# rg2/DeepFluoroLabeling-IPCAI2020

Measured on AMD Instinct MI355X. Metric: train images/sec, paper U-Net (depth 6, wf 5, BN, strided-conv down, seg + 14-landmark heads), 1x192x192 (8x-downsampled 184x184 padded), higher is better.
Workload: dtype bf16 (bf16 activations, activation gradients and GEMM weight copies in HBM; bf16 MFMA, fp32 accumulate, BatchNorm statistics, losses, weight gradients and master weights); 1 GPU; BASELINE configs[1]: 8x-downsampled, seg + 14-landmark heat-map dual head, batch 16 per GPU, Dice+NCC loss, SGD nesterov; global_batch=16, image=1x192x192, parallelism=dp1, math=bf16s, optimizer=dfl_amd.SGD(momentum 0.9, nesterov, wd 1e-4)

## Files before the change

deepfluorolabeling-ipcai2020_amd/_native.py:

```python
import ctypes as C
import os

_HERE = os.path.dirname(os.path.abspath(__file__))
LIB_PATH = os.environ.get('DFL_LIB_OVERRIDE') or os.path.join(_HERE, 'lib', 'libdfl_hip.so')

i32, i64, f32 = C.c_int32, C.c_int64, C.c_float
fp = C.c_void_p


class ConvArgs(C.Structure):
    _fields_ = [('x', fp), ('w', fp), ('bias', fp), ('in_scale', fp), ('in_shift', fp), ('add', fp),
                ('add_scale', fp), ('add_shift', fp), ('stat_other', fp), ('y', fp), ('stat_partials', fp),
                ('partial', fp),
                ('N', i32), ('Hin', i32), ('Win', i32), ('Cin', i32), ('ldx', i32),
                ('KH', i32), ('KW', i32), ('stride', i32), ('pad', i32),
                ('Hout', i32), ('Wout', i32), ('Ntot', i32), ('ldy', i32),
                ('ldadd', i32), ('ldso', i32), ('relu', i32), ('accumulate', i32), ('scatter2x2', i32),
                ('splits', i32), ('w_split', i32), ('x_split', i32), ('x_bf16', i32), ('y_bf16', i32),
                ('x2', fp), ('ldx2', i32), ('x_mode', i32),
                ('stat_totals', fp), ('in_tot', fp), ('in_gamma', fp), ('in_beta', fp), ('add_tot', fp), ('add_gamma', fp),
                ('add_beta', fp), ('in_count', C.c_double), ('add_count', C.c_double), ('bn_eps', f32), ('reserved3', i32),
                ('in_mean', fp), ('in_invstd', fp), ('x_out', fp), ('ldxo', i32), ('latency_form', i32), ('out_scale', fp), ('out_shift', fp)]


class WgradArgs(C.Structure):
    _fields_ = [('g', fp), ('d', fp), ('in_scale', fp), ('in_shift', fp), ('dw', fp), ('partial', fp),
                ('N', i32), ('Hin', i32), ('Win', i32), ('Cg', i32), ('ldg', i32),
                ('KH', i32), ('KW', i32), ('stride', i32), ('pad', i32),
                ('Hout', i32), ('Wout', i32), ('Cm', i32), ('ldd', i32), ('splits', i32), ('d_split', i32),
                ('g_bf16', i32), ('d_bf16', i32), ('d_mode', i32), ('d2', fp), ('coef', fp), ('bias_partial', fp),
                ('ldd2', i32), ('reserved2', i32), ('coef_tot', fp), ('bn_gamma', fp), ('bn_mean', fp), ('bn_invstd', fp),
                ('bn_count', C.c_double)]


class PackJob(C.Structure):
    _fields_ = [('src', fp), ('dst', fp), ('A', i32), ('B', i32), ('C', i32), ('kind', i32), ('flip', i32),
                ('split', i32), ('dst2', fp), ('kind2', i32), ('flip2', i32), ('first_tile', i32), ('split2', i32)]


PACK_PLAIN, SGD_PLAIN_TILE = 100, 4096


class SgdPackArgs(C.Structure):
    _fields_ = [('jobs_dev', fp), ('grad_delta', i64), ('buf_delta', i64), ('njobs', i32), ('total_tiles', i32), ('lr', f32),
                ('momentum', f32), ('weight_decay', f32), ('grad_scale', f32), ('nesterov', i32), ('reserved', i32)]


OPTIM_ADAM, OPTIM_RMSPROP = 1, 2


class OptimPackArgs(C.Structure):
    _fields_ = [('jobs_dev', fp), ('grad_delta', i64), ('state1_delta', i64), ('state2_delta', i64), ('beta1', C.c_double),
                ('beta2', C.c_double), ('alpha', C.c_double), ('njobs', i32), ('total_tiles', i32), ('kind', i32), ('lr', f32),
                ('eps', f32), ('weight_decay', f32), ('grad_scale', f32), ('step_size', f32), ('bc2_sqrt', f32), ('momentum', f32)]


class BnLiveJob(C.Structure):
    _fields_ = [('totals', fp), ('gamma', fp), ('beta', fp), ('running_mean', fp), ('running_var', fp), ('num_batches_tracked', fp),
                ('scale', fp), ('shift', fp), ('save_mean', fp), ('save_invstd', fp), ('count', i64), ('C', i32), ('eps', f32),
                ('momentum', f32), ('reserved', i32)]


class BnBwdLiveJob(C.Structure):
    _fields_ = [('totals', fp), ('save_mean', fp), ('save_invstd', fp), ('dgamma', fp), ('dbeta', fp), ('sum_out', fp), ('C', i32),
                ('reserved', i32)]


class BnBwdLiveArgs(C.Structure):
    _fields_ = [('jobs_dev', fp), ('njobs', i32), ('max_C', i32)]


class BnLiveArgs(C.Structure):
    _fields_ = [('jobs_dev', fp), ('njobs', i32), ('max_C', i32)]


class BnFinalizeArgs(C.Structure):
    _fields_ = [('partials', fp), ('gamma', fp), ('beta', fp), ('running_mean', fp), ('running_var', fp),
                ('num_batches_tracked', fp), ('scale', fp), ('shift', fp), ('save_mean', fp), ('save_invstd', fp),
                ('count', i64), ('nblocks', i32), ('C', i32), ('eps', f32), ('momentum', f32)]


class ColstatsArgs(C.Structure):
    _fields_ = [('a', fp), ('b', fp), ('partials', fp), ('M', i64), ('C', i32), ('lda', i32), ('ldb', i32),
                ('nblocks', i32), ('bf16', i32), ('reserved', i32)]


class BnBwdFinalizeArgs(C.Structure):
    _fields_ = [('partials', fp), ('gamma', fp), ('save_mean', fp), ('save_invstd', fp), ('dgamma', fp),
                ('dbeta', fp), ('coef', fp), ('count', i64), ('nblocks', i32), ('C', i32)]


class BnReluBwdArgs(C.Structure):
    _fields_ = [('dy', fp), ('r', fp), ('coef', fp), ('dpre', fp), ('partials', fp), ('M', i64), ('C', i32),
                ('lddy', i32), ('ldr', i32), ('ldo', i32), ('nblocks', i32), ('split_out', i32), ('bf16', i32),
                ('reserved', i32)]


class AffineCopyArgs(C.Structure):
    _fields_ = [('x', fp), ('y', fp), ('scale', fp), ('shift', fp),
                ('N', i32), ('H', i32), ('W', i32), ('C', i32),
                ('ldx', i32), ('xH', i32), ('xW', i32), ('xoy', i32), ('xox', i32),
                ('ldy', i32), ('yH', i32), ('yW', i32), ('yoy', i32), ('yox', i32),
                ('accumulate', i32), ('bf16', i32)]


class PoolArgs(C.Structure):
    _fields_ = [('x', fp), ('y', fp), ('dx', fp), ('N', i32), ('H', i32), ('W', i32), ('C', i32),
                ('ldx', i32), ('ldy', i32), ('lddx', i32), ('bf16', i32)]


class HeadFwdArgs(C.Structure):
    _fields_ = [('x', fp), ('w_seg', fp), ('w_l1', fp), ('w_l2', fp), ('seg', fp), ('heat', fp),
                ('N', i32), ('H', i32), ('W', i32), ('F', i32), ('ldx', i32),
                ('NC', i32), ('NM', i32), ('L', i32), ('softmax', i32), ('x_bf16', i32)]


class HeadBwdArgs(C.Structure):
    _fields_ = [('x', fp), ('seg', fp), ('dseg', fp), ('dheat', fp), ('w_seg', fp), ('w_l1', fp), ('w_l2', fp),
                ('dx', fp), ('scratch', fp),
                ('N', i32), ('H', i32), ('W', i32), ('F', i32), ('ldx', i32), ('lddx', i32),
                ('NC', i32), ('NM', i32), ('L', i32), ('softmax', i32), ('scratch_ld', i32), ('x_bf16', i32),
                ('dw_seg', fp), ('dw_l1', fp), ('dw_l2', fp), ('wg_partial', fp),
                ('stat_other', fp), ('stat_totals', fp), ('ldso', i32), ('reserved4', i32)]


class LossArgs(C.Structure):
    _fields_ = [('seg', fp), ('tseg', fp), ('heat', fp), ('theat', fp), ('loss', fp), ('dseg', fp), ('dheat', fp),
                ('ncc_vals', fp), ('sums', fp),
                ('seg_sN', i64), ('seg_sC', i64), ('seg_sH', i64), ('tseg_sN', i64), ('tseg_sC', i64), ('tseg_sH', i64),
                ('heat_sN', i64), ('heat_sC', i64), ('heat_sH', i64), ('theat_sN', i64), ('theat_sC', i64),
                ('theat_sH', i64),
                ('B', i32), ('C', i32), ('L', i32), ('h', i32), ('w', i32), ('skip_bg', i32),
                ('dice_wgt', f32), ('heat_wgt', f32), ('grad_scale', fp),
                ('dseg_sN', i64), ('dseg_sC', i64), ('dseg_sH', i64), ('dheat_sN', i64), ('dheat_sC', i64), ('dheat_sH', i64),
                ('stage', i32), ('reserved', i32)]


class EnsembleArgs(C.Structure):
    _fields_ = [('seg_ptrs', fp), ('heat_ptrs', fp), ('labels', fp), ('avg_seg', fp), ('heat_out', fp),
                ('minmax', fp),
                ('nnets', i32), ('C', i32), ('L', i32), ('Hp', i32), ('Wp', i32), ('h', i32), ('w', i32),
                ('oy', i32), ('ox', i32), ('raw_heat', i32)]


class SumPartialsArgs(C.Structure):
    _fields_ = [('src', fp), ('dst', fp), ('n', i64), ('splits', i32), ('T', i32)]


class PackArgs(C.Structure):
    _fields_ = [('jobs_dev', fp), ('max_elems', i64), ('njobs', i32), ('tiled', i32)]


class BnEvalArgs(C.Structure):
    _fields_ = [('gamma', fp), ('beta', fp), ('running_mean', fp), ('running_var', fp), ('scale', fp),
                ('shift', fp), ('C', i32), ('eps', f32)]


class ReducePartialsArgs(C.Structure):
    _fields_ = [('partials', fp), ('out', fp), ('nblocks', i32), ('stride', i32), ('C', i32), ('reserved', i32)]


class MemsetArgs(C.Structure):
    _fields_ = [('ptr', fp), ('bytes', i64)]


class ReduceJob(C.Structure):
    _fields_ = [('src', fp), ('dst', fp), ('n', i64), ('stride', i64), ('count', i32), ('first_block', i32),
                ('T', i32), ('reserved', i32)]


class ReduceBatchArgs(C.Structure):
    _fields_ = [('jobs_dev', fp), ('njobs', i32), ('total_blocks', i32)]


class PrepArgs(C.Structure):
# ... 50 lines not shown
    _fields_ = [('inp', fp), ('out', fp), ('plan', ResamplePlan), ('B', i32), ('reserved', i32)]


class FullresArgs(C.Structure):
    _fields_ = [('image', fp), ('labels', fp), ('rot180', fp), ('boxes', fp), ('n_boxes', fp), ('texts', fp),
                ('stamp_spans', fp), ('text_stamps', fp), ('text_masks', fp), ('scratch', fp), ('out', fp),
                ('plan', ResamplePlan), ('B', i32), ('H', i32), ('W', i32), ('n_tint', i32), ('tint_scale', f32),
                ('tint_add', (f32 * 3) * OVERLAY_MAX_COLORS), ('n_text_stamps', i32), ('n_stamp_spans', i32),
                ('tile0', i32), ('n_tiles', i32)]


MESH_MAX_LABELS, MESH_MC_CELLS, MESH_MAX_ITERS = 4, 4096, 64


class MeshMcArgs(C.Structure):
    _fields_ = [('volume', fp), ('tri_off', fp), ('tri_edges', fp), ('block_counts', fp), ('block_offsets', fp),
                ('totals', fp), ('keys', fp), ('nx', i32), ('ny', i32), ('nz', i32), ('n_labels', i32),
                ('labels', i32 * MESH_MAX_LABELS)]


class MeshDecodeArgs(C.Structure):
    _fields_ = [('keys', fp), ('pos', fp), ('V', i64), ('nx', i32), ('ny', i32)]


class MeshTopoArgs(C.Structure):
    _fields_ = [('tris', fp), ('edge_keys', fp), ('vt_keys', fp), ('T', i64), ('V', i64)]


class MeshCsrArgs(C.Structure):
    _fields_ = [('keys', fp), ('counts', fp), ('col', fp), ('row_ptr', fp), ('fixed', fp), ('nnz', i64), ('div', i64),
                ('col_div', i64), ('n_rows', i64)]


class MeshSmoothArgs(C.Structure):
    _fields_ = [('x', fp), ('row_ptr', fp), ('col', fp), ('fixed', fp), ('t_a', fp), ('t_b', fp), ('acc', fp), ('out', fp),
                ('V', i64), ('iterations', i32), ('reserved', i32), ('coef', f32 * (MESH_MAX_ITERS + 1))]


class MeshXformArgs(C.Structure):
    _fields_ = [('x', fp), ('out', fp), ('V', i64), ('M', C.c_double * 16)]


class MeshNormalsArgs(C.Structure):
    _fields_ = [('pos', fp), ('tris', fp), ('vt_ptr', fp), ('vt_tri', fp), ('normals', fp), ('V', i64)]


PREPROC_MAX_FACTOR = 16


class PreprocProjsArgs(C.Structure):
    _fields_ = [('pixels', fp), ('rot180', fp), ('out', fp), ('scratch', fp), ('N', i32), ('R', i32), ('C', i32),
                ('crop', i32), ('factor', i32), ('u16', i32), ('log', i32), ('min_intensity', f32)]


class PreprocSegsArgs(C.Structure):
    _fields_ = [('segs', fp), ('rot180', fp), ('out', fp), ('status', fp), ('N', i32), ('R', i32), ('C', i32),
                ('crop', i32), ('factor', i32), ('reserved', i32)]


class RestoreLabelsArgs(C.Structure):
    _fields_ = [('labels', fp), ('rot180', fp), ('out', fp), ('N', i32), ('R', i32), ('C', i32), ('crop', i32),
                ('factor', i32), ('reserved', i32)]


DRR_EXACT, DRR_TRILINEAR, DRR_MAX_LABELS = 0, 1, 16


class DrrObject(C.Structure):
    _fields_ = [('o', f32 * 3), ('M', f32 * 9), ('box_lo', i32 * 3), ('box_hi', i32 * 3), ('mask', C.c_uint32)]


class DrrArgs(C.Structure):
    _fields_ = [('mu', fp), ('labels', fp), ('objects', fp), ('att', fp), ('plen', fp), ('label_map', fp), ('qscale', f32 * 9),
                ('nx', i32), ('ny', i32), ('nz', i32), ('H', i32), ('W', i32), ('views', i32), ('n_obj', i32), ('n_labels', i32),
                ('interp', i32), ('mapping', i32), ('step_mm', f32), ('min_len_mm', f32), ('reserved', i32)]


SIM_TOTALS = 5


class SimPrepareArgs(C.Structure):
    _fields_ = [('fixed', fp), ('mask', fp), ('fx', fp), ('fy', fp), ('counted', fp), ('totals', fp), ('H', i32), ('W', i32)]


class SimGradnccArgs(C.Structure):
    _fields_ = [('moving', fp), ('fx', fp), ('fy', fp), ('counted', fp), ('totals', fp), ('scratch', fp), ('cost', fp),
                ('scratch_doubles', i64), ('V', i32), ('H', i32), ('W', i32), ('reserved', i32)]


EXPOSE_MAX_RADIUS = 8


class ExposeArgs(C.Structure):
    _fields_ = [('att', fp), ('out', fp), ('key_q', fp), ('key_e', fp), ('z1', fp), ('z2', fp),
                ('taps', f32 * (2 * EXPOSE_MAX_RADIUS + 1)), ('rho', i32), ('V', i32), ('R', i32), ('C', i32), ('u16', i32),
                ('quantum', i32), ('electronic', i32), ('photons', f32), ('gain', f32), ('electronic_sigma', f32)]


class UpsampleArgs(C.Structure):
    _fields_ = [('x', fp), ('y', fp), ('N', i32), ('H', i32), ('W', i32), ('C', i32), ('ldx', i32), ('ldy', i32),
                ('bf16', i32), ('accumulate', i32)]


class SyncArgs(C.Structure):
    _fields_ = [('event', i32), ('reserved', i32)]


CONV_CFG_LATENCY = 39


class ConvPairArgs(C.Structure):
    _fields_ = [('a', fp), ('b', fp)]


class Op(C.Structure):
    _fields_ = [('kind', i32), ('stream', i32), ('args', fp)]


OP_CONV, OP_WGRAD, OP_SUM_PARTIALS, OP_PACK, OP_BN_FINALIZE, OP_BN_EVAL, OP_COLSTATS, OP_BN_BWD_FINALIZE, \
    OP_BN_RELU_BWD, OP_REDUCE_PARTIALS, OP_AFFINE_COPY, OP_POOL_FWD, OP_POOL_BWD, OP_HEAD_FWD, OP_HEAD_BWD, \
    OP_MEMSET, OP_REDUCE_BATCH, OP_RECORD, OP_WAIT, OP_UPSAMPLE_FWD, OP_UPSAMPLE_BWD, OP_BN_FINALIZE_LIVE, OP_BN_BWD_FINALIZE_LIVE, \
    OP_CONV_PAIR = range(1, 25)

_KIND_OF = {ConvArgs: OP_CONV, WgradArgs: OP_WGRAD, SumPartialsArgs: OP_SUM_PARTIALS, PackArgs: OP_PACK,
            BnFinalizeArgs: OP_BN_FINALIZE, BnEvalArgs: OP_BN_EVAL, ColstatsArgs: OP_COLSTATS,
            BnBwdFinalizeArgs: OP_BN_BWD_FINALIZE, BnReluBwdArgs: OP_BN_RELU_BWD,
            ReducePartialsArgs: OP_REDUCE_PARTIALS, AffineCopyArgs: OP_AFFINE_COPY, HeadFwdArgs: OP_HEAD_FWD,
            HeadBwdArgs: OP_HEAD_BWD, MemsetArgs: OP_MEMSET, ReduceBatchArgs: OP_REDUCE_BATCH, BnLiveArgs: OP_BN_FINALIZE_LIVE, BnBwdLiveArgs: OP_BN_BWD_FINALIZE_LIVE,
            ConvPairArgs: OP_CONV_PAIR}

_SIZEOF_ORDER = [ConvArgs, WgradArgs, PackJob, BnFinalizeArgs, ColstatsArgs, BnBwdFinalizeArgs, BnReluBwdArgs,
                 AffineCopyArgs, PoolArgs, HeadFwdArgs, HeadBwdArgs, LossArgs, EnsembleArgs, Op, ReduceJob, PrepArgs, EstLandsArgs,
                 UpsampleArgs, AugmentArgs, AugmentItem, OverlayArgs, ResamplePlan, ResampleArgs, FullresArgs, MeshMcArgs, MeshDecodeArgs,
                 MeshTopoArgs, MeshCsrArgs, MeshSmoothArgs, MeshXformArgs, MeshNormalsArgs, PreprocProjsArgs, PreprocSegsArgs,
                 RestoreLabelsArgs, SimPrepareArgs, SimGradnccArgs, ExposeArgs, DrrObject, DrrArgs, OptimPackArgs]

EXPORTS = ['dfl_version', 'dfl_last_error', 'dfl_sizeof', 'dfl_conv2d', 'dfl_conv_grid_m', 'dfl_conv2d_wgrad',
           'dfl_wgrad_suggest_splits', 'dfl_sum_partials', 'dfl_pack_weights', 'dfl_bn_finalize',
           'dfl_bn_eval_prepare', 'dfl_rowblock_count', 'dfl_colstats', 'dfl_bn_bwd_finalize',
           'dfl_bn_relu_bwd_apply', 'dfl_reduce_partials', 'dfl_affine_copy', 'dfl_maxpool2x2_fwd',
           'dfl_maxpool2x2_bwd', 'dfl_head_fwd', 'dfl_head_bwd', 'dfl_head_scratch_ld', 'dfl_head_scratch_off',
           'dfl_dice_ncc_loss', 'dfl_loss_scratch_doubles', 'dfl_ensemble_reduce', 'dfl_sgd_step', 'dfl_exec',
           'dfl_exec_timed', 'dfl_conv_config', 'dfl_wgrad_config', 'dfl_conv_suggest_splits', 'dfl_reduce_batch',
           'dfl_reduce_job_blocks', 'dfl_prep_batch', 'dfl_prep_scratch_doubles', 'dfl_est_lands', 'dfl_hard_dice', 'dfl_get_math_mode',
           'dfl_set_math_mode', 'dfl_graph_capture', 'dfl_graph_launch', 'dfl_graph_nodes', 'dfl_graph_destroy',
           'dfl_set_conv_rows_min_tiles', 'dfl_conv_candidates', 'dfl_conv_force_geometry', 'dfl_conv_tune_add',
           'dfl_head_wgrad_blocks', 'dfl_head_scratch_ld_for', 'dfl_head_scratch_off_for', 'dfl_upsample2x_fwd',
           'dfl_upsample2x_bwd', 'dfl_bn_finalize_live', 'dfl_bn_bwd_finalize_live', 'dfl_pack_weights_tiled',
           'dfl_sgd_pack_tiled', 'dfl_conv2d_pair', 'dfl_conv_pair_ok', 'dfl_augment_batch',
           'dfl_augment_scratch_bytes', 'dfl_overlay_batch', 'dfl_resample_bilinear_u8', 'dfl_fullres_overlay',
           'dfl_mesh_mc_count', 'dfl_mesh_mc_emit', 'dfl_mesh_decode', 'dfl_mesh_topology', 'dfl_mesh_csr', 'dfl_mesh_smooth',
           'dfl_mesh_transform', 'dfl_mesh_normals', 'dfl_adam_step', 'dfl_rmsprop_step', 'dfl_optim_pack_tiled',
           'dfl_preproc_projs', 'dfl_preproc_segs', 'dfl_restore_labels', 'dfl_drr_render', 'dfl_sim_prepare', 'dfl_sim_gradncc',
           'dfl_sim_scratch_doubles', 'dfl_drr_expose']


class DflError(RuntimeError):
    pass


_lib = None


def lib():
    global _lib
    if _lib is not None:
        return _lib
    if not os.path.exists(LIB_PATH):
        raise DflError('libdfl_hip.so not found at %s -- build it with __graft_entry__.build() '
                       '(csrc/build.sh); there is no fallback path' % LIB_PATH)
    L = C.CDLL(LIB_PATH)
    for name in EXPORTS:
        if not hasattr(L, name):
            raise DflError('libdfl_hip.so does not export %s' % name)
    L.dfl_last_error.restype = C.c_char_p
    L.dfl_loss_scratch_doubles.restype = i64
    L.dfl_loss_scratch_doubles.argtypes = [i32, i32, i32]
    L.dfl_rowblock_count.argtypes = [i64, i32]
    L.dfl_sum_partials.argtypes = [fp, fp, i64, i32, i32, fp]
    L.dfl_pack_weights.argtypes = [fp, i32, i64, fp]
    L.dfl_pack_weights_tiled.argtypes = [fp, i32, i32, fp]
    L.dfl_sgd_pack_tiled.argtypes = [fp, fp]
    L.dfl_bn_eval_prepare.argtypes = [fp, fp, fp, fp, fp, fp, i32, f32, fp]
    L.dfl_reduce_partials.argtypes = [fp, fp, i32, i32, i32, fp]
    L.dfl_reduce_batch.argtypes = [fp, i32, i32, fp]
    L.dfl_bn_finalize_live.argtypes = [fp, i32, i32, fp]
    L.dfl_bn_bwd_finalize_live.argtypes = [fp, i32, i32, fp]
    L.dfl_reduce_job_blocks.argtypes = [i64, i32]
    L.dfl_prep_scratch_doubles.restype = i64
    L.dfl_prep_scratch_doubles.argtypes = [i32]
    L.dfl_prep_batch.argtypes = [fp, fp]
    L.dfl_est_lands.argtypes = [fp, fp]
    L.dfl_augment_scratch_bytes.restype = i64
    L.dfl_augment_scratch_bytes.argtypes = [i32, i32, i32, i32]
    L.dfl_augment_batch.argtypes = [fp, fp]
    L.dfl_overlay_batch.argtypes = [fp, fp]
    L.dfl_resample_bilinear_u8.argtypes = [fp, fp]
    L.dfl_fullres_overlay.argtypes = [fp, fp]
    for fn in ('dfl_preproc_projs', 'dfl_preproc_segs', 'dfl_restore_labels', 'dfl_drr_render', 'dfl_sim_prepare', 'dfl_sim_gradncc',
               'dfl_drr_expose'):
        getattr(L, fn).argtypes = [fp, fp]
    for fn in ('dfl_mesh_mc_count', 'dfl_mesh_mc_emit', 'dfl_mesh_decode', 'dfl_mesh_topology', 'dfl_mesh_csr',
               'dfl_mesh_smooth', 'dfl_mesh_transform', 'dfl_mesh_normals'):
        getattr(L, fn).argtypes = [fp, fp]
    L.dfl_sim_scratch_doubles.restype = i64
    L.dfl_sim_scratch_doubles.argtypes = [i32, i32, i32]
    L.dfl_set_math_mode.argtypes = [i32]
    L.dfl_hard_dice.argtypes = [fp, fp, i64, i32, i32, fp, fp, fp]
    L.dfl_sgd_step.argtypes = [fp, fp, fp, i64, f32, f32, f32, f32, i32, i32, fp]
    L.dfl_adam_step.argtypes = [fp, fp, fp, fp, i64, f32, C.c_double, C.c_double, f32, f32, f32, f32, f32, fp]
    L.dfl_rmsprop_step.argtypes = [fp, fp, fp, fp, i64, f32, C.c_double, f32, f32, f32, f32, fp]
    L.dfl_optim_pack_tiled.argtypes = [fp, fp]
    L.dfl_exec.argtypes = [fp, i32, fp]
    L.dfl_exec_timed.argtypes = [fp, i32, fp, fp]
    L.dfl_set_conv_rows_min_tiles.argtypes = [i32]
    L.dfl_graph_capture.argtypes = [fp, i32, fp, fp]
    L.dfl_graph_launch.argtypes = [fp, fp]
    L.dfl_graph_nodes.argtypes = [fp]
    L.dfl_graph_destroy.argtypes = [fp]
    L.dfl_conv_config.argtypes = [fp]
    L.dfl_wgrad_config.argtypes = [fp]
    for fn in ('dfl_conv2d', 'dfl_conv2d_wgrad', 'dfl_bn_finalize', 'dfl_colstats', 'dfl_bn_bwd_finalize',
               'dfl_bn_relu_bwd_apply', 'dfl_affine_copy', 'dfl_maxpool2x2_fwd', 'dfl_maxpool2x2_bwd',
               'dfl_head_fwd', 'dfl_head_bwd', 'dfl_dice_ncc_loss', 'dfl_ensemble_reduce', 'dfl_upsample2x_fwd',
               'dfl_upsample2x_bwd'):
        getattr(L, fn).argtypes = [fp, fp]
    for fn in ('dfl_conv_grid_m', 'dfl_wgrad_suggest_splits', 'dfl_conv_suggest_splits'):
        getattr(L, fn).argtypes = [fp]
    L.dfl_conv_candidates.argtypes = [fp, fp, i32]
    L.dfl_head_wgrad_blocks.argtypes = [i64]
    L.dfl_head_scratch_ld_for.argtypes = [i32, i32, i32, i32]
    L.dfl_head_scratch_off_for.argtypes = [i32, i32, i32, i32, i32]
    L.dfl_conv_force_geometry.argtypes = [fp]
    L.dfl_conv_tune_add.argtypes = [fp, fp]
    L.dfl_conv2d_pair.argtypes = [fp, fp, fp]
    L.dfl_conv_pair_ok.argtypes = [fp, fp]
    for k, cls in enumerate(_SIZEOF_ORDER):
        if L.dfl_sizeof(k) != C.sizeof(cls):
            raise DflError('struct mirror %s has size %d, library says %d' % (cls.__name__, C.sizeof(cls), L.dfl_sizeof(k)))
    _lib = L
    if os.environ.get('DFL_TUNE', '1') != '0':
        load_tuning(L, TUNE_PATH)
    return L


TUNE_PATH = os.environ.get('DFL_TUNE_FILE') or os.path.join(_HERE, 'tune', 'gfx950_convp.txt')


def load_tuning(L, path):
    if not os.path.exists(path):
        return 0
    n = 0
    with open(path) as f:
        for line in f:
            line = line.split('#')[0].split()
            if len(line) != 15:
                continue
            v = (i32 * 15)(*[int(t) for t in line])
            if L.dfl_conv_tune_add(C.addressof(v), C.addressof(v) + 40) < 0:
                raise DflError('bad tuning entry in %s: %s' % (path, ' '.join(line)))
            n += 1
    return n


def check(rc, what=''):
    if rc < 0:
        raise DflError('%s failed (%d): %s' % (what or 'libdfl_hip call', rc, lib().dfl_last_error().decode()))
    return rc


def ptr(t):
    return None if t is None else t.data_ptr()


def byref(s):
    return C.addressof(s)


def call(fn_name, args_struct, stream):
    return check(getattr(lib(), fn_name)(C.addressof(args_struct), stream), fn_name)


class Graph:

    def __init__(self, handle, program):
        self.handle, self.program = handle, program

    def launch(self, stream):
        check(lib().dfl_graph_launch(self.handle, stream), 'dfl_graph_launch')

    @property
    def nodes(self):
        return lib().dfl_graph_nodes(self.handle)

    def __del__(self):
        try:
            if self.handle and _lib is not None:
                _lib.dfl_graph_destroy(self.handle)
        except Exception:
            pass
        self.handle = None


class Program:

    def __init__(self):
        self.structs = []
        self.kinds = []
        self.streams = []
        self.volatile = []
        self._ops = None
        self.keep = []
        self._chunks = {}

    def add(self, args_struct, kind=None, stream=0, volatile=False):
        self.structs.append(args_struct)
        self.kinds.append(kind if kind is not None else _KIND_OF[type(args_struct)])
        self.streams.append(stream)
        self.volatile.append(bool(volatile))
        self._ops = None
        self._chunks = {}
        return args_struct

    def insert(self, index, args_struct, kind=None, stream=0, volatile=False):
        self.structs.insert(index, args_struct)
        self.kinds.insert(index, kind if kind is not None else _KIND_OF[type(args_struct)])
        self.streams.insert(index, stream)
        self.volatile.insert(index, bool(volatile))
        self._ops = None
        self._chunks = {}
        return args_struct

    def pop(self):
        self.kinds.pop()
        self.streams.pop()
        self.volatile.pop()
        self._ops = None
        self._chunks = {}
        return self.structs.pop()

    def record(self, event, stream=0):
        return self.add(SyncArgs(event=event), OP_RECORD, stream)

    def wait(self, event, stream=0):
        return self.add(SyncArgs(event=event), OP_WAIT, stream)

    def add_pool(self, args_struct, backward):
        return self.add(args_struct, OP_POOL_BWD if backward else OP_POOL_FWD)

    def extend(self, other):
        for s, k, st, v in zip(other.structs, other.kinds, other.streams, other.volatile):
            self.add(s, k, st, v)
        self.keep.extend(other.keep)

    def __len__(self):
        return len(self.structs)

    def _build(self):
        arr = (Op * len(self.structs))()
        for i, (s, k) in enumerate(zip(self.structs, self.kinds)):
            arr[i].kind = k
            arr[i].stream = self.streams[i]
            arr[i].args = C.addressof(s)
        self._ops = arr

    def run_timed(self, stream):
        if self._ops is None:
            self._build()
        n = len(self.structs)
        ms = (C.c_float * n)()
        check(lib().dfl_exec_timed(C.addressof(self._ops), n, stream, C.addressof(ms)), 'dfl_exec_timed')
        return list(ms)

    def capture(self, stream, start=0, count=None):
        if self._ops is None:
            self._build()
        n = len(self.structs) - start if count is None else count
        h = C.c_void_p()
        check(lib().dfl_graph_capture(C.addressof(self._ops) + start * C.sizeof(Op), n, stream, C.addressof(h)),
              'dfl_graph_capture')
        return Graph(h.value, self)

    MIN_GRAPH_OPS = 2

    def graph_chunks(self, stream, start=0, count=None):
        n = len(self.structs) - start if count is None else count
        key = (start, n)
        chunks = self._chunks.get(key)
        if chunks is None:
# ... 32 lines not shown
```

deepfluorolabeling-ipcai2020_amd/csrc/conv_plan.hip:

```cpp
#include <stdlib.h>
#include <string.h>

#include <mutex>
#include <vector>

#include "conv_plan.h"
#include "conv_rows.h"
#include "direct_small.h"

namespace dfl {

bool convs_enabled() {
  static const bool on = [] {
    const char* e = getenv("DFL_CONVS");
    return e == nullptr || atoi(e) != 0;
  }();
  return on;
}

enum class Family { Patch, Latency, Unrolled, Narrow };
struct Tile {
  Family family;
  int layout;
  int pers;
// ... 230 lines not shown
  if (!ok) return false;
  pl->launch = t.launch;
  pl->pers = t.pers;
  return true;
}

struct ConvGeom { int tile, ipp, ph, pw, splits; };
static thread_local ConvGeom t_force = {-1, 0, 0, 0, 0};
struct TuneEntry { int key[10]; ConvGeom g; };
static std::mutex g_tune_mu;
static std::vector<TuneEntry> g_tune;

static void tune_key(const dfl_conv_args& a, int* k) {
  k[0] = a.N; k[1] = a.Hin; k[2] = a.Win; k[3] = a.Cin; k[4] = a.Ntot;
  k[5] = a.KH; k[6] = a.KW; k[7] = a.stride; k[8] = a.pad; k[9] = a.scatter2x2 ? 1 : 0;
}

static bool tune_lookup(const dfl_conv_args& a, ConvGeom* g) {
  int k[10];
  tune_key(a, k);
  std::lock_guard<std::mutex> lock(g_tune_mu);
  for (const TuneEntry& e : g_tune)
    if (memcmp(e.key, k, sizeof(k)) == 0) {
      *g = e.g;
      return true;
    }
  return false;
}

static bool columns_ok(const dfl_conv_args& a, int wn, int tn, bool wide) {
  const int n32 = (int)ceil_div(a.Ntot, 32) * 32, bn = wn * tn * 32;
  if (wide) return !(bn > n32 || (bn < 64 && n32 >= 64) || (tn > 1 && bn > a.Ntot));
  if (tn != 1) return false;
  return a.Ntot <= 32 ? wn == 1 : (a.Ntot <= 64 ? wn == 2 : wn == 4);
}

static int patch_shapes(const ConvP& base, const PatchTile& t, bool wide, int (*shapes)[3]) {
  const int QP = t.WM * t.TM * 32;
  const int HW = base.Hg * base.Wg;
  int ns = 0;
  if (HW <= QP) {
    shapes[ns][0] = QP / HW; shapes[ns][1] = base.Hg; shapes[ns][2] = base.Wg; ++ns;
  }
  if (base.Wg <= QP) {
    int ph = QP / base.Wg;
    if (ph > base.Hg) ph = base.Hg;
    shapes[ns][0] = 1; shapes[ns][1] = ph; shapes[ns][2] = base.Wg; ++ns;
  }
  static const int kPh[] = {1, 2, 4, 8, 16, 3, 6, 12};
  for (int k = 0; k < (wide ? 8 : 5) && ns < 22; ++k) {
    const int ph = kPh[k];
    int pw = QP / ph;
    if (pw >= base.Wg || ph > base.Hg) continue;
    shapes[ns][0] = 1; shapes[ns][1] = ph; shapes[ns][2] = pw; ++ns;
  }
  return ns;
}

template <typename F>
static void for_each_candidate(const dfl_conv_args& a, const ConvP& base, int force_splits, bool wide, F&& f) {
  const std::vector<Tile>& T = tiles();
  for (int ti = 0; ti < (int)T.size(); ++ti) {
    const Tile& t = T[ti];
    if (t.measured && !wide) continue;
    int shapes[24][3];
    int ns = 0;
    if (t.family == Family::Patch) {
      const PatchTile& pt = convp_tiles()[t.layout];
      if (columns_ok(a, pt.WN, pt.TN, wide)) ns = patch_shapes(base, pt, wide, shapes);
    } else if (t.family == Family::Unrolled) {
      const QLayout& q = convq_layouts()[t.layout];
      if (columns_ok(a, q.WN, 1, wide)) {
        shapes[0][0] = 1; shapes[0][1] = 8 * q.WM; shapes[0][2] = 12; ns = 1;
      }
    } else if (t.family == Family::Narrow) {
      if (convn_shape_ok(a)) {
        shapes[0][0] = 1; narrow_patch(t.layout, &shapes[0][1], &shapes[0][2]); ns = 1;
      }
    }
    for (int si = 0; si < ns; ++si) {
      for (int sp = 1; sp <= 32; sp *= 2) {
        if (force_splits > 0 && sp != force_splits) continue;
        if (!wide && a.scatter2x2 == 0 && a.accumulate == 0 && sp > 1 && base.T * a.Cin < 1024) break;
        ConvPlan q;
        q.p = base;
        if (!try_geometry(a, &q, t, shapes[si][0], shapes[si][1], shapes[si][2], sp)) continue;
        if (q.p.splits != sp) continue;
        f(ti, q);
      }
    }
  }
}

static int convp_validate(const dfl_conv_args* a, ConvP* p) {
  DFL_REQUIRE(a->x && a->w && a->y, "dfl_conv2d (bf16): x, w and y are required");
  DFL_REQUIRE(a->N > 0 && a->Hin > 0 && a->Win > 0 && a->Cin > 0 && a->Ntot > 0, "dfl_conv2d (bf16): bad sizes");
  DFL_REQUIRE(a->Ntot % 8 == 0 && a->ldy % 8 == 0 && aligned16(a->y) && (a->add == nullptr || (a->ldadd % 8 == 0 && aligned16(a->add))) &&
                  (a->stat_other == nullptr || (a->ldso % 8 == 0 && aligned16(a->stat_other))),
              "dfl_conv2d (bf16): output columns and the pixel strides of y / add / stat_other must be multiples of 8, tensors 16-byte aligned");
  {
    const int64_t opx = (int64_t)a->N * a->Hout * a->Wout, lim = 1ll << 32;
    DFL_REQUIRE(opx * a->ldy < lim && (a->add == nullptr || opx * a->ldadd < lim) && (a->stat_other == nullptr || opx * a->ldso < lim),
                "dfl_conv2d (bf16): y / add / stat_other must stay below 2^32 elements");
  }
  DFL_REQUIRE(a->Cin % 16 == 0 && a->ldx % 8 == 0 && aligned16(a->x) && aligned16(a->w),
              "dfl_conv2d (bf16): needs Cin %% 16 == 0, ldx %% 8 == 0 and 16-byte aligned x / w (Cin = %d, ldx = %d)", a->Cin, a->ldx);
  DFL_REQUIRE(a->w_split == 2, "dfl_conv2d (bf16): weights must be packed with dfl_pack_job.split = 2");
  DFL_REQUIRE(a->x_mode != 0 || (a->in_scale == nullptr) == (a->in_shift == nullptr), "dfl_conv2d: in_scale/in_shift go together");
  DFL_REQUIRE(a->in_tot == nullptr || (a->in_scale == nullptr && a->in_gamma != nullptr && a->in_count > 0 &&
                                       (a->x_mode == 0 ? a->in_beta != nullptr : (a->in_mean != nullptr && a->in_invstd != nullptr))),
              "dfl_conv2d (bf16): in_tot replaces in_scale / in_shift and needs in_gamma, in_count and in_beta (x_mode 0) or in_mean, in_invstd (x_mode 1)");
  DFL_REQUIRE(a->add_tot == nullptr || (a->add != nullptr && a->add_scale == nullptr && a->add_gamma != nullptr && a->add_beta != nullptr && a->add_count > 0),
              "dfl_conv2d (bf16): add_tot replaces add_scale / add_shift and needs add, add_gamma, add_beta, add_count");

  DFL_REQUIRE((a->add_scale == nullptr) == (a->add_shift == nullptr), "dfl_conv2d: add_scale/add_shift go together");
  DFL_REQUIRE(a->KH * a->KW <= 16 && a->KH > 0 && a->KW > 0 && a->stride > 0 && a->pad >= 0, "dfl_conv2d (bf16): bad window");
  memset(p, 0, sizeof(*p));
  p->a = *a;
  if (a->scatter2x2) {
    DFL_REQUIRE(a->KH == 1 && a->KW == 1 && a->stride == 1 && a->pad == 0, "dfl_conv2d: scatter2x2 needs a 1x1 gather");
    DFL_REQUIRE(a->Ntot % 4 == 0 && a->Hout >= 2 * a->Hin && a->Wout >= 2 * a->Win, "dfl_conv2d: scatter2x2 geometry");
    DFL_REQUIRE(a->add == nullptr, "dfl_conv2d: scatter2x2 has no add epilogue");
    p->Hg = a->Hin;
    p->Wg = a->Win;
    p->Cout = a->Ntot / 4;
  } else {
    const int ho = (a->Hin + 2 * a->pad - a->KH) / a->stride + 1;
    const int wo = (a->Win + 2 * a->pad - a->KW) / a->stride + 1;
    DFL_REQUIRE(ho == a->Hout && wo == a->Wout, "dfl_conv2d: Hout/Wout (%d,%d) do not match the window (%d,%d)", a->Hout,
                a->Wout, ho, wo);
    p->Hg = a->Hout;
    p->Wg = a->Wout;
    p->Cout = a->Ntot;
  }
  DFL_REQUIRE(a->ldy >= p->Cout, "dfl_conv2d: ldy < Cout");
  const int64_t M = (int64_t)a->N * p->Hg * p->Wg;
  DFL_REQUIRE(M < (1ll << 31), "dfl_conv2d: too many pixels");
  p->Mtot = (int)M;
  p->T = a->KH * a->KW;
  const int64_t xb = (((int64_t)a->N * a->Hin * a->Win - 1) * a->ldx + a->Cin) * 2;
  const int64_t wb = (int64_t)p->T * a->Cin * a->Ntot * 2;
  const int64_t lim = (1ll << 31) - 4096;
  DFL_REQUIRE(xb < lim && wb < lim, "dfl_conv2d (bf16): tensors must stay below 2 GiB");
  p->x_bytes = (uint32_t)xb;
  p->w_bytes = (uint32_t)wb;
  if (a->x_mode != 0) {
    DFL_REQUIRE(a->x_mode == 1 && a->x2 != nullptr && a->in_shift == nullptr && a->ldx2 % 8 == 0 && aligned16(a->x2) &&
                    (a->in_scale == nullptr || aligned16(a->in_scale)),
                "dfl_conv2d (bf16): x_mode 1 needs x2 (16-byte aligned, ldx2 %% 8 == 0), coefficients in in_scale and no in_shift");
    const int64_t x2b = (((int64_t)a->N * a->Hin * a->Win - 1) * a->ldx2 + a->Cin) * 2;
    DFL_REQUIRE(x2b < lim, "dfl_conv2d (bf16): tensors must stay below 2 GiB");
    p->x2_bytes = (uint32_t)x2b;
  }
  p->xo_bytes = 0;
  if (a->x_out != nullptr) {
    DFL_REQUIRE(a->x_mode == 1 && a->KH == 3 && a->KW == 3 && a->stride == 1 && a->pad == 1 && a->Hout == a->Hin && a->Wout == a->Win,
                "dfl_conv2d (bf16): x_out goes with x_mode 1 of a 3x3 stride-1 pad-1 layer");
    DFL_REQUIRE(a->ldxo % 8 == 0 && a->ldxo >= a->Cin && aligned16(a->x_out) && a->x_out != a->x && a->x_out != a->x2,
                "dfl_conv2d (bf16): x_out must be 16-byte aligned with ldxo %% 8 == 0, ldxo >= Cin, and a tensor of its own");
    const int64_t xob = (((int64_t)a->N * a->Hin * a->Win - 1) * a->ldxo + a->Cin) * 2;
    DFL_REQUIRE(xob < lim, "dfl_conv2d (bf16): tensors must stay below 2 GiB");
    p->xo_bytes = (uint32_t)xob;
  }
  return DFL_OK;
}

static int convp_plan_search(const dfl_conv_args* a, ConvPlan* pl, int force_splits) {
  memset(pl, 0, sizeof(*pl));
  const int rc = convp_validate(a, &pl->p);
  if (rc != DFL_OK) return rc;

  if (t_force.tile < 0 && convs_eligible(*a, pl->p)) {
    convs_plan(*a, &pl->p, force_splits);
    pl->lds = (size_t)pl->p.lds_bytes;
    pl->launch = tiles()[CONVS_TILE].launch;
    return DFL_OK;
  }

  DFL_REQUIRE(a->out_scale == nullptr, "dfl_conv2d (bf16): out_scale / out_shift are implemented by the latency form only (dfl_conv_config tells)");
  const ConvP base = pl->p;
  int best_tile = -1;
  {
    ConvGeom g;
    const bool forced = t_force.tile >= 0;
    if (forced) g = t_force;
    if (forced || tune_lookup(*a, &g)) {
      if (g.tile >= 0 && g.tile < (int)tiles().size() && (force_splits <= 0 || force_splits == g.splits)) {
        ConvPlan q = *pl;
        if (try_geometry(*a, &q, tiles()[g.tile], g.ipp, g.ph, g.pw, g.splits) && q.p.splits == g.splits) {
          *pl = q;
          best_tile = g.tile;
        }
      }
      DFL_REQUIRE(!forced || best_tile >= 0, "dfl_conv2d (bf16): the forced geometry (tile %d, patch %dx%dx%d, %d slices) does not fit this layer",
                  g.tile, g.ipp, g.ph, g.pw, g.splits);
    }
  }
  if (best_tile < 0) {
    double best = 1e300;
    for_each_candidate(*a, base, force_splits, false, [&](int ti, const ConvPlan& q) {
      if (q.cost < best) {
        best = q.cost;
        *pl = q;
        best_tile = ti;
      }
    });
  }
  DFL_REQUIRE(best_tile >= 0, "dfl_conv2d (bf16): no patch geometry fits this layer (%dx%d, Cin %d, Ntot %d)", a->Hin, a->Win,
              a->Cin, a->Ntot);
  pl->p.tile = best_tile;
  static const bool dbg = getenv("DFL_CONVP_DEBUG") != nullptr;
  if (dbg && force_splits == 0)
    fprintf(stderr, "convp %dx%d Cin%d->%d k%d s%d: tile %d patch %dx%dx%d CK %d blocks %d splits %d lds %zu cost %.0f%s\n", a->Hin, a->Win,
            a->Cin, a->Ntot, a->KH, a->stride, best_tile, pl->p.IPP, pl->p.PH, pl->p.PW, pl->p.CK, pl->p.nblk, pl->p.splits, pl->lds,
            pl->cost, tiles()[best_tile].measured ? " (measured)" : "");
  return DFL_OK;
}

struct PlanMemo { dfl_conv_args a; int force_splits; ConvPlan pl; };
static std::mutex g_memo_mu;
static std::vector<PlanMemo> g_memo[64];
static inline unsigned memo_bucket(const dfl_conv_args* a, int force_splits) {
  uint64_t h = 1469598103934665603ull;
  const uint64_t* w = reinterpret_cast<const uint64_t*>(a);
  for (size_t i = 0; i < sizeof(dfl_conv_args) / 8; ++i) h = (h ^ w[i]) * 1099511628211ull;
  h ^= (uint64_t)force_splits;
  return (unsigned)((h ^ (h >> 29)) & 63u);
}
static void memo_clear() {
  std::lock_guard<std::mutex> lock(g_memo_mu);
  for (auto& b : g_memo) b.clear();
}

int convp_plan(const dfl_conv_args* a, ConvPlan* pl, int force_splits) {
  static_assert(sizeof(dfl_conv_args) % 8 == 0, "hashed as 64-bit words");
  DFL_REQUIRE(a != nullptr && pl != nullptr, "dfl_conv2d (bf16): null arguments");
  if (t_force.tile >= 0) return convp_plan_search(a, pl, force_splits);
  const unsigned b = memo_bucket(a, force_splits);
  {
    std::lock_guard<std::mutex> lock(g_memo_mu);
    for (const PlanMemo& m : g_memo[b])
      if (m.force_splits == force_splits && memcmp(&m.a, a, sizeof(*a)) == 0) {
        *pl = m.pl;
        return DFL_OK;
      }
  }
  const int rc = convp_plan_search(a, pl, force_splits);
  if (rc != DFL_OK) return rc;
  std::lock_guard<std::mutex> lock(g_memo_mu);
  if (g_memo[b].size() >= 256) g_memo[b].clear();
  g_memo[b].push_back(PlanMemo{*a, force_splits, *pl});
  return DFL_OK;
}

static int convp_candidates(const dfl_conv_args* a, int32_t* out, int max) {
  ConvPlan pl;
  const int saved_tile = t_force.tile;
  t_force.tile = -1;
  const int rc = convp_plan(a, &pl, 0);
  t_force.tile = saved_tile;
  if (rc != DFL_OK) return -1;
  int n = 0;
  for_each_candidate(*a, pl.p, 0, true, [&](int ti, const ConvPlan& q) {
    if (n < max) {
      int32_t* o = out + 5 * n;
      o[0] = ti; o[1] = q.p.IPP; o[2] = q.p.PH; o[3] = q.p.PW; o[4] = q.p.splits;
    }
    ++n;
  });
  return n;
}

static bool latency32_plan(const ConvK& k, int force_splits, ConvPlan* pl) {
  if (!k.a.latency_form || !convs_enabled()) return false;
  memset(pl, 0, sizeof(*pl));
  ConvP* p = &pl->p;
  p->a = k.a;
  p->Mtot = k.Mtot;
  p->Hg = k.Hg;
  p->Wg = k.Wg;
  p->Cout = k.Cout;
  p->T = k.a.KH * k.a.KW;
  p->x_bytes = k.x_bytes;
  p->w_bytes = k.w_bytes;
  if (!convs_eligible(k.a, *p)) return false;
  convs_plan(k.a, p, force_splits);
  pl->lds = (size_t)p->lds_bytes;
  pl->launch = convs_launch;
  return true;
}

int conv_route(const dfl_conv_args* a, int want_splits, ConvRoute* r) {
  if (a != nullptr && a->x_bf16) {
    const int rc = convp_plan(a, &r->plan, want_splits);
    if (rc != DFL_OK) return rc;
    r->form = FORM_BF16;
    r->cfg = 16 + r->plan.p.tile;
    r->splits = r->plan.p.splits;
    return DFL_OK;
  }
  const int rc = conv_prepare(a, &r->k);
  if (rc != DFL_OK) return rc;
  const ConvK& k = r->k;
  int sug;
  if (direct_conv_ok(a)) {
    r->stat_form = FORM_DIRECT;
    r->stat_cfg = CFG_DIRECT;
    sug = 1;
  } else {
    const int t = conv_rows_tile(k);
    r->stat_form = t ? FORM_ROWS : FORM_GEMM;
    r->stat_cfg = t ? t : conv_gemm_cfg(k);
    const int rs = conv_rows_splits(k);
    sug = rs ? rs : conv_gemm_splits(k);
  }
  r->form = r->stat_form;
  r->cfg = r->stat_cfg;
  r->splits = want_splits > 0 ? want_splits : sug;
  if (convs_first_ok(a)) {
    r->form = FORM_FIRST;
    r->cfg = 16 + CONVS_TILE;
    r->splits = 1;
  } else if (latency32_plan(k, want_splits, &r->plan)) {
    r->form = FORM_LATENCY32;
    r->cfg = 16 + CONVS_TILE;
    r->splits = r->plan.p.splits;
  }
  return DFL_OK;
}

static int want_splits(const dfl_conv_args* a) { return a != nullptr && a->splits > 1 ? a->splits : 1; }

int conv_pair_route(const dfl_conv_args* a, const dfl_conv_args* b, ConvRoute* r) {
  if (a == nullptr || b == nullptr || !a->latency_form || conv_route(a, want_splits(a), r) != DFL_OK) return 0;
  return r->form == FORM_BF16 || r->form == FORM_LATENCY32 ? convs_pair_ok(a, b, r->plan.p) : 0;
}

}

extern "C" int dfl_conv_config(const dfl_conv_args* a) {
  dfl::ConvRoute r;
  const int rc = dfl::conv_route(a, dfl::want_splits(a), &r);
  return rc != DFL_OK ? rc : r.cfg;
}

extern "C" int dfl_conv_grid_m(const dfl_conv_args* a) {
  dfl::ConvRoute r;
  const int rc = dfl::conv_route(a, dfl::want_splits(a), &r);
  if (rc != DFL_OK) return rc;
  if (r.form == dfl::FORM_BF16) return r.plan.p.splits > 1 ? dfl::convp_finish_rows(r.plan.p) : r.plan.p.npatch;
  if (a->splits > 1) return dfl::conv_finish_rows(r.k.Mtot, a->Ntot);
  if (r.stat_form == dfl::FORM_DIRECT) return dfl::direct_conv_blocks(a);
  if (r.stat_form == dfl::FORM_ROWS) return r.k.Mtot / dfl::conv_rows_bm(r.stat_cfg);
  return (int)dfl::ceil_div(r.k.Mtot, dfl::conv_gemm_bm(r.stat_cfg));
}

extern "C" int dfl_conv_suggest_splits(const dfl_conv_args* a) {
  dfl::ConvRoute r;
  const int rc = dfl::conv_route(a, 0, &r);
  return rc != DFL_OK ? rc : r.splits;
}

extern "C" int dfl_conv_pair_ok(const dfl_conv_args* a, const dfl_conv_args* b) {
  dfl::ConvRoute r;
  return dfl::conv_pair_route(a, b, &r);
}

extern "C" int dfl_conv_candidates(const dfl_conv_args* a, int32_t* out, int32_t max_rows) {
  DFL_REQUIRE(a != nullptr && (out != nullptr || max_rows <= 0) && a->x_bf16, "dfl_conv_candidates: bf16 convolution arguments and an output table are required");
  const int n = dfl::convp_candidates(a, out, max_rows);
  return n < 0 ? (int)DFL_ERR_INVALID_ARG : n;
}

extern "C" int dfl_conv_force_geometry(const int32_t* geom) {
  if (geom == nullptr) dfl::t_force.tile = -1;
  else dfl::t_force = dfl::ConvGeom{geom[0], geom[1], geom[2], geom[3], geom[4]};
  return DFL_OK;
}

extern "C" int dfl_conv_tune_add(const int32_t* key, const int32_t* geom) {
  DFL_REQUIRE(key == nullptr || geom != nullptr, "dfl_conv_tune_add: a key needs a geometry");
  dfl::memo_clear();
  std::lock_guard<std::mutex> lock(dfl::g_tune_mu);
  if (key == nullptr) {
    dfl::g_tune.clear();
    return DFL_OK;
  }
  dfl::TuneEntry e;
  for (int i = 0; i < 10; ++i) e.key[i] = key[i];
  e.g = dfl::ConvGeom{geom[0], geom[1], geom[2], geom[3], geom[4]};
  for (dfl::TuneEntry& o : dfl::g_tune)
    if (memcmp(o.key, e.key, sizeof(e.key)) == 0) {
      o = e;
      return DFL_OK;
    }
  dfl::g_tune.push_back(e);
  return DFL_OK;
}
```

deepfluorolabeling-ipcai2020_amd/csrc/convp.h:

```cpp
#pragma once
#include "common.h"

namespace dfl {

struct ConvP {
  dfl_conv_args a;
  int Mtot, Cout;
  int Hg, Wg;
  int PH, PW, IPP;
  int npy, npx, npatch;
  int IH, IW;
  int CK, nblk, blk_per_slice;
  int splits, T;
  int pix_stride, upp_shift;
  int lds_bytes, tile;
  int ntiles, grid, xcd_mode;
  uint32_t x_bytes, w_bytes;
  uint32_t x2_bytes, xo_bytes;
  uint32_t mPP, mPW;
  int tab_off, pad1;
  int s_mt, s_nt, s_ksplit_shift, s_cpk_shift, s_ksteps, s_kper;
  uint32_t qm_npatch, qm_ntiles, qm_perimg, qm_npx;
  int q_ngroups, q_stride;
};
constexpr int CONVS_TILE = 39;
constexpr int kLdsOptIn = 160 * 1024;

struct ConvPlan;
typedef int (*ConvLaunch)(const ConvPlan& pl, hipStream_t s);

struct ConvPlan {
  ConvP p;
  size_t lds;
  ConvLaunch launch;
  int pers;
  double cost;
};

int convp_plan(const dfl_conv_args* a, ConvPlan* pl, int force_splits);
int convp_launch(const ConvPlan& pl, hipStream_t s);
int convp_finish_rows(const ConvP& p);
bool convs_enabled();

struct PatchTile { int WM, WN, TM, TN, GA, KS; ConvLaunch launch; };
constexpr int kNumPatchTiles = CONVS_TILE;
const PatchTile* convp_tiles();

struct QLayout { int WM, WN, KS; ConvLaunch launch; };
constexpr int kNumQ = 9;
const QLayout* convq_layouts();
bool convq_shape_ok(const dfl_conv_args& a);
size_t convq_lds_bytes(int ck, int layout, int blk_per_slice, int pers, int* tab_off);
bool convq_pers_ok(int layout, int ck, int x_mode);
bool convq_ck_ok(int layout, int ck);

struct NLayout { int WX, R; ConvLaunch launch; };
constexpr int kNumN = 6;
const NLayout* convn_layouts();
bool convn_shape_ok(const dfl_conv_args& a);
bool convn_layout_ok(int layout, int ntot, int cin);
size_t convn_lds_bytes(int layout, int cin, int ntot, int pers, int* tab_off);
bool convn_pers_ok(int layout, const dfl_conv_args& a);

bool convs_eligible(const dfl_conv_args& a, const ConvP& p);
void convs_plan(const dfl_conv_args& a, ConvP* p, int force_splits);
int convs_launch(const ConvPlan& pl, hipStream_t s);
bool convs_first_ok(const dfl_conv_args* a);
int convs_first_launch(const dfl_conv_args* a, hipStream_t s);
int convs_pair_ok(const dfl_conv_args* a, const dfl_conv_args* b, const ConvP& pa);
int convs_pair_launch(const ConvP& pa, const dfl_conv_args* b, hipStream_t s);

struct WgP;
int wgradp_suggest_splits(const dfl_wgrad_args* a);
int wgradp_launch(const dfl_wgrad_args* a, hipStream_t s);
int wgradp_config(const dfl_wgrad_args* a);

}
```

deepfluorolabeling-ipcai2020_amd/csrc/convp_bf16.hip:

```cpp
#include "common.h"
#include "convp.h"

namespace dfl {

constexpr uint32_t POOB = 0x80000000u;
#ifndef DFL_BRB_U
#define DFL_BRB_U 4
#endif
typedef unsigned int pu32x4 __attribute__((ext_vector_type(4)));

__device__ __forceinline__ float round_bf(float v) { return (float)(__bf16)v; }
__device__ __forceinline__ int pdiv(int q, uint32_t m, int d) { return d == 1 ? q : (int)__umulhi((uint32_t)q, m); }
__device__ __forceinline__ float ld_bf(const __bf16* p) { return (float)*p; }

#ifndef DFL_CONVP_G1
#define DFL_CONVP_G1 4
#endif
#ifndef DFL_CONVP_PRIME
#define DFL_CONVP_PRIME 0
#endif
template <int WM, int WN, int TM, int TN, int AFF, bool GA, int KS = 1>
#ifndef DFL_CONVP_ADEPTH
#define DFL_CONVP_ADEPTH 1
#endif
#ifndef DFL_CONVP_MINW3
#define DFL_CONVP_MINW3 2
#endif
__global__ void __launch_bounds__(256 * KS, (TM * TN >= 6 || KS == 2) ? 1 : (TM * TN <= 3 ? DFL_CONVP_MINW3 : 2)) convp_kernel(const ConvP p) {
  static_assert(WM * WN == 4, "four waves per k-group");
  static_assert(KS == 1 || (KS == 2 && !GA), "two k-groups: LDS-image form only");
  static_assert(AFF != 2 || !GA, "the fused BatchNorm + ReLU backward operand is staged through LDS");
  constexpr int NT = 256 * KS;
  extern __shared__ __attribute__((aligned(16))) unsigned char smem[];
  const dfl_conv_args& a = p.a;
  const int tid = threadIdx.x, lane = tid & 63, wave = (tid >> 6) & 3;
  const int kg = KS == 1 ? 0 : __builtin_amdgcn_readfirstlane(tid >> 8);
  const int wm = wave / WN, wn = wave % WN, li = lane & 31, lh = lane >> 5;
  const int S = p.pix_stride;
  const int PP = p.PH * p.PW;

  int bpatch, btile, bslice;
  {
    const int b = blockIdx.x;
    if (p.xcd_mode == 0) {
      bpatch = b % p.npatch;
      const int r = b / p.npatch;
      btile = r % p.ntiles;
      bslice = r / p.ntiles;
    } else {
      const int x = b & 7, r = b >> 3;
      int s;
      if (p.xcd_mode == 1) {
        s = x + 8 * (r / p.npatch);
        bpatch = r % p.npatch;
      } else {
        const int pairs = p.ntiles * p.splits;
        s = x % pairs;
        bpatch = x / pairs + (8 / pairs) * r;
      }
      if (s >= p.ntiles * p.splits || bpatch >= p.npatch) return;
      btile = s % p.ntiles;
      bslice = s / p.ntiles;
    }
  }
  const int per_img = p.npy * p.npx;
  const int pg = bpatch / per_img, pr = bpatch - pg * per_img;
  const int ppy = pr / p.npx, ppx = pr - ppy * p.npx;
  const int img0 = pg * p.IPP, gy0 = ppy * p.PH, gx0 = ppx * p.PW;
  const int n0 = btile * (WN * TN * 32);

  uint32_t a_base[TM];
#pragma unroll
  for (int i = 0; i < TM; ++i) {
    int q = (wm * TM + i) * 32 + li;
    int img = pdiv(q, p.mPP, PP);
    int r = q - img * PP;
    int py = pdiv(r, p.mPW, p.PW), px = r - py * p.PW;
    if (img >= p.IPP) img = 0, py = 0, px = 0;
    a_base[i] = (uint32_t)(((img * p.IH + py * a.stride) * p.IW + px * a.stride) * S + lh * 16);
  }

  __amdgpu_buffer_rsrc_t rsX = __builtin_amdgcn_make_buffer_rsrc(const_cast<float*>(a.x), 0, (int)p.x_bytes, 0x00020000);
  __amdgpu_buffer_rsrc_t rsW = __builtin_amdgcn_make_buffer_rsrc(const_cast<float*>(a.w), 0, (int)p.w_bytes, 0x00020000);
  uint32_t b_voff[TN];
#pragma unroll
  for (int j = 0; j < TN; ++j) {
    const int n = n0 + (wn * TN + j) * 32 + li;
    b_voff[j] = n < a.Ntot ? (uint32_t)(n * 32 + lh * 16) : POOB;
  }

  f32x16 acc[TM][TN];
#pragma unroll
  for (int i = 0; i < TM; ++i)
#pragma unroll
    for (int j = 0; j < TN; ++j)
#pragma unroll
      for (int r = 0; r < 16; ++r) acc[i][j][r] = 0.f;

  float* in_tab = reinterpret_cast<float*>(smem + p.tab_off);
  float* add_tab = in_tab + 384;
  {
    constexpr int BN0 = WN * TN * 32;
    const bool scat0 = a.scatter2x2 != 0;
    for (int col = tid; col < BN0; col += NT) {
      const int n = n0 + col;
      float sc_ = 1.f, sh_ = 0.f, b_ = 0.f;
      if (n < a.Ntot) {
        if (a.bias != nullptr) b_ = a.bias[scat0 ? n % p.Cout : n];
        if (a.add != nullptr) {
          if (a.add_scale != nullptr) sc_ = a.add_scale[n], sh_ = a.add_shift[n];
          else if (a.add_tot != nullptr) bn_live_affine(a.add_tot, a.add_gamma, a.add_beta, a.add_count, a.bn_eps, a.Ntot, n, &sc_, &sh_);
        }
      }
      add_tab[col] = sc_;
      add_tab[BN0 + col] = sh_;
      add_tab[2 * BN0 + col] = b_;
    }
  }

  const int upp = p.CK >> 3, upp_sh = p.upp_shift;
  const int cg = tid & (upp - 1);
  const int dpix = NT >> upp_sh;
  const int dpix_y = dpix / p.IW, dpix_x = dpix - dpix_y * p.IW;
  const int npix = p.IPP * p.IH * p.IW;
  const int CKC = p.CK >> 4;
  const int ckc_sh = p.upp_shift - 1;
  const int S_steps = p.T * CKC;
  const int cin_chunks = a.Cin >> 4;
  const int KW = a.KW;
  const int kw_magic = (256 + KW - 1) / KW;

#ifdef DFL_CONVP_TRACE
  long long tr_t[10];
  tr_t[6] = tr_t[7] = tr_t[8] = 0;
  tr_t[0] = __builtin_amdgcn_s_memtime();
  tr_t[5] = __builtin_amdgcn_s_memrealtime();
  tr_t[1] = tr_t[2] = 0;
#define TR(i) tr_t[i] = __builtin_amdgcn_s_memtime();
#define TRACC(i, t0) tr_t[i] += __builtin_amdgcn_s_memtime() - (t0);
#else
#define TR(i)
#define TRACC(i, t0)
#endif
  if constexpr (GA) {
    uint32_t a_goff[TM];
#pragma unroll
    for (int i = 0; i < TM; ++i) {
      const int q = (wm * TM + i) * 32 + li;
      const int img = pdiv(q, p.mPP, PP);
      const int r = q - img * PP;
      const int py = pdiv(r, p.mPW, p.PW), px = r - py * p.PW;
      const int n = img0 + img, gy = gy0 + py, gx = gx0 + px;
      const bool ok = img < p.IPP && n < a.N && gy < p.Hg && gx < p.Wg;
      a_goff[i] = ok ? (uint32_t)(((n * a.Hin + gy * a.stride) * a.Win + gx * a.stride) * a.ldx) * 2u + (uint32_t)lh * 16u : POOB;
    }
    constexpr int GG = 2;
    const int chunks = a.Cin >> 4;
    const int steps = p.T * chunks;
    const int ngr = (steps + GG - 1) / GG;
    pu32x4 areg[3][GG][TM], bqreg[3][GG][TN];
    int ls = 0, lcc = 0, ltx = 0;
    uint32_t lao = 0;
    const uint32_t bstep = (uint32_t)a.Ntot * 32u;
    const uint32_t pixb = (uint32_t)a.ldx * 2u;
    const uint32_t tap_x = pixb - (uint32_t)chunks * 32u, tap_y = (uint32_t)(a.Win - a.KW) * pixb;
    auto load_gr = [&](int set) {
#pragma unroll
      for (int e = 0; e < GG; ++e) {
        const bool live = ls < steps;
        const uint32_t ao = live ? lao : 0u, bo = live ? (uint32_t)ls * bstep : 0u;
#pragma unroll
        for (int i = 0; i < TM; ++i) areg[set][e][i] = __builtin_amdgcn_raw_buffer_load_b128(rsX, live ? a_goff[i] : POOB, ao, 0);
#pragma unroll
        for (int j = 0; j < TN; ++j) bqreg[set][e][j] = __builtin_amdgcn_raw_buffer_load_b128(rsW, live ? b_voff[j] : POOB, bo, 0);
        ++ls;
        lao += 32u;
        if (++lcc == chunks) {
          lcc = 0;
          lao += tap_x;
          if (++ltx == a.KW) {
            ltx = 0;
            lao += tap_y;
          }
        }
// ... 62 lines not shown
#pragma unroll
          for (int e = 0; e < 8; ++e) {
            sc[e] = in_tab[cg * 8 + e];
            sh[e] = in_tab[128 + cg * 8 + e];
          }
        } else {
#pragma unroll
          for (int e = 0; e < 8; ++e) {
            sc[e] = a.in_scale[c0 + cg * 8 + e];
            sh[e] = a.in_shift[c0 + cg * 8 + e];
          }
        }
      }
      __amdgpu_buffer_rsrc_t rsR = rsX, rsO = rsX;
      bool store_on = false;
      if constexpr (AFF == 2) {
        rsR = __builtin_amdgcn_make_buffer_rsrc(const_cast<float*>(a.x2), 0, (int)p.x2_bytes, 0x00020000);
        store_on = a.x_out != nullptr && btile == 0;
        if (store_on) rsO = __builtin_amdgcn_make_buffer_rsrc(a.x_out, 0, (int)p.xo_bytes, 0x00020000);
        if (a.in_tot != nullptr) {
          if (tid < p.CK)
            bn_live_coef(a.in_tot, a.in_gamma, a.in_mean, a.in_invstd, a.in_count, a.Cin, c0 + tid, in_tab + tid, in_tab + 128 + tid, in_tab + 256 + tid);
          __syncthreads();
#pragma unroll
          for (int e = 0; e < 8; ++e) {
            sc[e] = in_tab[cg * 8 + e];
            sh[e] = in_tab[128 + cg * 8 + e];
            sq[e] = in_tab[256 + cg * 8 + e];
          }
        } else {
#pragma unroll
          for (int e = 0; e < 8; ++e) {
            const int c = c0 + cg * 8 + e;
            sc[e] = a.in_scale != nullptr ? a.in_scale[c] : 1.f;
            sh[e] = a.in_scale != nullptr ? a.in_scale[a.Cin + c] : 0.f;
            sq[e] = a.in_scale != nullptr ? a.in_scale[2 * a.Cin + c] : 0.f;
          }
        }
      }
      int pix = tid >> upp_sh;
      int img = pix / (p.IH * p.IW);
      int rem = pix - img * (p.IH * p.IW);
      int iy = rem / p.IW, ix = rem - iy * p.IW;
      const int ybase = gy0 * a.stride - a.pad, xbase = gx0 * a.stride - a.pad;
      const uint32_t cbyte = (uint32_t)((c0 + cg * 8) * 2);
      constexpr int U = AFF == 2 ? DFL_BRB_U : 8;
      for (; pix < npix; pix += U * dpix) {
        pu32x4 v[U], v2[AFF == 2 ? U : 1];
        uint32_t offo[AFF == 2 ? U : 1];
        bool ok[U];
        int pixs[U];
#pragma unroll
        for (int u = 0; u < U; ++u) {
          const int gy = ybase + iy, gx = xbase + ix, n = img0 + img;
          pixs[u] = pix + u * dpix;
          ok[u] = pixs[u] < npix && n < a.N && (unsigned)gy < (unsigned)a.Hin && (unsigned)gx < (unsigned)a.Win;
          const uint32_t off = (uint32_t)(((n * a.Hin + gy) * a.Win + gx) * a.ldx) * 2u + cbyte;
          v[u] = __builtin_amdgcn_raw_buffer_load_b128(rsX, ok[u] ? off : POOB, 0, 0);
          if constexpr (AFF == 2) {
            const uint32_t off2 = (uint32_t)(((n * a.Hin + gy) * a.Win + gx) * a.ldx2) * 2u + cbyte;
            v2[u] = __builtin_amdgcn_raw_buffer_load_b128(rsR, ok[u] ? off2 : POOB, 0, 0);
            const bool own = store_on && ok[u] && (unsigned)(iy - a.pad) < (unsigned)p.PH && (unsigned)(ix - a.pad) < (unsigned)p.PW;
            offo[u] = own ? (uint32_t)(((n * a.Hin + gy) * a.Win + gx) * a.ldxo) * 2u + cbyte : POOB;
          }
          ix += dpix_x;
          iy += dpix_y;
          if (ix >= p.IW) {
            ix -= p.IW;
            ++iy;
          }
          while (iy >= p.IH) {
            iy -= p.IH;
            ++img;
          }
        }
#pragma unroll
        for (int u = 0; u < U; ++u) {
          if (pixs[u] < npix) {
            pu32x4 w = v[u];
            if constexpr (AFF == 1) {
              if (ok[u]) {
                w.x = pack_bf2(fmaf(bf_lo(w.x), sc[0], sh[0]), fmaf(bf_hi(w.x), sc[1], sh[1]));
                w.y = pack_bf2(fmaf(bf_lo(w.y), sc[2], sh[2]), fmaf(bf_hi(w.y), sc[3], sh[3]));
                w.z = pack_bf2(fmaf(bf_lo(w.z), sc[4], sh[4]), fmaf(bf_hi(w.z), sc[5], sh[5]));
                w.w = pack_bf2(fmaf(bf_lo(w.w), sc[6], sh[6]), fmaf(bf_hi(w.w), sc[7], sh[7]));
              }
            }
            if constexpr (AFF == 2) {
              const pu32x4 r = v2[u];
              auto brb = [](float dy, float rv, float A, float B, float Cc) { return rv > 0.f ? fmaf(A, dy, fmaf(B, rv, Cc)) : 0.f; };
              w.x = pack_bf2(brb(bf_lo(w.x), bf_lo(r.x), sc[0], sh[0], sq[0]), brb(bf_hi(w.x), bf_hi(r.x), sc[1], sh[1], sq[1]));
              w.y = pack_bf2(brb(bf_lo(w.y), bf_lo(r.y), sc[2], sh[2], sq[2]), brb(bf_hi(w.y), bf_hi(r.y), sc[3], sh[3], sq[3]));
              w.z = pack_bf2(brb(bf_lo(w.z), bf_lo(r.z), sc[4], sh[4], sq[4]), brb(bf_hi(w.z), bf_hi(r.z), sc[5], sh[5], sq[5]));
              w.w = pack_bf2(brb(bf_lo(w.w), bf_lo(r.w), sc[6], sh[6], sq[6]), brb(bf_hi(w.w), bf_hi(r.w), sc[7], sh[7], sq[7]));
              if (store_on) __builtin_amdgcn_raw_buffer_store_b128(w, rsO, offo[u], 0, 0);
            }
            *reinterpret_cast<pu32x4*>(smem + (uint32_t)pixs[u] * (uint32_t)S + (uint32_t)cg * 16u) = w;
          }
        }
      }
    }
    __syncthreads();
    TRACC(1, tb0)
#ifdef DFL_CONVP_TRACE
    const long long tb1 = __builtin_amdgcn_s_memtime();
#endif

    static_assert(G % 2 == 0 || DFL_CONVP_ADEPTH == 1, "the A-fragment sets alternate inside a group");
    constexpr int AD = DFL_CONVP_ADEPTH;
    bf16x8_t afq[AD][TM];
    auto fetch_a = [&](int s, int slot) {
      s = s < S_steps ? s : S_steps - 1;
      const int tap = s >> ckc_sh, cc = s & (CKC - 1);
      const int ty = (tap * kw_magic) >> 8, tx = tap - ty * KW;
      const uint32_t aoff = (uint32_t)((ty * p.IW + tx) * S + cc * 32);
#pragma unroll
      for (int i = 0; i < TM; ++i) afq[slot][i] = __builtin_bit_cast(bf16x8_t, *reinterpret_cast<const pu32x4*>(smem + a_base[i] + aoff));
    };
    auto compute_group = [&](int gl, int set) {
      const int g = gl * KS + kg;
#pragma unroll
      for (int e = 0; e < G; ++e) {
        bf16x8_t af[TM];
#pragma unroll
        for (int i = 0; i < TM; ++i) af[i] = afq[e % AD][i];
        fetch_a(e + AD < G ? g * G + e + AD : (g + KS) * G + (e + AD - G), e % AD);
#pragma unroll
        for (int j = 0; j < TN; ++j) {
          const bf16x8_t bf = __builtin_bit_cast(bf16x8_t, breg[set][e][j]);
#pragma unroll
          for (int i = 0; i < TM; ++i) acc[i][j] = __builtin_amdgcn_mfma_f32_32x32x16_bf16(af[i], bf, acc[i][j], 0, 0, 0);
        }
      }
    };
#pragma unroll
    for (int d = 0; d < AD; ++d) fetch_a(kg * G + d, d);
    if (!DFL_CONVP_PRIME) {
      load_group(blk, 0, 0);
      load_group(blk, 1, 1);
    }
    for (int g = 0; g < ngroups; g += 3) {
      load_group(blk, g + 2, 2);
      compute_group(g, 0);
      if (g + 1 < ngroups) {
        load_group(blk, g + 3, 0);
        compute_group(g + 1, 1);
      }
      if (g + 2 < ngroups) {
        load_group(blk, g + 4, 1);
        compute_group(g + 2, 2);
      }
    }
    TRACC(2, tb1)
  }
  }
  TR(3)

  if constexpr (KS == 2) {
    constexpr int XP = WN * TN * 32 + 4;
    float* xg = reinterpret_cast<float*>(smem);
#pragma unroll
    for (int i = 0; i < TM; ++i) {
      __syncthreads();
      if (kg == 1) {
#pragma unroll
        for (int j = 0; j < TN; ++j)
#pragma unroll
          for (int r = 0; r < 16; ++r) xg[(wm * 32 + mfma32_row(r, lane)) * XP + (wn * TN + j) * 32 + li] = acc[i][j][r];
      }
      __syncthreads();
      if (kg == 0) {
#pragma unroll
        for (int j = 0; j < TN; ++j)
#pragma unroll
          for (int r = 0; r < 16; ++r) acc[i][j][r] += xg[(wm * 32 + mfma32_row(r, lane)) * XP + (wn * TN + j) * 32 + li];
      }
    }
  }

  const bool sliced = p.splits > 1;
  if (sliced) {
    if (KS == 2 && kg == 1) return;
    float* part = a.partial + (int64_t)bslice * p.Mtot * a.Ntot;
#pragma unroll
    for (int i = 0; i < TM; ++i) {
#pragma unroll
      for (int g = 0; g < 4; ++g) {
        const int q = (wm * TM + i) * 32 + 8 * g + 4 * lh;
        int img = pdiv(q, p.mPP, PP);
        int r = q - img * PP;
        int py = pdiv(r, p.mPW, p.PW), px = r - py * p.PW;
#pragma unroll
        for (int rr = 0; rr < 4; ++rr) {
          const int n = img0 + img, gy = gy0 + py, gx = gx0 + px;
          const bool rok = img < p.IPP && n < a.N && gy < p.Hg && gx < p.Wg;
          const int64_t m = ((int64_t)n * p.Hg + gy) * p.Wg + gx;
#pragma unroll
          for (int j = 0; j < TN; ++j) {
            const int col = n0 + (wn * TN + j) * 32 + li;
            if (rok && col < a.Ntot) part[m * a.Ntot + col] = acc[i][j][4 * g + rr];
          }
          if (++px == p.PW) {
            px = 0;
            if (++py == p.PH) {
              py = 0;
              ++img;
            }
          }
        }
      }
    }
    return;
  }

  constexpr int BN = WN * TN * 32;
  if constexpr (GA) __syncthreads();
  constexpr int EP = BN + 4;
  constexpr int UPR = BN / 8;
  constexpr int RPS = (NT / UPR) < WM * 32 ? (NT / UPR) : WM * 32;
  static_assert(NT % UPR == 0 && (WM * 32) % RPS == 0, "row phase mapping");
  const bool rowthread = (RPS * UPR == NT) ? true : (tid < RPS * UPR);
  float* ep = reinterpret_cast<float*>(smem);
  const bool do_stats = a.stat_partials != nullptr || a.stat_totals != nullptr;
  const bool scat = a.scatter2x2 != 0;
  const unsigned short* addp = reinterpret_cast<const unsigned short*>(a.add);
  const unsigned short* sop = reinterpret_cast<const unsigned short*>(a.stat_other);
  unsigned short* yp = reinterpret_cast<unsigned short*>(a.y);
  const int ucol = (tid % UPR) * 8;
  const int urow = tid / UPR;
  const int ncol = n0 + ucol;
  const bool cok = ncol < a.Ntot;
  const int cab = (scat && cok) ? ncol / p.Cout : 0;
  const int cco = scat ? ncol - cab * p.Cout : ncol;
  float cbias[8], casc[8], cash[8], s1[8], s2[8];
#pragma unroll
  for (int e = 0; e < 8; ++e) {
    casc[e] = add_tab[ucol + e];
    cash[e] = add_tab[BN + ucol + e];
    cbias[e] = add_tab[2 * BN + ucol + e];
    s1[e] = 0.f;
    s2[e] = 0.f;
  }
  auto unpack = [](const pu32x4 w, float* f) {
    f[0] = bf_lo(w.x); f[1] = bf_hi(w.x); f[2] = bf_lo(w.y); f[3] = bf_hi(w.y);
    f[4] = bf_lo(w.z); f[5] = bf_hi(w.z); f[6] = bf_lo(w.w); f[7] = bf_hi(w.w);
  };
  __builtin_amdgcn_s_waitcnt(0x0F70);
#pragma unroll
  for (int i = 0; i < TM; ++i) {
#ifdef DFL_CONVP_TRACE
    const long long te0 = __builtin_amdgcn_s_memtime();
#endif
    __syncthreads();
    TRACC(6, te0)
#ifdef DFL_CONVP_TRACE
    const long long te1 = __builtin_amdgcn_s_memtime();
#endif
    if (KS == 1 || kg == 0) {
#pragma unroll
      for (int j = 0; j < TN; ++j)
#pragma unroll
        for (int r = 0; r < 16; ++r)
          ep[(wm * 32 + mfma32_row(r, lane)) * EP + (wn * TN + j) * 32 + li] = acc[i][j][r];
    }
    __syncthreads();
    TRACC(7, te1)
#ifdef DFL_CONVP_TRACE
    const long long te2 = __builtin_amdgcn_s_memtime();
#endif
    for (int rl = rowthread ? urow : WM * 32; rl < WM * 32; rl += RPS) {
      const int q = ((rl >> 5) * TM + i) * 32 + (rl & 31);
      const int img = pdiv(q, p.mPP, PP);
      const int rr = q - img * PP;
      const int py = pdiv(rr, p.mPW, p.PW), px = rr - py * p.PW;
      const int n = img0 + img, gy = gy0 + py, gx = gx0 + px;
      if (!(cok && img < p.IPP && n < a.N && gy < p.Hg && gx < p.Wg)) continue;
      const uint32_t m = (uint32_t)((n * p.Hg + gy) * p.Wg + gx);
      float v[8];
      const float4 v0 = *reinterpret_cast<const float4*>(ep + rl * EP + ucol);
      const float4 v1 = *reinterpret_cast<const float4*>(ep + rl * EP + ucol + 4);
      v[0] = v0.x; v[1] = v0.y; v[2] = v0.z; v[3] = v0.w; v[4] = v1.x; v[5] = v1.y; v[6] = v1.z; v[7] = v1.w;
#pragma unroll
      for (int e = 0; e < 8; ++e) {
        v[e] += cbias[e];
        if (a.relu) v[e] = fmaxf(v[e], 0.f);
      }
      if (addp != nullptr) {
        float o[8];
        unpack(*reinterpret_cast<const pu32x4*>(addp + (m * (uint32_t)a.ldadd + (uint32_t)ncol)), o);
#pragma unroll
        for (int e = 0; e < 8; ++e) v[e] += fmaf(o[e], casc[e], cash[e]);
      }
      const uint32_t opix = scat ? (uint32_t)((n * a.Hout + 2 * gy + (cab >> 1)) * a.Wout + 2 * gx + (cab & 1)) : m;
      const int ocol = scat ? cco : ncol;
      const uint32_t yo = opix * (uint32_t)a.ldy + (uint32_t)ocol;
      if (a.accumulate) {
        float o[8];
        unpack(*reinterpret_cast<const pu32x4*>(yp + yo), o);
#pragma unroll
        for (int e = 0; e < 8; ++e) v[e] += o[e];
      }
      pu32x4 w;
      w.x = pack_bf2(v[0], v[1]);
      w.y = pack_bf2(v[2], v[3]);
      w.z = pack_bf2(v[4], v[5]);
      w.w = pack_bf2(v[6], v[7]);
      *reinterpret_cast<pu32x4*>(yp + yo) = w;
      if (do_stats) {
        float vr[8], u[8];
        unpack(w, vr);
        if (sop != nullptr) {
          unpack(*reinterpret_cast<const pu32x4*>(sop + (opix * (uint32_t)a.ldso + (uint32_t)ocol)), u);
        } else {
#pragma unroll
          for (int e = 0; e < 8; ++e) u[e] = vr[e];
        }
#pragma unroll
        for (int e = 0; e < 8; ++e) {
          s1[e] += vr[e];
          s2[e] = fmaf(vr[e], u[e], s2[e]);
        }
      }
    }
    TRACC(8, te2)
  }
#ifdef DFL_CONVP_TRACE
  if (tid == 0 && a.partial != nullptr) {
    long long* sink = reinterpret_cast<long long*>(a.partial) + (int64_t)(bpatch + p.npatch * btile) * 12;
    sink[8] = tr_t[6]; sink[9] = tr_t[7]; sink[10] = tr_t[8];
    sink[0] = tr_t[0]; sink[1] = tr_t[1]; sink[2] = tr_t[2]; sink[3] = tr_t[3]; sink[4] = __builtin_amdgcn_s_memtime();
    sink[5] = tr_t[5]; sink[6] = __builtin_amdgcn_s_memrealtime(); sink[7] = 1;
  }
#endif
  if (!do_stats) return;
  __syncthreads();
  float* red = reinterpret_cast<float*>(smem);
  if (rowthread) {
#pragma unroll
    for (int e = 0; e < 8; ++e) {
      red[(urow * 2 + 0) * BN + ucol + e] = s1[e];
      red[(urow * 2 + 1) * BN + ucol + e] = s2[e];
    }
  }
  __syncthreads();
  for (int idx = tid; idx < 2 * BN; idx += NT) {
    const int which = idx / BN, col = idx - which * BN;
    const int n = n0 + col;
    if (n < a.Ntot) {
      float sum = 0.f;
      for (int w = 0; w < RPS; ++w) sum += red[(w * 2 + which) * BN + col];
      if (scat) {
        const int ab = n / p.Cout, co = n - ab * p.Cout;
        if (a.stat_totals != nullptr) bn_live_add(a.stat_totals, bpatch * 4 + ab, which, p.Cout, co, sum);
        else a.stat_partials[(((int64_t)bpatch * 4 + ab) * 2 + which) * p.Cout + co] = sum;
      } else if (a.stat_totals != nullptr) {
        bn_live_add(a.stat_totals, bpatch, which, a.Ntot, n, sum);
      } else {
        a.stat_partials[((int64_t)bpatch * 2 + which) * a.Ntot + n] = sum;
      }
    }
  }
}

__global__ void __launch_bounds__(256) convp_finish_kernel(const ConvP p, int TX, int rows_per_block) {
  __shared__ float red[2][256];
  const dfl_conv_args& a = p.a;
  const int Ntot = a.Ntot;
  const int TY = 256 / TX;
  const int tx = threadIdx.x % TX, ty = threadIdx.x / TX;
  const int n = blockIdx.y * TX + tx;
  const bool nok = n < Ntot;
  int co = n, ab = 0;
  if (a.scatter2x2 && nok) {
    ab = n / p.Cout;
    co = n - ab * p.Cout;
  }
  const float bias = (a.bias != nullptr && nok) ? a.bias[co] : 0.f;
  float asc = 1.f, ash = 0.f;
  if (a.add != nullptr && a.add_scale != nullptr && nok) {
    asc = a.add_scale[n];
    ash = a.add_shift[n];
  } else if (a.add != nullptr && a.add_tot != nullptr && nok) {
    bn_live_affine(a.add_tot, a.add_gamma, a.add_beta, a.add_count, a.bn_eps, Ntot, n, &asc, &ash);
  }
  const __bf16* addp = reinterpret_cast<const __bf16*>(a.add);
  const __bf16* sop = reinterpret_cast<const __bf16*>(a.stat_other);
  __bf16* yp = reinterpret_cast<__bf16*>(a.y);
  const float osc = (a.out_scale != nullptr && nok) ? a.out_scale[co] : 1.f, osh = (a.out_scale != nullptr && nok) ? a.out_shift[co] : 0.f;
  const int64_t slice = (int64_t)p.Mtot * Ntot;
  const int r0 = blockIdx.x * rows_per_block;
  const int r1 = min(r0 + rows_per_block, p.Mtot);
  float s1 = 0.f, s2 = 0.f;
  if (nok) {
    for (int m = r0 + ty; m < r1; m += TY) {
      const float* pp = a.partial + (int64_t)m * Ntot + n;
      float v = 0.f;
      for (int s = 0; s < p.splits; ++s) v += pp[(int64_t)s * slice];
      v += bias;
      if (a.relu) v = fmaxf(v, 0.f);
      if (addp != nullptr) v += fmaf(ld_bf(addp + (int64_t)m * a.ldadd + n), asc, ash);
      int64_t opix = m;
      if (a.scatter2x2) {
        const int jx = m % p.Wg;
        const int t = m / p.Wg;
        const int iy = t % p.Hg;
        const int ni = t / p.Hg;
        opix = ((int64_t)ni * a.Hout + 2 * iy + (ab >> 1)) * a.Wout + 2 * jx + (ab & 1);
      }
      __bf16* dst = yp + opix * a.ldy + co;
      if (a.accumulate) v += (float)*dst;
      __bf16 hv = (__bf16)v;
      if (a.out_scale != nullptr) hv = (__bf16)fmaf((float)hv, osc, osh);
      *dst = hv;
      const float vr = (float)hv;
      const float u = (sop != nullptr) ? ld_bf(sop + opix * a.ldso + co) : vr;
      s1 += vr;
      s2 = fmaf(vr, u, s2);
    }
  }
  if (a.stat_partials == nullptr && a.stat_totals == nullptr) return;
  red[0][threadIdx.x] = s1;
  red[1][threadIdx.x] = s2;
  __syncthreads();
  if (ty == 0 && nok) {
    float t1 = 0.f, t2 = 0.f;
    for (int y = 0; y < TY; ++y) {
      t1 += red[0][y * TX + tx];
      t2 += red[1][y * TX + tx];
    }
    if (a.scatter2x2 && a.stat_totals != nullptr) {
      bn_live_add(a.stat_totals, (int)blockIdx.x * 4 + ab, 0, p.Cout, co, t1);
      bn_live_add(a.stat_totals, (int)blockIdx.x * 4 + ab, 1, p.Cout, co, t2);
    } else if (a.scatter2x2) {
      a.stat_partials[(((int64_t)blockIdx.x * 4 + ab) * 2 + 0) * p.Cout + co] = t1;
      a.stat_partials[(((int64_t)blockIdx.x * 4 + ab) * 2 + 1) * p.Cout + co] = t2;
    } else if (a.stat_totals != nullptr) {
      bn_live_add(a.stat_totals, (int)blockIdx.x, 0, Ntot, n, t1);
      bn_live_add(a.stat_totals, (int)blockIdx.x, 1, Ntot, n, t2);
    } else {
      a.stat_partials[((int64_t)blockIdx.x * 2 + 0) * Ntot + n] = t1;
      a.stat_partials[((int64_t)blockIdx.x * 2 + 1) * Ntot + n] = t2;
    }
  }
}


constexpr int FIN_ROWS = 128;
constexpr int FIN_TX = 32;
static int finish_rows_p(int M, int Ntot) {
  int64_t nb = ceil_div((int64_t)M * Ntot, 1024);
  if (nb > 2048) nb = 2048;
  if (nb > FIN_ROWS) nb = FIN_ROWS;
  if (nb > M) nb = M;
  return nb < 1 ? 1 : (int)nb;
}

int convp_finish_rows(const ConvP& p) { return finish_rows_p(p.Mtot, p.a.Ntot); }

template <int WM, int WN, int TM, int TN, bool GA = false, int KS = 1>
static int convp_launch_t(const ConvPlan& pl, hipStream_t s) {
  const ConvP& p = pl.p;
  const bool aff = p.a.in_scale != nullptr || p.a.in_tot != nullptr;
  dim3 grid((unsigned)p.grid);
  constexpr int NT_ = 256 * KS;
  if constexpr (GA) {
    auto k = convp_kernel<WM, WN, TM, TN, 0, true>;
    DFL_LDS_OPT_IN(k, kLdsOptIn, "dfl_conv2d (bf16)")
    hipLaunchKernelGGL(k, grid, dim3(256), pl.lds, s, p);
  } else if (p.a.x_mode != 0) {
    auto k = convp_kernel<WM, WN, TM, TN, 2, false, KS>;
    DFL_LDS_OPT_IN(k, kLdsOptIn, "dfl_conv2d (bf16)")
    hipLaunchKernelGGL(k, grid, dim3(NT_), pl.lds, s, p);
  } else if (aff) {
    auto k = convp_kernel<WM, WN, TM, TN, 1, false, KS>;
    DFL_LDS_OPT_IN(k, kLdsOptIn, "dfl_conv2d (bf16)")
    hipLaunchKernelGGL(k, grid, dim3(NT_), pl.lds, s, p);
  } else {
    auto k = convp_kernel<WM, WN, TM, TN, 0, false, KS>;
    DFL_LDS_OPT_IN(k, kLdsOptIn, "dfl_conv2d (bf16)")
    hipLaunchKernelGGL(k, grid, dim3(NT_), pl.lds, s, p);
  }
  return check_launch("dfl_conv2d (bf16)");
}

const PatchTile* convp_tiles() {
  static const PatchTile t[kNumPatchTiles] = {
    {4, 1, 2, 1, 0, 1, convp_launch_t<4, 1, 2, 1>}, {4, 1, 1, 1, 0, 1, convp_launch_t<4, 1, 1, 1>}, {2, 2, 4, 1, 0, 1, convp_launch_t<2, 2, 4, 1>},
    {2, 2, 3, 1, 0, 1, convp_launch_t<2, 2, 3, 1>}, {2, 2, 2, 1, 0, 1, convp_launch_t<2, 2, 2, 1>}, {1, 4, 2, 1, 0, 1, convp_launch_t<1, 4, 2, 1>},
    {1, 4, 3, 1, 0, 1, convp_launch_t<1, 4, 3, 1>}, {1, 4, 4, 1, 0, 1, convp_launch_t<1, 4, 4, 1>}, {1, 4, 6, 1, 0, 1, convp_launch_t<1, 4, 6, 1>},
    {1, 4, 9, 1, 0, 1, convp_launch_t<1, 4, 9, 1>}, {2, 2, 1, 1, 0, 1, convp_launch_t<2, 2, 1, 1>}, {1, 4, 1, 1, 0, 1, convp_launch_t<1, 4, 1, 1>},
    {4, 1, 3, 1, 0, 1, convp_launch_t<4, 1, 3, 1>}, {4, 1, 4, 1, 0, 1, convp_launch_t<4, 1, 4, 1>}, {2, 2, 6, 1, 0, 1, convp_launch_t<2, 2, 6, 1>},
    {2, 2, 2, 2, 0, 1, convp_launch_t<2, 2, 2, 2>}, {2, 2, 3, 2, 0, 1, convp_launch_t<2, 2, 3, 2>}, {2, 2, 4, 2, 0, 1, convp_launch_t<2, 2, 4, 2>},
    {4, 1, 2, 2, 0, 1, convp_launch_t<4, 1, 2, 2>}, {4, 1, 3, 2, 0, 1, convp_launch_t<4, 1, 3, 2>}, {1, 4, 2, 2, 0, 1, convp_launch_t<1, 4, 2, 2>},
    {1, 4, 3, 2, 0, 1, convp_launch_t<1, 4, 3, 2>},
    {4, 1, 1, 1, 1, 1, convp_launch_t<4, 1, 1, 1, true>}, {4, 1, 2, 1, 1, 1, convp_launch_t<4, 1, 2, 1, true>},
    {2, 2, 1, 1, 1, 1, convp_launch_t<2, 2, 1, 1, true>}, {2, 2, 2, 1, 1, 1, convp_launch_t<2, 2, 2, 1, true>},
    {1, 4, 1, 1, 1, 1, convp_launch_t<1, 4, 1, 1, true>}, {1, 4, 2, 1, 1, 1, convp_launch_t<1, 4, 2, 1, true>},
    {4, 1, 1, 2, 1, 1, convp_launch_t<4, 1, 1, 2, true>}, {2, 2, 1, 2, 1, 1, convp_launch_t<2, 2, 1, 2, true>},
    {1, 4, 3, 1, 0, 2, convp_launch_t<1, 4, 3, 1, false, 2>}, {1, 4, 2, 1, 0, 2, convp_launch_t<1, 4, 2, 1, false, 2>},
    {1, 4, 4, 1, 0, 2, convp_launch_t<1, 4, 4, 1, false, 2>}, {2, 2, 3, 1, 0, 2, convp_launch_t<2, 2, 3, 1, false, 2>},
    {2, 2, 2, 1, 0, 2, convp_launch_t<2, 2, 2, 1, false, 2>}, {1, 4, 2, 2, 0, 2, convp_launch_t<1, 4, 2, 2, false, 2>},
    {2, 2, 2, 2, 0, 2, convp_launch_t<2, 2, 2, 2, false, 2>}, {4, 1, 3, 1, 0, 2, convp_launch_t<4, 1, 3, 1, false, 2>},
    {4, 1, 2, 1, 0, 2, convp_launch_t<4, 1, 2, 1, false, 2>}};
  return t;
}

int convp_launch(const ConvPlan& pl, hipStream_t s) {
  const ConvP& p = pl.p;
  const int rc = pl.launch(pl, s);
  if (rc != DFL_OK || p.splits <= 1) return rc;
  int tx = 1;
  while (tx * 2 <= p.a.Ntot && tx * 2 <= FIN_TX) tx *= 2;
  const int nb = finish_rows_p(p.Mtot, p.a.Ntot);
  const int rpb = (int)ceil_div(p.Mtot, nb);
  dim3 grid((unsigned)nb, (unsigned)ceil_div(p.a.Ntot, tx));
  hipLaunchKernelGGL(convp_finish_kernel, grid, dim3(256), 0, s, p, tx, rpb);
  return check_launch("dfl_conv2d (bf16, split-K finish)");
}

}
```

deepfluorolabeling-ipcai2020_amd/csrc/convq_bf16.hip:

```cpp
#include "common.h"
#include "convp.h"

namespace dfl {
namespace {

constexpr uint32_t QOOB = 0x80000000u;
typedef unsigned int qu32x4 __attribute__((ext_vector_type(4)));

__device__ __forceinline__ void q_unpack(const qu32x4 w, float* f) {
  f[0] = bf_lo(w.x); f[1] = bf_hi(w.x); f[2] = bf_lo(w.y); f[3] = bf_hi(w.y);
  f[4] = bf_lo(w.z); f[5] = bf_hi(w.z); f[6] = bf_lo(w.w); f[7] = bf_hi(w.w);
}

constexpr int QPW = 12, QIW = 14, QTM = 3;
constexpr int q_row_pitch(int ck) {
  int r = QIW * (2 * ck + 16) / 16;
  while (r % 16 != 12) ++r;
  return r * 16;
}
constexpr int q_buf_bytes(int ck, int wm, int wn, int ks, int pers) {
  const int img = (8 * wm + 2) * q_row_pitch(ck);
  if (pers == 0) return img;
  const int nt = 64 * wm * wn * ks, bn = 32 * wn;
  const int epi = ks * wm * 32 * (bn + 4) * 4, red = (nt / (bn / 8)) * 2 * bn * 4;
  int b = img > epi ? img : epi;
  b = b > red ? b : red;
  return (b + 15) / 16 * 16;
}

template <int CK, int WM, int WN, int KS, int AFF, int PERS>
__global__ void __launch_bounds__(64 * WM * WN * KS, 2) convq_kernel(const ConvP p) {
  constexpr int NT = 64 * WM * WN * KS;
  static_assert(NT == 256 || NT == 512, "four or eight waves");
  constexpr int QBN = 32 * WN, QEP = QBN + 4;
  constexpr int QPH = 8 * WM, QIH = QPH + 2, QNPIX = QIH * QIW;
  constexpr int S = 2 * CK + 16;
  constexpr int RPB = q_row_pitch(CK);
  static_assert(RPB >= QIW * S && (RPB / 16) % 16 == 12, "conflict-free row pitch");
  constexpr int CKC = CK / 16, CCL = CKC / KS, STEPS = 9 * CCL;
  constexpr int GS = (STEPS % 12 == 0) ? 4 : 3;
  constexpr int NG = STEPS / GS;
  static_assert(CCL >= 1 && STEPS % GS == 0 && NG % 3 == 0 && STEPS % 3 == 0, "ring and fragment slots are static");
  constexpr int UPX = CK / 8;
  constexpr int NU = QNPIX * UPX;
  constexpr int U = (NU + NT - 1) / NT;
  constexpr int CHU = (U + 2) / 3;
  constexpr int NCH = (U + CHU - 1) / CHU;
  static_assert(NT % UPX == 0, "a thread keeps its channel group");
  constexpr int EPP = (WN == 4 && PERS == 0) ? 1 : 3;
  constexpr int TPP = QTM / EPP;
  constexpr int RW = 32 * TPP;
  constexpr int RI = WM * RW;
  constexpr int UPR = QBN / 8;
  constexpr int RPS = NT / UPR;
  constexpr int BUF = q_buf_bytes(CK, WM, WN, KS, PERS);
  constexpr int ROWS_UNROLL = PERS == 2 ? 1 : 8;
  extern __shared__ __attribute__((aligned(16))) unsigned char smem[];
  const dfl_conv_args& a = p.a;
  const int tid = threadIdx.x, lane = tid & 63, li = lane & 31, lh = lane >> 5;
  const int wave = __builtin_amdgcn_readfirstlane(tid >> 6);
  const int wn = wave % WN, wm = (wave / WN) % WM, kg = wave / (WN * WM);

  auto qdiv = [](int q, uint32_t m, int d) { return d == 1 ? q : (int)__umulhi((uint32_t)q, m); };
  int pidx, btile, bslice;
  {
    const int b = blockIdx.x;
    if (PERS != 0) {
      const int r = qdiv(b, p.qm_npatch, p.q_ngroups);
      pidx = b - r * p.q_ngroups;
      bslice = qdiv(r, p.qm_ntiles, p.ntiles);
      btile = r - bslice * p.ntiles;
    } else if (p.xcd_mode == 0) {
      const int r = qdiv(b, p.qm_npatch, p.npatch);
      pidx = b - r * p.npatch;
      bslice = qdiv(r, p.qm_ntiles, p.ntiles);
      btile = r - bslice * p.ntiles;
    } else {
      const int x = b & 7, r = b >> 3;
      int s;
      if (p.xcd_mode == 1) {
        const int rq = qdiv(r, p.qm_npatch, p.npatch);
        s = x + 8 * rq;
        pidx = r - rq * p.npatch;
      } else {
        const int pairs = p.ntiles * p.splits;
        s = x % pairs;
        pidx = x / pairs + (8 / pairs) * r;
      }
      if (s >= p.ntiles * p.splits || pidx >= p.npatch) return;
      bslice = qdiv(s, p.qm_ntiles, p.ntiles);
      btile = s - bslice * p.ntiles;
    }
  }
  const int pstride = PERS != 0 ? p.q_ngroups : 0x40000000;
  const int per_img = p.npy * p.npx;
  struct Pos { int gy0, gx0, img; };
  auto pos_of = [&](int pi) {
    const int img = qdiv(pi, p.qm_perimg, per_img), pr = pi - img * per_img;
    const int ppy = qdiv(pr, p.qm_npx, p.npx), ppx = pr - ppy * p.npx;
    return Pos{ppy * QPH, ppx * QPW, img};
  };
  const int n0 = btile * QBN;
  const int blk_begin = bslice * p.blk_per_slice;
  const int blk_end = min(blk_begin + p.blk_per_slice, p.nblk);
  const int CKS = p.blk_per_slice * CK;

  __amdgpu_buffer_rsrc_t rsX = __builtin_amdgcn_make_buffer_rsrc(const_cast<float*>(a.x), 0, (int)p.x_bytes, 0x00020000);
  __amdgpu_buffer_rsrc_t rsW = __builtin_amdgcn_make_buffer_rsrc(const_cast<float*>(a.w), 0, (int)p.w_bytes, 0x00020000);
  __amdgpu_buffer_rsrc_t rsR = rsX, rsO = rsX;
  bool store_on = false;
  if constexpr (AFF == 2) {
    rsR = __builtin_amdgcn_make_buffer_rsrc(const_cast<float*>(a.x2), 0, (int)p.x2_bytes, 0x00020000);
    store_on = a.x_out != nullptr && btile == 0;
    if (store_on) rsO = __builtin_amdgcn_make_buffer_rsrc(a.x_out, 0, (int)p.xo_bytes, 0x00020000);
  }

  const int ncol = n0 + wn * 32 + li;
  const uint32_t b_voff = ncol < a.Ntot ? (uint32_t)(ncol * 32 + lh * 16) : QOOB;
  const uint32_t nt32 = (uint32_t)a.Ntot * 32u;
  const uint32_t tapS = (uint32_t)(a.Cin >> 4) * nt32;
  qu32x4 breg[3][GS];
  auto load_group = [&](const int g, const uint32_t wb, const bool live) __attribute__((always_inline)) {
#pragma unroll
    for (int e = 0; e < GS; ++e) {
      const int s = g * GS + e, t = s / CCL, c = s % CCL;
      const uint32_t soff = wb + (uint32_t)t * tapS + (uint32_t)c * nt32;
      breg[g % 3][e] = __builtin_amdgcn_raw_buffer_load_b128(rsW, live ? b_voff : QOOB, live ? soff : 0u, 0);
    }
  };
  auto wbase = [&](int blk) { return (uint32_t)(blk * CKC + kg * CCL) * nt32; };
  load_group(0, wbase(blk_begin), true);
  load_group(1, wbase(blk_begin), true);

  const int cg = tid & (UPX - 1);
  const int pix0 = tid / UPX;
  float* col_tab = reinterpret_cast<float*>(smem + p.tab_off);
  float* in_tab = col_tab + 3 * QBN;
  struct Unit { qu32x4 v, v2; };
  auto unit_pix = [&](int j) { return pix0 + j * (NT / UPX); };
  auto unit_load = [&](int j, const Pos& ps, int c0, bool live, Unit* un) __attribute__((always_inline)) {
    const int pix = unit_pix(j);
    const int iy = pix / QIW, ix = pix - iy * QIW;
    const int gy = ps.gy0 - 1 + iy, gx = ps.gx0 - 1 + ix;
    const bool ok = live && pix < QNPIX && (unsigned)gy < (unsigned)a.Hin && (unsigned)gx < (unsigned)a.Win;
    const uint32_t pixel = ((uint32_t)ps.img * (uint32_t)a.Hin + (uint32_t)gy) * (uint32_t)a.Win + (uint32_t)gx;
    const uint32_t cb = (uint32_t)((c0 + cg * 8) * 2);
    un->v = __builtin_amdgcn_raw_buffer_load_b128(rsX, ok ? pixel * (uint32_t)a.ldx * 2u + cb : QOOB, 0, 0);
    if constexpr (AFF == 2) un->v2 = __builtin_amdgcn_raw_buffer_load_b128(rsR, ok ? pixel * (uint32_t)a.ldx2 * 2u + cb : QOOB, 0, 0);
  };
  auto unit_store = [&](int j, const Pos& ps, int c0, int crel, uint32_t buf, const Unit& un) __attribute__((always_inline)) {
    const int pix = unit_pix(j);
    if (pix >= QNPIX) return;
    const int iy = pix / QIW, ix = pix - iy * QIW;
    const int gy = ps.gy0 - 1 + iy, gx = ps.gx0 - 1 + ix;
    const bool ok = (unsigned)gy < (unsigned)a.Hin && (unsigned)gx < (unsigned)a.Win;
    qu32x4 w = un.v;
    if constexpr (AFF == 1) {
      if (ok) {
        const float4 s0 = *reinterpret_cast<const float4*>(in_tab + crel + cg * 8), s1 = *reinterpret_cast<const float4*>(in_tab + crel + cg * 8 + 4);
        const float4 h0 = *reinterpret_cast<const float4*>(in_tab + CKS + crel + cg * 8), h1 = *reinterpret_cast<const float4*>(in_tab + CKS + crel + cg * 8 + 4);
        w.x = pack_bf2(fmaf(bf_lo(w.x), s0.x, h0.x), fmaf(bf_hi(w.x), s0.y, h0.y));
        w.y = pack_bf2(fmaf(bf_lo(w.y), s0.z, h0.z), fmaf(bf_hi(w.y), s0.w, h0.w));
        w.z = pack_bf2(fmaf(bf_lo(w.z), s1.x, h1.x), fmaf(bf_hi(w.z), s1.y, h1.y));
        w.w = pack_bf2(fmaf(bf_lo(w.w), s1.z, h1.z), fmaf(bf_hi(w.w), s1.w, h1.w));
      }
    }
    if constexpr (AFF == 2) {
      const qu32x4 r = un.v2;
      const float4 A0 = *reinterpret_cast<const float4*>(in_tab + crel + cg * 8), A1 = *reinterpret_cast<const float4*>(in_tab + crel + cg * 8 + 4);
      const float4 B0 = *reinterpret_cast<const float4*>(in_tab + CKS + crel + cg * 8), B1 = *reinterpret_cast<const float4*>(in_tab + CKS + crel + cg * 8 + 4);
      const float4 C0 = *reinterpret_cast<const float4*>(in_tab + 2 * CKS + crel + cg * 8), C1 = *reinterpret_cast<const float4*>(in_tab + 2 * CKS + crel + cg * 8 + 4);
      auto brb = [](float dy, float rv, float A, float B, float Cc) { return rv > 0.f ? fmaf(A, dy, fmaf(B, rv, Cc)) : 0.f; };
      w.x = pack_bf2(brb(bf_lo(w.x), bf_lo(r.x), A0.x, B0.x, C0.x), brb(bf_hi(w.x), bf_hi(r.x), A0.y, B0.y, C0.y));
      w.y = pack_bf2(brb(bf_lo(w.y), bf_lo(r.y), A0.z, B0.z, C0.z), brb(bf_hi(w.y), bf_hi(r.y), A0.w, B0.w, C0.w));
      w.z = pack_bf2(brb(bf_lo(w.z), bf_lo(r.z), A1.x, B1.x, C1.x), brb(bf_hi(w.z), bf_hi(r.z), A1.y, B1.y, C1.y));
      w.w = pack_bf2(brb(bf_lo(w.w), bf_lo(r.w), A1.z, B1.z, C1.z), brb(bf_hi(w.w), bf_hi(r.w), A1.w, B1.w, C1.w));
      if (store_on) {
        const bool own = ok && (unsigned)(iy - 1) < (unsigned)QPH && (unsigned)(ix - 1) < (unsigned)QPW;
        const uint32_t pixel = ((uint32_t)ps.img * (uint32_t)a.Hin + (uint32_t)gy) * (uint32_t)a.Win + (uint32_t)gx;
        __builtin_amdgcn_raw_buffer_store_b128(w, rsO, own ? pixel * (uint32_t)a.ldxo * 2u + (uint32_t)((c0 + cg * 8) * 2) : QOOB, 0, 0);
      }
    }
    *reinterpret_cast<qu32x4*>(smem + buf + (uint32_t)(iy * RPB + ix * S) + (uint32_t)cg * 16u) = w;
  };

  Pos pos = pos_of(pidx);
  {
    constexpr int UG = AFF == 2 ? 6 : 10;
    constexpr int UG0 = U < UG ? U : UG;
    Unit un[UG0];
#pragma unroll
    for (int j = 0; j < UG0; ++j) unit_load(j, pos, blk_begin * CK, true, &un[j]);
    if (tid < QBN) {
      const int col = n0 + tid;
      const bool ok = col < a.Ntot;
      float b_ = 0.f, sc_ = 1.f, sh_ = 0.f;
      if (a.bias != nullptr && ok && p.splits <= 1) b_ = a.bias[col];
      if (a.add != nullptr && ok) {
        if (a.add_scale != nullptr) sc_ = a.add_scale[col], sh_ = a.add_shift[col];
        else if (a.add_tot != nullptr) bn_live_affine(a.add_tot, a.add_gamma, a.add_beta, a.add_count, a.bn_eps, a.Ntot, col, &sc_, &sh_);
      }
      col_tab[tid] = b_;
      col_tab[QBN + tid] = sc_;
      col_tab[2 * QBN + tid] = sh_;
    }
    if constexpr (AFF == 1) {
      for (int c = tid; c < CKS; c += NT) {
        const int ch = blk_begin * CK + c;
        float sc_, sh_;
        if (a.in_tot != nullptr) bn_live_affine(a.in_tot, a.in_gamma, a.in_beta, a.in_count, a.bn_eps, a.Cin, ch, &sc_, &sh_);
        else sc_ = a.in_scale[ch], sh_ = a.in_shift[ch];
        in_tab[c] = sc_;
        in_tab[CKS + c] = sh_;
      }
    }
    if constexpr (AFF == 2) {
      for (int c = tid; c < CKS; c += NT) {
        const int ch = blk_begin * CK + c;
        float A = 1.f, B = 0.f, Cc = 0.f;
        if (a.in_tot != nullptr) bn_live_coef(a.in_tot, a.in_gamma, a.in_mean, a.in_invstd, a.in_count, a.Cin, ch, &A, &B, &Cc);
        else if (a.in_scale != nullptr) A = a.in_scale[ch], B = a.in_scale[a.Cin + ch], Cc = a.in_scale[2 * a.Cin + ch];
        in_tab[c] = A;
        in_tab[CKS + c] = B;
        in_tab[2 * CKS + c] = Cc;
      }
    }
    if (AFF != 0) __syncthreads();
#pragma unroll
    for (int j = 0; j < UG0; ++j) unit_store(j, pos, blk_begin * CK, 0, 0u, un[j]);
#pragma unroll
    for (int j0 = UG0; j0 < U; j0 += UG0) {
#pragma unroll
      for (int j = 0; j < UG0; ++j)
        if (j0 + j < U) unit_load(j0 + j, pos, blk_begin * CK, true, &un[j]);
#pragma unroll
      for (int j = 0; j < UG0; ++j)
        if (j0 + j < U) unit_store(j0 + j, pos, blk_begin * CK, 0, 0u, un[j]);
    }
  }
  Unit deep[PERS == 2 ? U : 1];
  if constexpr (PERS == 2) {
    const bool live = pidx + pstride < p.npatch;
    const Pos pn = pos_of(live ? pidx + pstride : pidx);
#pragma unroll
    for (int j = 0; j < U; ++j) unit_load(j, pn, blk_begin * CK, live, &deep[j]);
  }

  uint32_t a_addr[QTM];
#pragma unroll
  for (int i = 0; i < QTM; ++i) {
    const int q = i * 32 + li, py = q / QPW, px = q - py * QPW;
    a_addr[i] = (uint32_t)((py + wm * 8) * RPB + px * S + lh * 16 + kg * CCL * 32);
  }
  f32x16 acc[QTM];
  bf16x8_t afr[3][QTM];
  auto fetch_a = [&](const int s) __attribute__((always_inline)) {
    const int t = s / CCL, c = s % CCL;
    const int off = (t / 3) * RPB + (t % 3) * S + c * 32;
#pragma unroll
    for (int i = 0; i < QTM; ++i) afr[s % 3][i] = __builtin_bit_cast(bf16x8_t, *reinterpret_cast<const qu32x4*>(smem + a_addr[i] + off));
  };
  const int ucol = (tid % UPR) * 8, urow = tid / UPR;
  const int ecol = n0 + ucol;
  const bool cok = ecol < a.Ntot;
  const bool sliced = p.splits > 1;
  const bool do_stats = !sliced && (a.stat_partials != nullptr || a.stat_totals != nullptr);
  const unsigned short* addp = reinterpret_cast<const unsigned short*>(a.add);
  const unsigned short* sop = reinterpret_cast<const unsigned short*>(a.stat_other);
  unsigned short* yp = reinterpret_cast<unsigned short*>(a.y);
  __syncthreads();

  uint32_t cur = 0u;
  for (;;) {
    const int pnext = pidx + pstride;
    const bool next_ok = PERS != 0 && pnext < p.npatch;
    const Pos posn = pos_of(next_ok ? pnext : pidx);
#pragma unroll
    for (int i = 0; i < QTM; ++i)
#pragma unroll
      for (int r = 0; r < 16; ++r) acc[i][r] = 0.f;
    fetch_a(0);
    fetch_a(1);
    for (int blk = blk_begin; blk < blk_end; ++blk) {
      const bool last = PERS == 2 ? true : blk + 1 == blk_end;
      const bool ring_next = !last || next_ok;
      const bool has_next = PERS == 2 ? false : (!last || (PERS == 1 && next_ok));
      const uint32_t wb = wbase(blk), wbn = wbase(last ? blk_begin : blk + 1);
      const uint32_t nxt = BUF - cur;
      const Pos& psn = last ? posn : pos;
      const int c0n = last ? blk_begin * CK : (blk + 1) * CK, creln = last ? 0 : (blk + 1 - blk_begin) * CK;
      Unit un[CHU];
#pragma unroll
      for (int t = 0; t < 9; ++t) {
#pragma unroll
        for (int c = 0; c < CCL; ++c) {
          const int s = t * CCL + c;
          if (s % GS == 0) {
            const int g = s / GS + 2;
            if (g < NG) load_group(g, wb, true);
            else load_group(g - NG, wbn, ring_next);
          }
          if (s + 2 < STEPS) fetch_a(s + 2);
          const bf16x8_t bf = __builtin_bit_cast(bf16x8_t, breg[(s / GS) % 3][s % GS]);
#pragma unroll
          for (int i = 0; i < QTM; ++i) acc[i] = __builtin_amdgcn_mfma_f32_32x32x16_bf16(afr[s % 3][i], bf, acc[i], 0, 0, 0);
          __builtin_amdgcn_sched_barrier(0);
        }
        if ((t & 1) == 0 && has_next) {
          const int ch = t / 2;
          if (ch >= 1 && ch - 1 < NCH) {
#pragma unroll
            for (int e = 0; e < CHU; ++e)
              if ((ch - 1) * CHU + e < U) unit_store((ch - 1) * CHU + e, psn, c0n, creln, nxt, un[e]);
          }
          if (ch < NCH) {
#pragma unroll
            for (int e = 0; e < CHU; ++e)
              if (ch * CHU + e < U) unit_load(ch * CHU + e, psn, c0n, true, &un[e]);
          }
        }
      }
      if (!last) {
        __syncthreads();
#pragma unroll
        for (int i = 0; i < QTM; ++i) a_addr[i] += nxt - cur;
        cur = nxt;
        fetch_a(0);
        fetch_a(1);
      }
    }
    if constexpr (PERS == 2) {
      if (next_ok) {
#pragma unroll
        for (int j = 0; j < U; ++j) unit_store(j, posn, blk_begin * CK, 0, BUF - cur, deep[j]);
      }
      const bool live = pnext + pstride < p.npatch;
      const Pos pn2 = pos_of(live ? pnext + pstride : pidx);
#pragma unroll
      for (int j = 0; j < U; ++j) unit_load(j, pn2, blk_begin * CK, live, &deep[j]);
    }

    __syncthreads();
    float* ep = reinterpret_cast<float*>(smem + (PERS != 0 ? cur : 0u));
    float s1[8], s2[8];
#pragma unroll
    for (int e = 0; e < 8; ++e) {
      s1[e] = 0.f;
      s2[e] = 0.f;
    }
#pragma unroll
    for (int pass = 0; pass < EPP; ++pass) {
      if (pass > 0) __syncthreads();
#pragma unroll
      for (int i = 0; i < TPP; ++i)
#pragma unroll
        for (int r = 0; r < 16; ++r) ep[(kg * RI + wm * RW + i * 32 + mfma32_row(r, lane)) * QEP + wn * 32 + li] = acc[pass * TPP + i][r];
      __syncthreads();
#pragma unroll ROWS_UNROLL
      for (int rl = urow; rl < RI; rl += RPS) {
        const int rw = rl / RW, q = rw * 96 + pass * RW + (rl - rw * RW);
        const int py = q / QPW, px = q - py * QPW;
        const int gy = pos.gy0 + py, gx = pos.gx0 + px;
        if (!(cok && gy < p.Hg && gx < p.Wg)) continue;
        const uint32_t m = (uint32_t)((pos.img * p.Hg + gy) * p.Wg + gx);
        float v[8];
        {
          const float4 v0 = *reinterpret_cast<const float4*>(ep + rl * QEP + ucol);
          const float4 v1 = *reinterpret_cast<const float4*>(ep + rl * QEP + ucol + 4);
          v[0] = v0.x; v[1] = v0.y; v[2] = v0.z; v[3] = v0.w; v[4] = v1.x; v[5] = v1.y; v[6] = v1.z; v[7] = v1.w;
        }
        if constexpr (KS == 2) {
          const float4 v0 = *reinterpret_cast<const float4*>(ep + (RI + rl) * QEP + ucol);
          const float4 v1 = *reinterpret_cast<const float4*>(ep + (RI + rl) * QEP + ucol + 4);
          v[0] += v0.x; v[1] += v0.y; v[2] += v0.z; v[3] += v0.w; v[4] += v1.x; v[5] += v1.y; v[6] += v1.z; v[7] += v1.w;
        }
        if (sliced) {
          float* part = a.partial + ((int64_t)bslice * p.Mtot + m) * a.Ntot + ecol;
          *reinterpret_cast<float4*>(part) = make_float4(v[0], v[1], v[2], v[3]);
          *reinterpret_cast<float4*>(part + 4) = make_float4(v[4], v[5], v[6], v[7]);
          continue;
        }
        {
          const float4 b0 = *reinterpret_cast<const float4*>(col_tab + ucol), b1 = *reinterpret_cast<const float4*>(col_tab + ucol + 4);
          const float cb[8] = {b0.x, b0.y, b0.z, b0.w, b1.x, b1.y, b1.z, b1.w};
#pragma unroll
          for (int e = 0; e < 8; ++e) {
            v[e] += cb[e];
            if (a.relu) v[e] = fmaxf(v[e], 0.f);
          }
        }
        if (addp != nullptr) {
          float o[8];
          q_unpack(*reinterpret_cast<const qu32x4*>(addp + (m * (uint32_t)a.ldadd + (uint32_t)ecol)), o);
          const float4 c0 = *reinterpret_cast<const float4*>(col_tab + QBN + ucol), c1 = *reinterpret_cast<const float4*>(col_tab + QBN + ucol + 4);
          const float4 h0 = *reinterpret_cast<const float4*>(col_tab + 2 * QBN + ucol), h1 = *reinterpret_cast<const float4*>(col_tab + 2 * QBN + ucol + 4);
          const float sc[8] = {c0.x, c0.y, c0.z, c0.w, c1.x, c1.y, c1.z, c1.w}, sh[8] = {h0.x, h0.y, h0.z, h0.w, h1.x, h1.y, h1.z, h1.w};
#pragma unroll
          for (int e = 0; e < 8; ++e) v[e] += fmaf(o[e], sc[e], sh[e]);
        }
        const uint32_t yo = m * (uint32_t)a.ldy + (uint32_t)ecol;
        if (a.accumulate) {
          float o[8];
          q_unpack(*reinterpret_cast<const qu32x4*>(yp + yo), o);
#pragma unroll
          for (int e = 0; e < 8; ++e) v[e] += o[e];
        }
        qu32x4 w;
        w.x = pack_bf2(v[0], v[1]);
        w.y = pack_bf2(v[2], v[3]);
        w.z = pack_bf2(v[4], v[5]);
        w.w = pack_bf2(v[6], v[7]);
        *reinterpret_cast<qu32x4*>(yp + yo) = w;
        if (do_stats) {
          float vr[8], u[8];
          q_unpack(w, vr);
          if (sop != nullptr) {
            q_unpack(*reinterpret_cast<const qu32x4*>(sop + (m * (uint32_t)a.ldso + (uint32_t)ecol)), u);
          } else {
#pragma unroll
            for (int e = 0; e < 8; ++e) u[e] = vr[e];
          }
#pragma unroll
          for (int e = 0; e < 8; ++e) {
            s1[e] += vr[e];
            s2[e] = fmaf(vr[e], u[e], s2[e]);
          }
        }
      }
    }
    if (do_stats) {
      __syncthreads();
      float* red = ep;
#pragma unroll
      for (int e = 0; e < 8; ++e) {
        red[(urow * 2 + 0) * QBN + ucol + e] = s1[e];
        red[(urow * 2 + 1) * QBN + ucol + e] = s2[e];
      }
      __syncthreads();
      for (int idx = tid; idx < 2 * QBN; idx += NT) {
        const int which = idx / QBN, col = idx - which * QBN;
        const int n = n0 + col;
        if (n < a.Ntot) {
          float sum = 0.f;
          for (int w = 0; w < RPS; ++w) sum += red[(w * 2 + which) * QBN + col];
          if (a.stat_totals != nullptr) bn_live_add(a.stat_totals, pidx, which, a.Ntot, n, sum);
          else a.stat_partials[((int64_t)pidx * 2 + which) * a.Ntot + n] = sum;
        }
      }
    }
    if (!next_ok) break;
    __syncthreads();
#pragma unroll
    for (int i = 0; i < QTM; ++i) a_addr[i] += (BUF - cur) - cur;
    cur = BUF - cur;
    pidx = pnext;
    pos = posn;
  }
}

static size_t q_tab_off(int ck, int layout, int blk_per_slice, int pers) {
  const QLayout c = convq_layouts()[layout];
  if (pers != 0) return 2 * (size_t)q_buf_bytes(ck, c.WM, c.WN, c.KS, 1);
  const int NT = 64 * c.WM * c.WN * c.KS, BN = 32 * c.WN, EPP = c.WN == 4 ? 1 : 3;
  size_t lds = (size_t)(blk_per_slice > 1 ? 2 : 1) * (8 * c.WM + 2) * q_row_pitch(ck);
  const size_t epi = (size_t)c.KS * c.WM * (96 / EPP) * (BN + 4) * sizeof(float);
  const size_t red = (size_t)(NT / (BN / 8)) * 2 * BN * sizeof(float);
  if (lds < epi) lds = epi;
  if (lds < red) lds = red;
  return (lds + 15) / 16 * 16;
}

constexpr bool q_pers_ok(int ck, int nt, int x_mode, int pers) { return pers == 0 || !(ck == 128 && nt == 256 && x_mode != 0); }

template <int CK, int WM, int WN, int KS, int PERS>
int convq_launch_t(const ConvPlan& pl, hipStream_t s) {
  constexpr int NT = 64 * WM * WN * KS;
  const ConvP& p = pl.p;
  const bool aff = p.a.in_scale != nullptr || p.a.in_tot != nullptr;
  dim3 grid((unsigned)p.grid);
#define DFL_CQ_LAUNCH(AFF_)                                                                                                   \
  {                                                                                                                             \
    auto k = convq_kernel<CK, WM, WN, KS, AFF_, PERS>;                                                                          \
    DFL_LDS_OPT_IN(k, kLdsOptIn, "dfl_conv2d (bf16, unrolled 3x3)")                                                            \
    hipLaunchKernelGGL(k, grid, dim3(NT), pl.lds, s, p);                                                                        \
  }
  if (p.a.x_mode != 0) {
    if constexpr (q_pers_ok(CK, NT, 1, PERS) && PERS != 2) DFL_CQ_LAUNCH(2)
    else DFL_REQUIRE(false, "dfl_conv2d (bf16, unrolled 3x3): the persistent form of this layout does not take the two-tensor operand");
  } else if (aff) DFL_CQ_LAUNCH(1)
  else DFL_CQ_LAUNCH(0)
#undef DFL_CQ_LAUNCH
  return check_launch("dfl_conv2d (bf16, unrolled 3x3)");
}

constexpr bool q_inst(int ck, int wm, int wn, int ks) {
  return ((8 * wm + 2) * QIW * (ck / 8) + 64 * wm * wn * ks - 1) / (64 * wm * wn * ks) <= 10 && ck / 16 >= ks;
}

template <int CK, int WM, int WN, int KS>
int convq_launch_p(const ConvPlan& pl, hipStream_t s) {
  const ConvP& p = pl.p;
  if (pl.pers == 0) return convq_launch_t<CK, WM, WN, KS, 0>(pl, s);
  if constexpr (CK <= 64) {
    if (p.blk_per_slice == 1 && p.a.x_mode == 0) return convq_launch_t<CK, WM, WN, KS, 2>(pl, s);
  }
  return convq_launch_t<CK, WM, WN, KS, 1>(pl, s);
}

template <int WM, int WN, int KS>
int convq_launch_ck(const ConvPlan& pl, hipStream_t s) {
  if (pl.p.CK == 128) {
    if constexpr (q_inst(128, WM, WN, KS)) return convq_launch_p<128, WM, WN, KS>(pl, s);
  } else if (pl.p.CK == 64) {
    if constexpr (q_inst(64, WM, WN, KS)) return convq_launch_p<64, WM, WN, KS>(pl, s);
  } else if (pl.p.CK == 32) {
    if constexpr (q_inst(32, WM, WN, KS)) return convq_launch_p<32, WM, WN, KS>(pl, s);
  }
  set_error("dfl_conv2d (bf16, unrolled 3x3): no instantiation for %d resident channels in configuration %d", pl.p.CK, pl.p.tile);
  return DFL_ERR_INVALID_ARG;
}

}

const QLayout* convq_layouts() {
  static const QLayout t[kNumQ] = {{1, 4, 1, convq_launch_ck<1, 4, 1>}, {1, 4, 2, convq_launch_ck<1, 4, 2>}, {2, 4, 1, convq_launch_ck<2, 4, 1>},
                                   {2, 2, 1, convq_launch_ck<2, 2, 1>}, {4, 2, 1, convq_launch_ck<4, 2, 1>}, {2, 2, 2, convq_launch_ck<2, 2, 2>},
                                   {4, 1, 1, convq_launch_ck<4, 1, 1>}, {8, 1, 1, convq_launch_ck<8, 1, 1>}, {4, 1, 2, convq_launch_ck<4, 1, 2>}};
  return t;
}

bool convq_shape_ok(const dfl_conv_args& a) {
  return a.KH == 3 && a.KW == 3 && a.stride == 1 && a.pad == 1 && a.scatter2x2 == 0 && a.Cin % 32 == 0 && a.Ntot % 8 == 0 &&
         a.Hout == a.Hin && a.Wout == a.Win && a.out_scale == nullptr;
}

bool convq_ck_ok(int layout, int ck) {
  if (layout < 0 || layout >= kNumQ || (ck != 32 && ck != 64 && ck != 128)) return false;
  const QLayout c = convq_layouts()[layout];
  return q_inst(ck, c.WM, c.WN, c.KS);
}

size_t convq_lds_bytes(int ck, int layout, int blk_per_slice, int pers, int* tab_off) {
  const size_t off = q_tab_off(ck, layout, blk_per_slice, pers);
  if (tab_off != nullptr) *tab_off = (int)off;
  return off + (size_t)(3 * 32 * convq_layouts()[layout].WN + 3 * blk_per_slice * ck) * sizeof(float);
}

bool convq_pers_ok(int layout, int ck, int x_mode) {
  const QLayout c = convq_layouts()[layout];
  return q_pers_ok(ck, 64 * c.WM * c.WN * c.KS, x_mode, 1);
}

}
```

deepfluorolabeling-ipcai2020_amd/plan.py:

```python
import ctypes as C
import os

import numpy as np
import torch

from . import _native as nat
from ._native import (ConvArgs, WgradArgs, PackJob, BnFinalizeArgs, ColstatsArgs, BnBwdFinalizeArgs, BnReluBwdArgs,
                      AffineCopyArgs, PoolArgs, HeadFwdArgs, HeadBwdArgs, PackArgs, BnEvalArgs, UpsampleArgs, BnLiveJob, BnLiveArgs,
                      BnBwdLiveJob, BnBwdLiveArgs, MemsetArgs, ReduceJob, ReduceBatchArgs, Program)

BN_EPS = 1.0e-5
BN_MOMENTUM = 0.1


class Act:
    __slots__ = ('t', 'ptr', 'ld', 'N', 'H', 'W', 'C', 'esz')

    def __init__(self, t, ptr, ld, N, H, W, C, esz=4):
        self.t, self.ptr, self.ld, self.N, self.H, self.W, self.C, self.esz = t, ptr, ld, N, H, W, C, esz

    @property
    def M(self):
        return self.N * self.H * self.W

    @property
    def bf16(self):
        return int(self.esz == 2)

    def chan_slice(self, c0, c):
        return Act(self.t, self.ptr + self.esz * c0, self.ld, self.N, self.H, self.W, c, self.esz)


class PlanError(RuntimeError):
    pass


KEEP_GRADS = False


class _Layer:
    __slots__ = ('w', 'wname', 'relu', 'inp', 'gin', 'inp_aff', 'r', 'bn', 'live_bwd')

    def __init__(self, w, wname, relu, inp, gin, inp_aff, r, bn, live_bwd):
        self.w, self.wname, self.relu, self.inp, self.gin, self.inp_aff = w, wname, relu, inp, gin, inp_aff
        self.r, self.bn, self.live_bwd = r, bn, live_bwd


class _Block:
    __slots__ = ('prefix', 'xin', 'out', 'convs', 'rw', 'last_r', 'last_live')

    def __init__(self, prefix, xin, out):
        self.prefix, self.xin, self.out = prefix, xin, out
        self.convs = []
        self.rw = None
        self.last_r = None
        self.last_live = False


class UNetPlan:
    PACK_TILED = os.environ.get('DFL_PACK_TILED', '1') != '0'
    FUSE_BRB = os.environ.get('DFL_FUSE_BRB', '1') != '0'
    FUSE_DOWN_STATS = os.environ.get('DFL_FUSE_DOWN_STATS', '1') != '0'
    FLUSH_BYTES = int(float(os.environ.get('DFL_FLUSH_MB', '16')) * (1 << 20))
    DPRE_OUT_BYTES = int(float(os.environ.get('DFL_DPRE_OUT_MB', '12')) * (1 << 20))
    LIVE_BN = os.environ.get('DFL_LIVE_BN', '1') != '0'
    LIVE_HEAD = os.environ.get('DFL_LIVE_HEAD', '1') != '0'
    BN_R = 8

    def __init__(self, cfg, params, buffers, N, H, W, training, need_grad, device, input_grad=False):
        self.cfg = cfg
        self.P = params
        self.Bf = buffers
        self.N, self.H, self.W = N, H, W
        self.training = training
        self.need_grad = need_grad
        self.input_grad = bool(input_grad and need_grad)
        self.dx_in = None
        self.dev = device
        self.lib = nat.lib()
        self._keep = []
        self.fwd = Program()
        self.bwd = Program() if need_grad else None
        self._prep = Program()
        self._pack_jobs = []
        self.busy = False
        self.graph = None
        self.generation = 0
        self._scratch = {}
        self._red_pending = []
        self._red_bytes = 0
        self._red_flushes = []
        self.partial_sum_bytes = 0
        self._tiled_host = self._tiled_index = None
        self.math = self.lib.dfl_get_math_mode()
        self.bf16 = self.math == 4
        self.adt = torch.bfloat16 if self.bf16 else torch.float32
        self.aesz = 2 if self.bf16 else 4
        self._packed_split = {}
        self.relu_out = {}
        self._tot_fwd, self._tot_bwd, self._live_jobs, self._live_bwd_pending = [None, 0], [None, 0], [], []
        self.dbg = {}
        self.keep_grads = bool(KEEP_GRADS)
        self.pool_in = {}
        self._latency_form = int(not training and not need_grad and os.environ.get('DFL_PLAN_LATENCY_FORM', '1') != '0')
        self._build()

    def _new(self, nelem, dtype=torch.float32):
        t = torch.empty(max(int(nelem), 1), dtype=dtype, device=self.dev)
        self._keep.append(t)
        return t

    def _const(self, n, value):
        key = ('const', int(n), float(value))
        t = self._scratch.get(key)
        if t is None:
            t = torch.full((int(n),), float(value), dtype=torch.float32, device=self.dev)
            self._keep.append(t)
            self._scratch[key] = t
        return t

    def _act(self, N, H, W, C):
        t = self._new(N * H * W * C, self.adt)
        return Act(t, t.data_ptr(), C, N, H, W, C, self.aesz)

    def _scratch_act(self, key, N, H, W, C):
        need = N * H * W * C
        t = self._scratch.get(key)
        if t is None or t.numel() < need:
            raise PlanError('scratch %s not sized' % key)
        if self.keep_grads:
            return self._act(N, H, W, C)
        return Act(t, t.data_ptr(), C, N, H, W, C, self.aesz)

    def _pack(self, w, kind, flip=0):
        A, B, KH, KW = w.shape
        Cc = KH * KW
        K = {1: Cc * B, 2: Cc * A, 3: A}[kind]
        N = {1: A, 2: B, 3: Cc * B}[kind]
        cin = B if kind == 1 else A
        if self.bf16 and cin % 16 == 0:
            dst = self._new((K + 15) // 16 * N * 16, torch.bfloat16)
            self._packed_split[dst.data_ptr()] = 2
            self._pack_jobs.append((w, dst, A, B, Cc, kind, flip, 2))
            return dst
        dst = self._new((K + 3) // 4 * N * 4)
        split = int(self.math in (1, 3) and cin % 16 == 0)
        self._packed_split[dst.data_ptr()] = split
        self._pack_jobs.append((w, dst, A, B, Cc, kind, flip, split))
        return dst

    def _pack_conv_fwd(self, w):
        return self._pack(w, 1)

    def _pack_conv_dgrad(self, w):
        return self._pack(w, 2, flip=1)

    def _pack_down_dgrad(self, w):
        return self._pack(w, 3)

    def _pack_convT_fwd(self, w):
        return self._pack(w, 3)

    def _pack_convT_dgrad(self, w):
        return self._pack(w, 1)

    @staticmethod
    def _set_pack_job(a, job):
        src, dst, A, B, Cc, kind, flip, split = job
        a.src, a.dst, a.A, a.B, a.C, a.kind, a.flip, a.split = src.data_ptr(), dst.data_ptr(), A, B, Cc, kind, flip, split

    def _upload(self, arr):
        t = torch.from_numpy(np.frombuffer(bytes(arr), dtype=np.uint8).copy()).to(self.dev)
        self._keep.append(t)
        return t.data_ptr()

    def _finish_pack(self):
        self.pack = Program()
        self.pack.extend(self._prep)
        if not self._pack_jobs:
            return
        if self.PACK_TILED:
            self._finish_pack_tiled()
        else:
            self._add_pack_launch(self._pack_jobs)

    def _add_pack_launch(self, jobs):
        arr = (PackJob * len(jobs))()
        for a, job in zip(arr, jobs):
            self._set_pack_job(a, job)
        mx = max(A * B * Cc for (_, _, A, B, Cc, _, _, _) in jobs)
        self.pack.add(PackArgs(jobs_dev=self._upload(arr), max_elems=mx, njobs=len(jobs)))

    def _finish_pack_tiled(self):
        tiled, rest, by_src = [], [], {}
        for job in self._pack_jobs:
            src, dst, A, B, Cc, kind, flip, split = job
            if A % 32 == 0 and B % 32 == 0 and Cc <= 9:
                k = src.data_ptr()
                if k in by_src and len(by_src[k]) == 1:
                    by_src[k].append(job)
                else:
                    by_src[k] = [job]
                    tiled.append(by_src[k])
            else:
                rest.append(job)
        if tiled:
            arr = (PackJob * len(tiled))()
            tiles = 0
            for a, group in zip(arr, tiled):
                self._set_pack_job(a, group[0])
                if len(group) > 1:
                    a.dst2, a.kind2, a.flip2, a.split2 = group[1][1].data_ptr(), group[1][5], group[1][6], group[1][7]
                a.first_tile = tiles
                tiles += (a.A // 32) * (a.B // 32)
            self._tiled_index = len(self.pack)
            self.pack.add(PackArgs(jobs_dev=self._upload(arr), max_elems=tiles, njobs=len(tiled), tiled=1))
            srcs = [g[0][0].data_ptr() for g in tiled]
            if len(set(srcs)) == len(srcs):
                self._tiled_host = (bytes(arr), len(tiled), tiles, {g[0][0].data_ptr(): g[0][0].numel() for g in tiled})
        if rest:
            self._add_pack_launch(rest)

    def _conv(self, prog, x, w, y, KH, KW, stride, pad, Ntot, bias=None, in_aff=None, relu=0, add=None,
              add_aff=None, accumulate=0, scatter=0, stats=False, stat_other=None, Hout=None, Wout=None, x_split=0, brb=None,
              in_live=None, add_live=None, stat_totals=None, x_out=None, out_aff=None):
        a = ConvArgs()
        a.x, a.w, a.y = x.ptr, w.data_ptr(), y.ptr
        a.w_split = self._packed_split.get(w.data_ptr(), 0)
        a.x_split = x_split
        a.x_bf16, a.y_bf16 = x.bf16, y.bf16
        if (add is not None and add.bf16 != y.bf16) or (stat_other is not None and stat_other.bf16 != y.bf16):
            raise PlanError('internal: mixed element types in a convolution epilogue')
        a.bias = nat.ptr(bias)
        if in_aff is not None:
            a.in_scale, a.in_shift = in_aff[0].data_ptr(), in_aff[1].data_ptr()
        if in_live is not None:
            a.in_tot, a.in_gamma, a.in_beta, a.in_count = in_live[0], in_live[1].data_ptr(), in_live[2].data_ptr(), float(in_live[3])
            a.bn_eps = BN_EPS
        if add_live is not None:
            a.add_tot, a.add_gamma, a.add_beta, a.add_count = add_live[0], add_live[1].data_ptr(), add_live[2].data_ptr(), float(add_live[3])
            a.bn_eps = BN_EPS
        if brb is not None:
            r_act, coef = brb
            a.x_mode, a.x2, a.ldx2 = 1, r_act.ptr, r_act.ld
            if isinstance(coef, dict):
                a.in_tot, a.in_gamma, a.in_mean, a.in_invstd = coef['tot'], coef['gamma'].data_ptr(), coef['mean'].data_ptr(), coef['invstd'].data_ptr()
                a.in_count = float(coef['count'])
            else:
                a.in_scale = nat.ptr(coef)
            if x_out is not None:
                a.x_out, a.ldxo = x_out.ptr, x_out.ld
        if add is not None:
            a.add, a.ldadd = add.ptr, add.ld
            if add_aff is not None:
                a.add_scale, a.add_shift = add_aff[0].data_ptr(), add_aff[1].data_ptr()
        a.N, a.Hin, a.Win, a.Cin, a.ldx = x.N, x.H, x.W, x.C, x.ld
        a.KH, a.KW, a.stride, a.pad = KH, KW, stride, pad
        a.Hout, a.Wout = (y.H, y.W) if Hout is None else (Hout, Wout)
        a.Ntot, a.ldy = Ntot, y.ld
        a.relu, a.accumulate, a.scatter2x2 = relu, accumulate, scatter
        a.latency_form = self._latency_form
        self._out_aff_taken = False
        if out_aff is not None:
            a.out_scale, a.out_shift = out_aff[0].data_ptr(), out_aff[1].data_ptr()
            if self.lib.dfl_conv_config(C.addressof(a)) == 16 + nat.CONV_CFG_LATENCY:
                self._out_aff_taken = True
            else:
                a.out_scale, a.out_shift = None, None
        sp = nat.check(self.lib.dfl_conv_suggest_splits(C.addressof(a)), 'dfl_conv_suggest_splits')
        if sp > 1:
            M = x.N * (x.H * x.W if scatter else a.Hout * a.Wout)
            a.splits = sp
            a.partial = self._shared_scratch('conv_partial', sp * M * Ntot).data_ptr()
        partials = None
        if stat_totals is not None:
            a.stat_totals = stat_totals
            if stat_other is not None:
                a.stat_other, a.ldso = stat_other.ptr, stat_other.ld
            partials = ('live', stat_totals)
        elif stats:
            gm = nat.check(self.lib.dfl_conv_grid_m(C.addressof(a)), 'dfl_conv_grid_m')
            partials = self._new(gm * 2 * Ntot)
            a.stat_partials = partials.data_ptr()
            if stat_other is not None:
                a.stat_other, a.ldso = stat_other.ptr, stat_other.ld
            partials = (partials, 4 * gm if scatter else gm)
        prog.add(a)
        return partials

    def _wgrad(self, prog, g, d, dw, KH, KW, stride, pad, Hout, Wout, in_aff=None, d_split=0, brb=None,
               bias_out=None, bias_plain=False):
        a = WgradArgs()
        a.d_split = d_split
        a.g_bf16, a.d_bf16 = g.bf16, d.bf16
        a.g, a.d, a.dw = g.ptr, d.ptr, dw.data_ptr()
        if in_aff is not None:
            a.in_scale, a.in_shift = in_aff[0].data_ptr(), in_aff[1].data_ptr()
        a.N, a.Hin, a.Win, a.Cg, a.ldg = g.N, g.H, g.W, g.C, g.ld
        a.KH, a.KW, a.stride, a.pad = KH, KW, stride, pad
        a.Hout, a.Wout, a.Cm, a.ldd = Hout, Wout, d.C, d.ld
        if brb is not None:
            r_act, coef = brb
            a.d_mode, a.d2, a.ldd2 = 1, r_act.ptr, r_act.ld
            if isinstance(coef, dict):
                a.coef_tot, a.bn_gamma, a.bn_mean, a.bn_invstd = coef['tot'], coef['gamma'].data_ptr(), coef['mean'].data_ptr(), coef['invstd'].data_ptr()
                a.bn_count = float(coef['count'])
            else:
                a.coef = nat.ptr(coef)
        a.splits = 1
        s = nat.check(self.lib.dfl_wgrad_suggest_splits(C.addressof(a)), 'dfl_wgrad_suggest_splits')
        a.splits = s
        bias_job = None
        if (brb is not None or bias_plain) and bias_out is not None:
            bpart = self._new(s * d.C)
            a.bias_partial = bpart.data_ptr()
            bias_job = (bpart.data_ptr(), bias_out.data_ptr(), d.C, d.C, s, 1)
        n = d.C * g.C * KH * KW
        if s > 1:
            big = 4 * n >= self.FLUSH_BYTES
            part = self._shared_scratch('wg_partial', s * n) if big else self._new(s * n)
            a.partial = part.data_ptr()
        prog.add(a)
        if bias_job is not None:
            self._red_pending.append(bias_job)
            self._red_bytes += 4 * d.C
        if s > 1:
            self._defer_sum(prog, part.data_ptr(), dw.data_ptr(), n, n, s, KH * KW)

    def _defer_sum(self, prog, src, dst, n, stride, count, T=1):
        self._red_pending.append((src, dst, n, stride, count, T))
        self._red_bytes += 4 * n
        self._maybe_flush(prog)

    def _maybe_flush(self, prog):
        if self._red_bytes >= self.FLUSH_BYTES:
            self._flush_sums(prog)

    def _flush_sums(self, prog):
        self._flush_live_bwd(prog)
        jobs = self._red_pending
        if not jobs:
            return
        arr = (ReduceJob * len(jobs))()
        blocks = 0
        for a, (src, dst, n, stride, count, T) in zip(arr, jobs):
            a.src, a.dst, a.n, a.stride, a.count, a.first_block, a.T = src, dst, n, stride, count, blocks, T
            blocks += nat.check(self.lib.dfl_reduce_job_blocks(n, count), 'dfl_reduce_job_blocks')
        self._red_flushes.append((len(prog.structs), [j[1] for j in jobs]))
        self.partial_sum_bytes += sum(4 * n * count for (_, _, n, _, count, _) in jobs)
        prog.add(ReduceBatchArgs(jobs_dev=self._upload(arr), njobs=len(jobs), total_blocks=blocks))
        self._red_pending, self._red_bytes = [], 0

    def _dz_for(self, g, N, H, W, Cc, fused):
        key = 'dpre0' if fused and g.t is self._scratch.get('dz') else 'dz'
        return self._scratch_act(key, N, H, W, Cc)

    def _bn_totals(self, Cc, bwd=False):
        need = self.BN_R * 2 * Cc
        ar = self._tot_bwd if bwd else self._tot_fwd
        if ar[0] is None:
            ar[0] = self._new(sum(self.chans) * self.bd * 2 * self.BN_R * 2, torch.float64)
        assert ar[1] + need <= ar[0].numel()
        ptr = ar[0].data_ptr() + 8 * ar[1]
        ar[1] += need
        return ptr

    def _flush_live_bwd(self, prog):
        jobs = self._live_bwd_pending
        if not jobs:
            return
        arr = (BnBwdLiveJob * len(jobs))()
        for a, j in zip(arr, jobs):
            a.totals, a.save_mean, a.save_invstd = j['tot'], j['mean'].data_ptr(), j['invstd'].data_ptr()
            a.dgamma, a.dbeta, a.sum_out, a.C = j['dgamma'].data_ptr(), j['dbeta'].data_ptr(), nat.ptr(j['sum_out']), j['C']
        dsts = [j[k].data_ptr() for j in jobs for k in ('dgamma', 'dbeta', 'sum_out') if j[k] is not None]
        self._red_flushes.append((len(prog.structs), dsts))
        prog.add(BnBwdLiveArgs(jobs_dev=self._upload(arr), njobs=len(jobs), max_C=max(j['C'] for j in jobs)))
        self._live_bwd_pending = []

    def _finish_live_bn(self):
        jobs = self._live_jobs
        if not jobs:
            return
        arr = (BnLiveJob * len(jobs))()
        for a, j in zip(arr, jobs):
            a.totals, a.gamma, a.beta = j['totals'], j['gamma'].data_ptr(), j['beta'].data_ptr()
            a.running_mean = self.Bf[j['bname'] + '.running_mean'].data_ptr()
            a.running_var = self.Bf[j['bname'] + '.running_var'].data_ptr()
            a.num_batches_tracked = self.Bf[j['bname'] + '.num_batches_tracked'].data_ptr()
            a.scale, a.shift, a.save_mean, a.save_invstd = (j[k].data_ptr() for k in ('scale', 'shift', 'mean', 'invstd'))
            a.count, a.C, a.eps, a.momentum = j['count'], j['C'], BN_EPS, BN_MOMENTUM
        self.fwd.add(BnLiveArgs(jobs_dev=self._upload(arr), njobs=len(jobs), max_C=max(j['C'] for j in jobs)))
        self.fwd.insert(0, MemsetArgs(ptr=self._tot_fwd[0].data_ptr(), bytes=8 * self._tot_fwd[1]))

    def _shared_scratch(self, key, nelem):
        t = self._scratch.get(key)
        if t is None or t.numel() < nelem:
            t = self._new(nelem)
            self._scratch[key] = t
        return t

    def _colsum(self, prog, a, out):
        nb = self.lib.dfl_rowblock_count(a.M, a.C)
        part = self._new(nb * 2 * a.C)
        prog.add(ColstatsArgs(a=a.ptr, b=None, partials=part.data_ptr(), M=a.M, C=a.C, lda=a.ld, ldb=0, nblocks=nb,
                              bf16=a.bf16))
        self._defer_sum(prog, part.data_ptr(), out.data_ptr(), a.C, 2 * a.C, nb)

    _WRAP = ((-1, 0, 1), (0, 1, None), (0, None, 1))

    def _wrap_regions(self, H, W):
        out = []
        for sy, dy, h in ((H - 1, 0, 1), (0, 1, H), (0, H + 1, 1)):
            for sx, dx, w in ((W - 1, 0, 1), (0, 1, W), (0, W + 1, 1)):
# ... 483 lines not shown
        N, G, bwd = self.N, self.G, self.bwd
        dnxt = dnxt_sums = None
        for i in reversed(range(self.depth)):
            rec = self._down[i]
            blk = rec['blk']
            out = blk.out
            Ci = self.chans[i]
            if i != self.depth - 1:
                sums = None
                if self.direct_bridge[i]:
                    dout = self.dcat[i].chan_slice(Ci, Ci)
                else:
                    dout = self._act(N, out.H, out.W, Ci)
                    oy, ox, ch, cw = rec['crop']
                    src = self.dcat[i].chan_slice(Ci, Ci)
                    bwd.add(MemsetArgs(ptr=dout.ptr, bytes=dout.esz * dout.M * Ci))
                    bwd.add(AffineCopyArgs(x=src.ptr, y=dout.ptr, N=N, H=ch, W=cw, C=Ci, ldx=src.ld, xH=ch, xW=cw,
                                           ldy=dout.ld, yH=out.H, yW=out.W, yoy=oy, yox=ox, bf16=src.bf16))
                nxt = rec['nxt']
                if self.cfg['max_pool']:
                    bwd.add_pool(PoolArgs(x=out.ptr, y=dnxt.ptr, dx=dout.ptr, N=N, H=out.H, W=out.W, C=Ci, ldx=out.ld,
                                          ldy=dnxt.ld, lddx=dout.ld, bf16=out.bf16), backward=True)
                else:
                    wname = 'downsample_convs.%d' % i
                    if dnxt_sums is not None:
                        self._defer_sum(bwd, dnxt_sums[0].data_ptr(), G[wname + '.bias'].data_ptr(), Ci, 2 * Ci, dnxt_sums[1])
                    else:
                        self._colsum(bwd, dnxt, G[wname + '.bias'])
                    self._wgrad(bwd, out, dnxt, G[wname + '.weight'], 2, 2, 2, 0, nxt.H, nxt.W)
                    wd = self._pack_down_dgrad(self.P[wname + '.weight'])
                    r_last = blk.last_r
                    want = (self.FUSE_DOWN_STATS and r_last is not None and bool(dout.bf16) and bool(r_last.bf16)
                            and out.H == 2 * nxt.H and out.W == 2 * nxt.W)
                    sums = self._conv(bwd, dnxt, wd, dout, 1, 1, 1, 0, 4 * Ci, accumulate=1, scatter=1,
                                      Hout=out.H, Wout=out.W, stats=want, stat_other=r_last if want else None,
                                      stat_totals=self._bn_totals(Ci, bwd=True) if (want and blk.last_live) else None)
            xin = blk.xin
            if i > 0:
                dxin = self._act(N, xin.H, xin.W, xin.C)
            elif self.input_grad:
                if self.bf16:
                    raise PlanError('gradients with respect to the network input are implemented for the fp32-tensor arithmetic '
                                    'modes only (DFL_MATH=fp32 / bf16x3 / bf16x6 / bf16), not for bf16 storage')
                dxin = self.dx_in = self._act(N, xin.H, xin.W, xin.C)
            else:
                dxin = None
            dnxt_sums = self._block_backward(blk, dout, dxin, fused_in=sums,
                                             dxin_stats=dxin is not None and i > 0 and not self.cfg['max_pool'])
            dnxt = dxin

    def _block_backward(self, blk, dout, dxin, fused_in=None, dxin_stats=False):
        self.dbg['dout:' + blk.prefix] = dout
        if dxin is not None:
            self.dbg['dxin:' + blk.prefix] = dxin
        if self.do_res:
            self._wgrad(self.bwd, blk.xin, dout, self.G[blk.prefix + '.res_conv1x1.weight'], 1, 1, 1, 0, blk.xin.H, blk.xin.W)
        g, sums = dout, fused_in
        for d in reversed(range(self.bd)):
            self.dbg['g:' + blk.convs[d].relu] = g
            coef = self._bn_backward_coef(blk, d, g, sums)
            g, sums = self._layer_backward(blk, d, g, coef, dout, dxin, dxin_stats)
            self._maybe_flush(self.bwd)
        return sums

    def _bn_backward_coef(self, blk, d, g, sums):
        cv, G, bwd = blk.convs[d], self.G, self.bwd
        r, Cout = cv.r, cv.r.C
        res_bias = G[blk.prefix + '.res_conv1x1.bias'] if (self.do_res and d == self.bd - 1) else None
        if cv.bn is None:
            if res_bias is not None:
                self._colsum(bwd, g, res_bias)
            return None
        gamma, mean, invstd, bname = cv.bn
        if sums is not None and sums[0] == 'live':
            assert cv.live_bwd
            self._live_bwd_pending.append(dict(tot=sums[1], mean=mean, invstd=invstd, dgamma=G[bname + '.weight'],
                                               dbeta=G[bname + '.bias'], C=Cout, sum_out=res_bias))
            return dict(tot=sums[1], gamma=gamma, mean=mean, invstd=invstd, count=r.M)
        if sums is None:
            nb = self.lib.dfl_rowblock_count(r.M, Cout)
            part = self._new(nb * 2 * Cout)
            bwd.add(ColstatsArgs(a=g.ptr, b=r.ptr, partials=part.data_ptr(), M=r.M, C=Cout, lda=g.ld,
                                 ldb=r.ld, nblocks=nb, bf16=r.bf16))
            sums = (part, nb)
        part, prow = sums
        coef = self._new(3 * Cout)
        self.dbg['coef:' + cv.relu] = coef
        bwd.add(BnBwdFinalizeArgs(partials=part.data_ptr(), gamma=gamma.data_ptr(),
                                  save_mean=mean.data_ptr(), save_invstd=invstd.data_ptr(),
                                  dgamma=G[bname + '.weight'].data_ptr(),
                                  dbeta=G[bname + '.bias'].data_ptr(), coef=coef.data_ptr(),
                                  count=r.M if self.training else 0,
                                  nblocks=prow, C=Cout))
        if res_bias is not None:
            self._defer_sum(bwd, part.data_ptr(), res_bias.data_ptr(), Cout, 2 * Cout, prow)
        return coef

    def _layer_backward(self, blk, d, g, coef, dout, dxin, dxin_stats):
        cv, G, bwd, N = blk.convs[d], self.G, self.bwd, self.N
        r, inp, Cout, pad, circ = cv.r, cv.inp, cv.r.C, self.pad, self.circular
        self._dpre_turn ^= 1
        if g.t is self._scratch.get('dpre%d' % self._dpre_turn):
            self._dpre_turn ^= 1
        fuse_brb = self.FUSE_BRB and bool(r.bf16) and bool(inp.bf16) and inp.C % 16 == 0 and g.bf16 == r.bf16
        if (self.FUSE_BRB and bool(r.bf16) and g.bf16 == r.bf16 and not inp.bf16 and inp.C == 1
                and d == 0 and dxin is None and Cout in (8, 16, 32, 64)):
            fuse_brb = True
        brb = (r, coef) if fuse_brb else None
        dsplit = 0
        if fuse_brb:
            dpre = g
        else:
            dpre = self._scratch_act('dpre%d' % self._dpre_turn, N, r.H, r.W, Cout)
            nb = self.lib.dfl_rowblock_count(r.M, Cout)
            bpart = self._new(nb * Cout)
            dsplit = int(self.math in (1, 3) and Cout % 16 == 0 and inp.C % 4 == 0 and inp.C * 9 > 12)
            bwd.add(BnReluBwdArgs(dy=g.ptr, r=r.ptr, coef=nat.ptr(coef), dpre=dpre.ptr,
                                  partials=bpart.data_ptr(), M=r.M, C=Cout, lddy=g.ld, ldr=r.ld, ldo=dpre.ld,
                                  nblocks=nb, split_out=dsplit, bf16=r.bf16))
            self._defer_sum(bwd, bpart.data_ptr(), G[cv.wname + '.bias'].data_ptr(), Cout, Cout, nb)
        dmat = None
        if (fuse_brb and bool(inp.bf16) and not circ and pad == 1 and (d > 0 or dxin is not None)
                and 'dmat' in self._scratch and r.M * Cout * 2 <= self.DPRE_OUT_BYTES):
            dmat = self._scratch_act('dmat', N, r.H, r.W, Cout)
            self.dbg['dmat:' + cv.relu] = dmat
        if dmat is None:
            self._layer_wgrad(cv, dpre, d_split=dsplit, brb=brb)
        sums = None
        if circ and (d > 0 or dxin is not None):
            wd = self._pack_conv_dgrad(cv.w)
            dzp = self._framed_grad(inp)
            self._conv(bwd, dpre, wd, dzp, 3, 3, 1, 2, inp.C, x_split=dsplit, brb=brb)
            if d > 0:
                g = self._dz_for(g, N, inp.H, inp.W, Cout, fuse_brb)
                self._wrap_fold(bwd, dzp, g)
            else:
                self._wrap_fold(bwd, dzp, dxin)
                if self.do_res:
                    sums = self._conv(bwd, dout, self._pack_conv_dgrad(blk.rw), dxin, 1, 1, 1, 0, blk.xin.C,
                                      accumulate=1, stats=dxin_stats)
        elif d > 0:
            wd = self._pack_conv_dgrad(cv.w)
            dz = self._dz_for(g, N, inp.H, inp.W, Cout, fuse_brb)
            prev = blk.convs[d - 1]
            if prev.bn is not None:
                sums = self._conv(bwd, dpre, wd, dz, 3, 3, 1, 2 - pad, Cout, stats=True, stat_other=prev.r,
                                  x_split=dsplit, brb=brb, x_out=dmat,
                                  stat_totals=self._bn_totals(Cout, bwd=True) if prev.live_bwd else None)
            else:
                self._conv(bwd, dpre, wd, dz, 3, 3, 1, 2 - pad, Cout, x_split=dsplit, brb=brb, x_out=dmat)
            g = dz
        elif dxin is not None:
            wd = self._pack_conv_dgrad(cv.w)
            sums = self._conv(bwd, dpre, wd, dxin, 3, 3, 1, 2 - pad, blk.xin.C,
                              x_split=dsplit, stats=dxin_stats and not self.do_res, brb=brb, x_out=dmat)
            if self.do_res:
                sums = self._conv(bwd, dout, self._pack_conv_dgrad(blk.rw), dxin, 1, 1, 1, 0, blk.xin.C,
                                  accumulate=1, stats=dxin_stats)
        if dmat is not None:
            self._layer_wgrad(cv, dmat, bias_plain=True)
        return g, sums

    def _layer_wgrad(self, cv, d, **kw):
        self._wgrad(self.bwd, cv.gin, d, self.G[cv.wname + '.weight'], 3, 3, 1, 0 if self.circular else self.pad, cv.r.H, cv.r.W,
                    in_aff=cv.inp_aff, bias_out=self.G[cv.wname + '.bias'], **kw)

    def _finish_backward(self):
        self._flush_sums(self.bwd)
        if self._tot_bwd[0] is not None:
            self.bwd.insert(0, MemsetArgs(ptr=self._tot_bwd[0].data_ptr(), bytes=8 * self._tot_bwd[1]))
            self._red_flushes = [(idx + 1, dsts) for idx, dsts in self._red_flushes]

    def _grad_ready_ops(self):
        by_ptr = {self.G[k].data_ptr(): k for k in self.grad_names}
        self.grad_ready_op = {}
        for idx, st in enumerate(self.bwd.structs):
            for field in ('dw', 'dst', 'out', 'dgamma', 'dbeta', 'dw_seg', 'dw_l1', 'dw_l2'):
                name = by_ptr.get(getattr(st, field, None))
                if name is not None:
                    self.grad_ready_op[name] = idx
        for idx, dsts in self._red_flushes:
            for d in dsts:
                name = by_ptr.get(d)
                if name is not None:
                    self.grad_ready_op[name] = max(idx, self.grad_ready_op.get(name, -1))
        last = len(self.bwd.structs) - 1
        if self.g_l2_eff is not None:
            for name in self.tail_names:
                self.grad_ready_op[name] = last
        if self.eff_heads is not None:
            for name in ('seg_conv.weight', 'lands_1x1.0.weight'):
                self.grad_ready_op[name] = last

    def fold_tail(self):
        if self.eff_heads is not None:
            e = self.eff_heads
            F, F2 = e['F'], e['F2']
            e['w_seg'][:, :F].copy_(self.P['seg_conv.weight'])
            w1 = self.P['lands_1x1.0.weight']
            e['w_l1'][:, F:F + F2].copy_(w1[:, :F2])
            e['w_l1'][:, F + F2:].copy_(w1[:, F2:])
        if self.w_l2_eff is None:
            return
        mats = [self.P[n].view(self.P[n].shape[0], self.P[n].shape[1]) for n in self.tail_names]
        eff = mats[0]
        for m in mats[1:]:
            eff = m @ eff
        self.w_l2_eff.view(eff.shape).copy_(eff)

    def unfold_tail_grads(self):
        if self.eff_heads is not None and self.need_grad:
            e = self.eff_heads
            F, F2 = e['F'], e['F2']
            if self.split_heads:
                torch.add(self.g_seg_full, e['g_seg'][:, :F], out=self.G['seg_conv.weight'])
            else:
                self.G['seg_conv.weight'].copy_(e['g_seg'][:, :F])
            g1 = self.G['lands_1x1.0.weight']
            g1[:, :F2].copy_(e['g_l1'][:, F:F + F2])
            g1[:, F2:].copy_(e['g_l1'][:, F + F2:])
        if self.g_l2_eff is None:
            return
        mats = [self.P[n].view(self.P[n].shape[0], self.P[n].shape[1]) for n in self.tail_names]
        G = self.g_l2_eff.view(mats[-1].shape[0], mats[0].shape[1])
        k = len(mats)
        below = [None] * k
        for j in range(1, k):
            below[j] = mats[j - 1] if below[j - 1] is None else mats[j - 1] @ below[j - 1]
        above = None
        for j in reversed(range(k)):
            g = G if above is None else above.t() @ G
            if below[j] is not None:
                g = g @ below[j].t()
            self.G[self.tail_names[j]].view(g.shape).copy_(g)
            above = mats[j] if above is None else above @ mats[j]

    def run_pack_rest(self, stream):
        i, n = self._tiled_index, len(self.pack)
        if i > 0:
            self.pack.run(stream, 0, i)
        if n - i - 1 > 0:
            self.pack.run(stream, i + 1, n - i - 1)

    def new_outputs(self):
        N = self.N
        h, w = self.out_hw
        hl, wl = self.heat_hw
        seg = torch.empty((N, self.NC, h, w), dtype=torch.float32, device=self.dev)
        heat = torch.empty((N, self.L, hl, wl), dtype=torch.float32, device=self.dev) if self.L > 0 else None
        return seg, heat

    def bind_outputs(self, seg, heat):
        if self.split_heads:
            self.head_fwd_seg.seg = seg.data_ptr()
            self.head_fwd.seg = self.seg_crop.data_ptr()
        else:
            self.head_fwd.seg = seg.data_ptr()
        self.head_fwd.heat = nat.ptr(heat)

    def bind_grads(self, seg, dseg, dheat):
        if self.split_heads:
            self.head_bwd_seg.seg, self.head_bwd_seg.dseg = seg.data_ptr(), dseg.data_ptr()
            self.head_bwd.seg, self.head_bwd.dseg = self.seg_crop.data_ptr(), self.dseg_zero.data_ptr()
        else:
            self.head_bwd.seg, self.head_bwd.dseg = seg.data_ptr(), dseg.data_ptr()
        self.head_bwd.dheat = nat.ptr(dheat)

    def grads(self):
        return [None if k in self.dead_params else self.G[k] for k in self.grad_names]

    def act_nchw(self, act):
        esz = act.esz
        base = act.t.view(-1)
        off = (act.ptr - base.data_ptr()) // esz
        v = base.as_strided((act.N, act.H, act.W, act.C), (act.H * act.W * act.ld, act.W * act.ld, act.ld, 1), off)
        return v.permute(0, 3, 1, 2).float().contiguous()
```

include/dfl_hip.h:

```cpp
#ifndef DFL_HIP_H
#define DFL_HIP_H

#include <stddef.h>
#include <stdint.h>

#ifdef __cplusplus
extern "C" {
#endif

typedef void* dfl_stream_t;

typedef enum {
  DFL_OK = 0,
  DFL_ERR_INVALID_ARG = -1,
  DFL_ERR_UNSUPPORTED = -2,
  DFL_ERR_LAUNCH = -3,
  DFL_ERR_WORKSPACE = -4
} dfl_status;

int dfl_version(void);
const char* dfl_last_error(void);
int dfl_sizeof(int which);

typedef struct {
  const float* x;
  const float* w;
  const float* bias;
  const float* in_scale;
  const float* in_shift;
  const float* add;
  const float* add_scale;
  const float* add_shift;
  const float* stat_other;
  float* y;
  float* stat_partials;
  float* partial;
  int32_t N, Hin, Win, Cin, ldx;
  int32_t KH, KW, stride, pad;
  int32_t Hout, Wout, Ntot, ldy;
  int32_t ldadd, ldso;
  int32_t relu;
  int32_t accumulate;
  int32_t scatter2x2;
  int32_t splits;
  int32_t w_split;
  int32_t x_split;
  int32_t x_bf16, y_bf16;
  const float* x2;
  int32_t ldx2, x_mode;
  double* stat_totals;
  const double* in_tot;
  const float* in_gamma;
  const float* in_beta;
  const double* add_tot;
  const float* add_gamma;
  const float* add_beta;
  double in_count, add_count;
  float bn_eps;
  int32_t reserved3;
  const float* in_mean;
  const float* in_invstd;
  void* x_out;
  int32_t ldxo;
  int32_t latency_form;
  const float* out_scale;
  const float* out_shift;
} dfl_conv_args;
#define DFL_BN_R 8

int dfl_conv2d(const dfl_conv_args* a, dfl_stream_t stream);
int dfl_conv2d_pair(const dfl_conv_args* a, const dfl_conv_args* b, dfl_stream_t stream);
int dfl_conv_pair_ok(const dfl_conv_args* a, const dfl_conv_args* b);
int dfl_conv_grid_m(const dfl_conv_args* a);
int dfl_conv_suggest_splits(const dfl_conv_args* a);

int dfl_conv_candidates(const dfl_conv_args* a, int32_t* out, int32_t max_rows);
int dfl_conv_force_geometry(const int32_t* geom);
int dfl_conv_tune_add(const int32_t* key, const int32_t* geom);

typedef struct {
  const float* g;
  const float* d;
  const float* in_scale;
  const float* in_shift;
  float* dw;
  float* partial;
  int32_t N, Hin, Win, Cg, ldg;
  int32_t KH, KW, stride, pad;
  int32_t Hout, Wout, Cm, ldd;
  int32_t splits;
  int32_t d_split;
  int32_t g_bf16, d_bf16;
  int32_t d_mode;
  const float* d2;
  const float* coef;
  float* bias_partial;
  int32_t ldd2, reserved2;
  const double* coef_tot;
  const float* bn_gamma;
  const float* bn_mean;
  const float* bn_invstd;
  double bn_count;
} dfl_wgrad_args;

int dfl_conv2d_wgrad(const dfl_wgrad_args* a, dfl_stream_t stream);
int dfl_wgrad_suggest_splits(const dfl_wgrad_args* a);

int dfl_sum_partials(const float* src, float* dst, int64_t n, int32_t splits, int32_t T, dfl_stream_t stream);

typedef struct {
  const float* src;
  float* dst;
  int32_t A, B, C;
  int32_t kind, flip;
  int32_t split;
  float* dst2;
  int32_t kind2, flip2;
  int32_t first_tile;
  int32_t split2;
} dfl_pack_job;

int dfl_pack_weights(const dfl_pack_job* jobs_dev, int32_t njobs, int64_t max_elems, dfl_stream_t stream);
int dfl_pack_weights_tiled(const dfl_pack_job* jobs_dev, int32_t njobs, int32_t total_tiles, dfl_stream_t stream);

typedef struct {
  const float* partials;
  const float* gamma;
  const float* beta;
  float* running_mean;
  float* running_var;
  int64_t* num_batches_tracked;
  float* scale;
  float* shift;
  float* save_mean;
  float* save_invstd;
  int64_t count;
  int32_t nblocks, C;
  float eps, momentum;
} dfl_bn_finalize_args;

int dfl_bn_finalize(const dfl_bn_finalize_args* a, dfl_stream_t stream);

typedef struct {
  const double* totals;
  const float* gamma; const float* beta;
  float* running_mean; float* running_var; int64_t* num_batches_tracked;
  float* scale; float* shift; float* save_mean; float* save_invstd;
  int64_t count;
  int32_t C;
  float eps, momentum;
  int32_t reserved;
} dfl_bn_live_job;
int dfl_bn_finalize_live(const dfl_bn_live_job* jobs_dev, int32_t njobs, int32_t max_C, dfl_stream_t stream);
typedef struct {
  const double* totals;
  const float* save_mean; const float* save_invstd;
  float* dgamma; float* dbeta; float* sum_out;
  int32_t C, reserved;
} dfl_bn_bwd_live_job;
int dfl_bn_bwd_finalize_live(const dfl_bn_bwd_live_job* jobs_dev, int32_t njobs, int32_t max_C, dfl_stream_t stream);
int dfl_bn_eval_prepare(const float* gamma, const float* beta, const float* running_mean,
                        const float* running_var, float* scale, float* shift, int32_t C, float eps,
                        dfl_stream_t stream);

int dfl_rowblock_count(int64_t M, int32_t C);

typedef struct {
  const float* a; const float* b;
  float* partials;
  int64_t M;
  int32_t C, lda, ldb, nblocks;
  int32_t bf16, reserved;
} dfl_colstats_args;
int dfl_colstats(const dfl_colstats_args* a, dfl_stream_t stream);

typedef struct {
  const float* partials;
  const float* gamma; const float* save_mean; const float* save_invstd;
  float* dgamma; float* dbeta;
  float* coef;
  int64_t count;
  int32_t nblocks, C;
} dfl_bn_bwd_finalize_args;
int dfl_bn_bwd_finalize(const dfl_bn_bwd_finalize_args* a, dfl_stream_t stream);

typedef struct {
  const float* dy; const float* r; const float* coef;
  float* dpre;
  float* partials;
  int64_t M;
  int32_t C, lddy, ldr, ldo, nblocks;
  int32_t split_out;
  int32_t bf16, reserved;
} dfl_bn_relu_bwd_args;
int dfl_bn_relu_bwd_apply(const dfl_bn_relu_bwd_args* a, dfl_stream_t stream);

int dfl_reduce_partials(const float* partials, float* out, int32_t nblocks, int32_t stride, int32_t C,
                        dfl_stream_t stream);

typedef struct {
  const float* src;
  float* dst;
  int64_t n, stride;
  int32_t count, first_block;
  int32_t T, reserved;
} dfl_reduce_job;
int dfl_reduce_job_blocks(int64_t n, int32_t count);
int dfl_reduce_batch(const dfl_reduce_job* jobs_dev, int32_t njobs, int32_t total_blocks, dfl_stream_t stream);

typedef struct {
  const float* x; float* y; const float* scale; const float* shift;
  int32_t N, H, W, C;
  int32_t ldx, xH, xW, xoy, xox;
  int32_t ldy, yH, yW, yoy, yox;
  int32_t accumulate;
  int32_t bf16;
} dfl_affine_copy_args;
int dfl_affine_copy(const dfl_affine_copy_args* a, dfl_stream_t stream);

// ... 329 lines not shown
int dfl_mesh_transform(const dfl_mesh_xform_args* a, dfl_stream_t stream);

typedef struct {
  const float* pos;
  const int32_t* tris;
  const int32_t* vt_ptr;
  const int32_t* vt_tri;
  float* normals;
  int64_t V;
} dfl_mesh_normals_args;
int dfl_mesh_normals(const dfl_mesh_normals_args* a, dfl_stream_t stream);

#define DFL_PREPROC_MAX_FACTOR 16
typedef struct {
  const void* pixels;
  const int32_t* rot180;
  float* out;
  uint32_t* scratch;
  int32_t N, R, C, crop, factor;
  int32_t u16, log;
  float min_intensity;
} dfl_preproc_projs_args;
int dfl_preproc_projs(const dfl_preproc_projs_args* a, dfl_stream_t stream);

typedef struct {
  const unsigned char* segs;
  const int32_t* rot180;
  unsigned char* out;
  int32_t* status;
  int32_t N, R, C, crop, factor, reserved;
} dfl_preproc_segs_args;
int dfl_preproc_segs(const dfl_preproc_segs_args* a, dfl_stream_t stream);

typedef struct {
  const unsigned char* labels;
  const int32_t* rot180;
  unsigned char* out;
  int32_t N, R, C, crop, factor, reserved;
} dfl_restore_labels_args;
int dfl_restore_labels(const dfl_restore_labels_args* a, dfl_stream_t stream);

#define DFL_DRR_EXACT 0
#define DFL_DRR_TRILINEAR 1
#define DFL_DRR_MAX_LABELS 16
typedef struct {
  float o[3];
  float M[9];
  int32_t box_lo[3], box_hi[3];
  uint32_t mask;
} dfl_drr_object;

typedef struct {
  const float* mu;
  const unsigned char* labels;
  const dfl_drr_object* objects;
  float* att;
  float* plen;
  unsigned char* label_map;
  float qscale[9];
  int32_t nx, ny, nz, H, W, views, n_obj, n_labels;
  int32_t interp, mapping;
  float step_mm, min_len_mm;
  int32_t reserved;
} dfl_drr_args;
int dfl_drr_render(const dfl_drr_args* a, dfl_stream_t stream);

#define DFL_SIM_TOTALS 5
typedef struct {
  const float* fixed;
  const unsigned char* mask;
  float* fx;
  float* fy;
  unsigned char* counted;
  double* totals;
  int32_t H, W;
} dfl_sim_prepare_args;
int dfl_sim_prepare(const dfl_sim_prepare_args* a, dfl_stream_t stream);

typedef struct {
  const float* moving;
  const float* fx;
  const float* fy;
  const unsigned char* counted;
  const double* totals;
  double* scratch;
  double* cost;
  int64_t scratch_doubles;
  int32_t V, H, W, reserved;
} dfl_sim_gradncc_args;
int dfl_sim_gradncc(const dfl_sim_gradncc_args* a, dfl_stream_t stream);
int64_t dfl_sim_scratch_doubles(int32_t V, int32_t H, int32_t W);

#define DFL_EXPOSE_MAX_RADIUS 8
typedef struct {
  const float* att;
  void* out;
  const uint64_t* key_q;
  const uint64_t* key_e;
  float* z1;
  float* z2;
  float taps[2 * DFL_EXPOSE_MAX_RADIUS + 1];
  int32_t rho;
  int32_t V, R, C;
  int32_t u16, quantum, electronic;
  float photons, gain, electronic_sigma;
} dfl_expose_args;
int dfl_drr_expose(const dfl_expose_args* a, dfl_stream_t stream);

#define DFL_MATH_DEFAULT 0
int dfl_get_math_mode(void);
int dfl_set_math_mode(int32_t mode);

typedef enum {
  DFL_OP_CONV = 1, DFL_OP_WGRAD = 2, DFL_OP_SUM_PARTIALS = 3, DFL_OP_PACK = 4, DFL_OP_BN_FINALIZE = 5,
  DFL_OP_BN_EVAL = 6, DFL_OP_COLSTATS = 7, DFL_OP_BN_BWD_FINALIZE = 8, DFL_OP_BN_RELU_BWD = 9,
  DFL_OP_REDUCE_PARTIALS = 10, DFL_OP_AFFINE_COPY = 11, DFL_OP_POOL_FWD = 12, DFL_OP_POOL_BWD = 13,
  DFL_OP_HEAD_FWD = 14, DFL_OP_HEAD_BWD = 15, DFL_OP_MEMSET = 16, DFL_OP_REDUCE_BATCH = 17,
  DFL_OP_RECORD = 18, DFL_OP_WAIT = 19, DFL_OP_UPSAMPLE_FWD = 20, DFL_OP_UPSAMPLE_BWD = 21,
  DFL_OP_BN_FINALIZE_LIVE = 22, DFL_OP_BN_BWD_FINALIZE_LIVE = 23, DFL_OP_CONV_PAIR = 24
} dfl_op_kind;

typedef struct { const float* src; float* dst; int64_t n; int32_t splits; int32_t T; } dfl_sum_partials_args;
typedef struct { const dfl_pack_job* jobs_dev; int64_t max_elems; int32_t njobs; int32_t tiled; } dfl_pack_args;
typedef struct { const float* gamma; const float* beta; const float* running_mean; const float* running_var;
                 float* scale; float* shift; int32_t C; float eps; } dfl_bn_eval_args;
typedef struct { const float* partials; float* out; int32_t nblocks, stride, C, reserved; } dfl_reduce_partials_args;
typedef struct { void* ptr; int64_t bytes; } dfl_memset_args;
typedef struct { const dfl_reduce_job* jobs_dev; int32_t njobs, total_blocks; } dfl_reduce_batch_args;
typedef struct { const dfl_bn_live_job* jobs_dev; int32_t njobs, max_C; } dfl_bn_live_args;
typedef struct { const dfl_bn_bwd_live_job* jobs_dev; int32_t njobs, max_C; } dfl_bn_bwd_live_args;
typedef struct { const dfl_conv_args* a; const dfl_conv_args* b; } dfl_conv_pair_args;

typedef struct { int32_t event; int32_t reserved; } dfl_sync_args;
#define DFL_MAX_SIDE_STREAMS 2

typedef struct {
  int32_t kind;
  int32_t stream;
  const void* args;
} dfl_op;

int dfl_exec(const dfl_op* ops, int32_t n_ops, dfl_stream_t stream);
int dfl_exec_timed(const dfl_op* ops, int32_t n_ops, dfl_stream_t stream, float* ms_out);

int dfl_set_conv_rows_min_tiles(int32_t n);

typedef struct dfl_graph_s* dfl_graph_t;
int dfl_graph_capture(const dfl_op* ops, int32_t n_ops, dfl_stream_t stream, dfl_graph_t* graph_out);
int dfl_graph_launch(dfl_graph_t graph, dfl_stream_t stream);
int dfl_graph_nodes(dfl_graph_t graph);
int dfl_graph_destroy(dfl_graph_t graph);
int dfl_conv_config(const dfl_conv_args* a);
int dfl_wgrad_config(const dfl_wgrad_args* a);

#ifdef __cplusplus
}
#endif
#endif
```

Before: 4643 images/sec.

## Fuse residual 1x1 dgrad into the 3x3 dgrad conv as a second K section

In the backward pass of residual blocks, the 1x1 residual-path data-gradient conv is folded into the 3x3 data-gradient conv kernel as an extra K section read straight from global memory with buffer loads. This removes a separate kernel launch and the read-modify-write accumulate pass over dxin. The main accumulator is first rounded to bf16 so the numerics match the old two-kernel path. It applies only to certain tile instantiations and only to unsliced launches, and it can force latency_form off and drop K-splitting for those layers.

```diff
diff --git a/deepfluorolabeling-ipcai2020_amd/_native.py b/deepfluorolabeling-ipcai2020_amd/_native.py
--- a/deepfluorolabeling-ipcai2020_amd/_native.py
+++ b/deepfluorolabeling-ipcai2020_amd/_native.py
@@ -20,7 +20,8 @@
                 ('x2', fp), ('ldx2', i32), ('x_mode', i32),
                 ('stat_totals', fp), ('in_tot', fp), ('in_gamma', fp), ('in_beta', fp), ('add_tot', fp), ('add_gamma', fp),
                 ('add_beta', fp), ('in_count', C.c_double), ('add_count', C.c_double), ('bn_eps', f32), ('reserved3', i32),
-                ('in_mean', fp), ('in_invstd', fp), ('x_out', fp), ('ldxo', i32), ('latency_form', i32), ('out_scale', fp), ('out_shift', fp)]
+                ('in_mean', fp), ('in_invstd', fp), ('x_out', fp), ('ldxo', i32), ('latency_form', i32), ('out_scale', fp), ('out_shift', fp),
+                ('x3', fp), ('w3', fp), ('ldx3', i32), ('C3', i32)]
 
 
 class WgradArgs(C.Structure):
@@ -377,7 +378,7 @@
            'dfl_mesh_mc_count', 'dfl_mesh_mc_emit', 'dfl_mesh_decode', 'dfl_mesh_topology', 'dfl_mesh_csr', 'dfl_mesh_smooth',
            'dfl_mesh_transform', 'dfl_mesh_normals', 'dfl_adam_step', 'dfl_rmsprop_step', 'dfl_optim_pack_tiled',
            'dfl_preproc_projs', 'dfl_preproc_segs', 'dfl_restore_labels', 'dfl_drr_render', 'dfl_sim_prepare', 'dfl_sim_gradncc',
-           'dfl_sim_scratch_doubles', 'dfl_drr_expose']
+           'dfl_sim_scratch_doubles', 'dfl_drr_expose', 'dfl_conv_res_fuse_ok']
 
 
 class DflError(RuntimeError):
@@ -460,6 +461,7 @@
     L.dfl_conv_tune_add.argtypes = [fp, fp]
     L.dfl_conv2d_pair.argtypes = [fp, fp, fp]
     L.dfl_conv_pair_ok.argtypes = [fp, fp]
+    L.dfl_conv_res_fuse_ok.argtypes = [fp]
     for k, cls in enumerate(_SIZEOF_ORDER):
         if L.dfl_sizeof(k) != C.sizeof(cls):
             raise DflError('struct mirror %s has size %d, library says %d' % (cls.__name__, C.sizeof(cls), L.dfl_sizeof(k)))
diff --git a/deepfluorolabeling-ipcai2020_amd/csrc/conv_plan.hip b/deepfluorolabeling-ipcai2020_amd/csrc/conv_plan.hip
--- a/deepfluorolabeling-ipcai2020_amd/csrc/conv_plan.hip
+++ b/deepfluorolabeling-ipcai2020_amd/csrc/conv_plan.hip
@@ -406,6 +406,22 @@
     DFL_REQUIRE(x2b < lim, "dfl_conv2d (bf16): tensors must stay below 2 GiB");
     p->x2_bytes = (uint32_t)x2b;
   }
+  if (a->x3 != nullptr) {
+    DFL_REQUIRE(a->w3 != nullptr && a->C3 > 0 && a->C3 % 16 == 0 && a->ldx3 % 8 == 0 && a->ldx3 >= a->C3 && aligned16(a->x3) && aligned16(a->w3),
+                "dfl_conv2d (bf16): x3 needs w3, C3 %% 16 == 0, ldx3 %% 8 == 0, ldx3 >= C3 and 16-byte aligned x3 / w3 (C3 = %d, ldx3 = %d)", a->C3, a->ldx3);
+    DFL_REQUIRE(a->y_bf16 && a->KH == 3 && a->KW == 3 && a->stride == 1 && a->pad == 1 && a->Hout == a->Hin && a->Wout == a->Win,
+                "dfl_conv2d (bf16): x3 goes with a 3x3 stride-1 pad-1 layer of bf16 tensors");
+    DFL_REQUIRE(a->add == nullptr && a->accumulate == 0 && a->relu == 0 && a->bias == nullptr && a->scatter2x2 == 0 && a->out_scale == nullptr &&
+                    a->latency_form == 0,
+                "dfl_conv2d (bf16): x3 excludes add, accumulate, relu, bias, scatter2x2, out_scale and latency_form");
+    const int64_t x3b = (((int64_t)a->N * a->Hin * a->Win - 1) * a->ldx3 + a->C3) * 2;
+    const int64_t w3b = (int64_t)a->C3 * a->Ntot * 2;
+    DFL_REQUIRE(x3b < lim && w3b < lim, "dfl_conv2d (bf16): tensors must stay below 2 GiB");
+    p->x3_bytes = (uint32_t)x3b;
+    p->w3_bytes = (uint32_t)w3b;
+  } else {
+    DFL_REQUIRE(a->w3 == nullptr && a->C3 == 0 && a->ldx3 == 0, "dfl_conv2d (bf16): w3 / C3 / ldx3 without x3");
+  }
   p->xo_bytes = 0;
   if (a->x_out != nullptr) {
     DFL_REQUIRE(a->x_mode == 1 && a->KH == 3 && a->KW == 3 && a->stride == 1 && a->pad == 1 && a->Hout == a->Hin && a->Wout == a->Win,
@@ -544,10 +560,22 @@
   return true;
 }
 
+bool conv_res_section_ok(const ConvPlan& pl) {
+  const ConvP& p = pl.p;
+  if (p.a.x3 == nullptr || p.a.x_mode != 1 || p.splits > 1 || p.tile < 0 || p.tile >= (int)tiles().size()) return false;
+  const Tile& t = tiles()[p.tile];
+  if (t.family == Family::Unrolled) return convq_res_ok(t.layout, p.CK, pl.pers);
+  return t.family == Family::Patch && convp_res_ok(t.layout);
+}
+
 int conv_route(const dfl_conv_args* a, int want_splits, ConvRoute* r) {
+  DFL_REQUIRE(a == nullptr || a->x_bf16 || (a->x3 == nullptr && a->w3 == nullptr), "dfl_conv2d: the second K section (x3) needs bf16 tensors");
   if (a != nullptr && a->x_bf16) {
     const int rc = convp_plan(a, &r->plan, want_splits);
     if (rc != DFL_OK) return rc;
+    DFL_REQUIRE(a->x3 == nullptr || conv_res_section_ok(r->plan),
+                "dfl_conv2d (bf16): the kernel this block routes to (configuration %d, %d K slices) does not take the second K section (x3): "
+                "ask dfl_conv_res_fuse_ok", r->plan.p.tile, r->plan.p.splits);
     r->form = FORM_BF16;
     r->cfg = 16 + r->plan.p.tile;
     r->splits = r->plan.p.splits;
@@ -615,6 +643,14 @@
   return rc != DFL_OK ? rc : r.splits;
 }
 
+extern "C" int dfl_conv_res_fuse_ok(const dfl_conv_args* a) {
+  DFL_REQUIRE(a != nullptr && a->x_bf16 && a->x3 != nullptr, "dfl_conv_res_fuse_ok: bf16 convolution arguments with x3 are required");
+  dfl::ConvPlan pl;
+  const int rc = dfl::convp_plan(a, &pl, a->splits > 1 ? a->splits : 0);
+  if (rc != DFL_OK) return rc;
+  return dfl::conv_res_section_ok(pl) ? 1 : 0;
+}
+
 extern "C" int dfl_conv_pair_ok(const dfl_conv_args* a, const dfl_conv_args* b) {
   dfl::ConvRoute r;
   return dfl::conv_pair_route(a, b, &r);
diff --git a/deepfluorolabeling-ipcai2020_amd/csrc/convp.h b/deepfluorolabeling-ipcai2020_amd/csrc/convp.h
--- a/deepfluorolabeling-ipcai2020_amd/csrc/convp.h
+++ b/deepfluorolabeling-ipcai2020_amd/csrc/convp.h
@@ -21,6 +21,7 @@
   int tab_off, pad1;
   int s_mt, s_nt, s_ksplit_shift, s_cpk_shift, s_ksteps, s_kper;
   uint32_t qm_npatch, qm_ntiles, qm_perimg, qm_npx;
+  uint32_t x3_bytes, w3_bytes;
   int q_ngroups, q_stride;
 };
 constexpr int CONVS_TILE = 39;
@@ -40,11 +41,13 @@
 int convp_plan(const dfl_conv_args* a, ConvPlan* pl, int force_splits);
 int convp_launch(const ConvPlan& pl, hipStream_t s);
 int convp_finish_rows(const ConvP& p);
+bool conv_res_section_ok(const ConvPlan& pl);
 bool convs_enabled();
 
 struct PatchTile { int WM, WN, TM, TN, GA, KS; ConvLaunch launch; };
 constexpr int kNumPatchTiles = CONVS_TILE;
 const PatchTile* convp_tiles();
+bool convp_res_ok(int tile);
 
 struct QLayout { int WM, WN, KS; ConvLaunch launch; };
 constexpr int kNumQ = 9;
@@ -52,6 +55,7 @@
 bool convq_shape_ok(const dfl_conv_args& a);
 size_t convq_lds_bytes(int ck, int layout, int blk_per_slice, int pers, int* tab_off);
 bool convq_pers_ok(int layout, int ck, int x_mode);
+bool convq_res_ok(int layout, int ck, int pers);
 bool convq_ck_ok(int layout, int ck);
 
 struct NLayout { int WX, R; ConvLaunch launch; };
diff --git a/deepfluorolabeling-ipcai2020_amd/csrc/convp_bf16.hip b/deepfluorolabeling-ipcai2020_amd/csrc/convp_bf16.hip
--- a/deepfluorolabeling-ipcai2020_amd/csrc/convp_bf16.hip
+++ b/deepfluorolabeling-ipcai2020_amd/csrc/convp_bf16.hip
@@ -19,7 +19,7 @@
 #ifndef DFL_CONVP_PRIME
 #define DFL_CONVP_PRIME 0
 #endif
-template <int WM, int WN, int TM, int TN, int AFF, bool GA, int KS = 1>
+template <int WM, int WN, int TM, int TN, int AFF, bool GA, int KS = 1, bool RES = false>
 #ifndef DFL_CONVP_ADEPTH
 #define DFL_CONVP_ADEPTH 1
 #endif
@@ -30,6 +30,7 @@
   static_assert(WM * WN == 4, "four waves per k-group");
   static_assert(KS == 1 || (KS == 2 && !GA), "two k-groups: LDS-image form only");
   static_assert(AFF != 2 || !GA, "the fused BatchNorm + ReLU backward operand is staged through LDS");
+  static_assert(!RES || (AFF == 2 && !GA && KS == 1), "the second K section: two-tensor operand, LDS-image form, one k-group");
   constexpr int NT = 256 * KS;
   extern __shared__ __attribute__((aligned(16))) unsigned char smem[];
   const dfl_conv_args& a = p.a;
@@ -398,6 +399,68 @@
       }
     }
     TRACC(2, tb1)
+  }
+  if constexpr (RES) {
+#pragma unroll
+    for (int i = 0; i < TM; ++i)
+#pragma unroll
+      for (int j = 0; j < TN; ++j)
+#pragma unroll
+        for (int r = 0; r < 16; r += 2) {
+          const uint32_t w = pack_bf2(acc[i][j][r], acc[i][j][r + 1]);
+          acc[i][j][r] = bf_lo(w);
+          acc[i][j][r + 1] = bf_hi(w);
+        }
+    __amdgpu_buffer_rsrc_t rsX3 = __builtin_amdgcn_make_buffer_rsrc(const_cast<void*>(a.x3), 0, (int)p.x3_bytes, 0x00020000);
+    __amdgpu_buffer_rsrc_t rsW3 = __builtin_amdgcn_make_buffer_rsrc(const_cast<void*>(a.w3), 0, (int)p.w3_bytes, 0x00020000);
+    uint32_t r_goff[TM];
+#pragma unroll
+    for (int i = 0; i < TM; ++i) {
+      const int q = (wm * TM + i) * 32 + li;
+      const int img = pdiv(q, p.mPP, PP);
+      const int r = q - img * PP;
+      const int py = pdiv(r, p.mPW, p.PW), px = r - py * p.PW;
+      const int n = img0 + img, gy = gy0 + py, gx = gx0 + px;
+      const bool ok = img < p.IPP && n < a.N && gy < p.Hg && gx < p.Wg;
+      r_goff[i] = ok ? (uint32_t)(((n * a.Hin + gy) * a.Win + gx) * a.ldx3) * 2u + (uint32_t)lh * 16u : POOB;
+    }
+    constexpr int RG = 2;
+    const int rchunks = a.C3 >> 4;
+    const uint32_t rbstep = (uint32_t)a.Ntot * 32u;
+    pu32x4 rareg[2][RG][TM], rbreg[2][RG][TN];
+    auto res_load = [&](int g, int set) {
+#pragma unroll
+      for (int e = 0; e < RG; ++e) {
+        const int c = g * RG + e;
+        const bool live = c < rchunks;
+        const uint32_t ao = live ? (uint32_t)c * 32u : 0u, bo = live ? (uint32_t)c * rbstep : 0u;
+#pragma unroll
+        for (int i = 0; i < TM; ++i) rareg[set][e][i] = __builtin_amdgcn_raw_buffer_load_b128(rsX3, live ? r_goff[i] : POOB, ao, 0);
+#pragma unroll
+        for (int j = 0; j < TN; ++j) rbreg[set][e][j] = __builtin_amdgcn_raw_buffer_load_b128(rsW3, live ? b_voff[j] : POOB, bo, 0);
+      }
+    };
+    auto res_compute = [&](int set) {
+#pragma unroll
+      for (int e = 0; e < RG; ++e)
+#pragma unroll
+        for (int j = 0; j < TN; ++j) {
+          const bf16x8_t bf = __builtin_bit_cast(bf16x8_t, rbreg[set][e][j]);
+#pragma unroll
+          for (int i = 0; i < TM; ++i)
+            acc[i][j] = __builtin_amdgcn_mfma_f32_32x32x16_bf16(__builtin_bit_cast(bf16x8_t, rareg[set][e][i]), bf, acc[i][j], 0, 0, 0);
+        }
+    };
+    const int rgroups = (rchunks + RG - 1) / RG;
+    res_load(0, 0);
+    for (int g = 0; g < rgroups; g += 2) {
+      res_load(g + 1, 1);
+      res_compute(0);
+      if (g + 1 < rgroups) {
+        res_load(g + 2, 0);
+        res_compute(1);
+      }
+    }
   }
   }
   TR(3)
@@ -703,6 +766,10 @@
 
 int convp_finish_rows(const ConvP& p) { return finish_rows_p(p.Mtot, p.a.Ntot); }
 
+constexpr bool p_res_inst(int wm, int wn, int tm, int tn, bool ga, int ks) {
+  return !ga && ks == 1 && !(wm == 2 && wn == 2 && tm == 4 && tn == 1) && !(wm == 1 && wn == 4 && tm == 2 && tn == 1);
+}
+
 template <int WM, int WN, int TM, int TN, bool GA = false, int KS = 1>
 static int convp_launch_t(const ConvPlan& pl, hipStream_t s) {
   const ConvP& p = pl.p;
@@ -710,9 +777,19 @@
   dim3 grid((unsigned)p.grid);
   constexpr int NT_ = 256 * KS;
   if constexpr (GA) {
+    DFL_REQUIRE(p.a.x3 == nullptr, "dfl_conv2d (bf16): the streamed configurations do not take the second K section (x3)");
     auto k = convp_kernel<WM, WN, TM, TN, 0, true>;
     DFL_LDS_OPT_IN(k, kLdsOptIn, "dfl_conv2d (bf16)")
     hipLaunchKernelGGL(k, grid, dim3(256), pl.lds, s, p);
+  } else if (p.a.x3 != nullptr) {
+    if constexpr (p_res_inst(WM, WN, TM, TN, GA, KS)) {
+      DFL_REQUIRE(p.a.x_mode != 0 && p.splits <= 1, "dfl_conv2d (bf16): the second K section (x3) needs x_mode 1 and an unsliced launch");
+      auto k = convp_kernel<WM, WN, TM, TN, 2, false, 1, true>;
+      DFL_LDS_OPT_IN(k, kLdsOptIn, "dfl_conv2d (bf16)")
+      hipLaunchKernelGGL(k, grid, dim3(NT_), pl.lds, s, p);
+    } else {
+      DFL_REQUIRE(false, "dfl_conv2d (bf16): this configuration is not built with the second K section (dfl_conv_res_fuse_ok tells)");
+    }
   } else if (p.a.x_mode != 0) {
     auto k = convp_kernel<WM, WN, TM, TN, 2, false, KS>;
     DFL_LDS_OPT_IN(k, kLdsOptIn, "dfl_conv2d (bf16)")
@@ -751,6 +828,11 @@
   return t;
 }
 
+bool convp_res_ok(int tile) {
+  const PatchTile& t = convp_tiles()[tile];
+  return p_res_inst(t.WM, t.WN, t.TM, t.TN, t.GA != 0, t.KS);
+}
+
 int convp_launch(const ConvPlan& pl, hipStream_t s) {
   const ConvP& p = pl.p;
   const int rc = pl.launch(pl, s);
diff --git a/deepfluorolabeling-ipcai2020_amd/csrc/convq_bf16.hip b/deepfluorolabeling-ipcai2020_amd/csrc/convq_bf16.hip
--- a/deepfluorolabeling-ipcai2020_amd/csrc/convq_bf16.hip
+++ b/deepfluorolabeling-ipcai2020_amd/csrc/convq_bf16.hip
@@ -28,8 +28,16 @@
   return (b + 15) / 16 * 16;
 }
 
-template <int CK, int WM, int WN, int KS, int AFF, int PERS>
+constexpr int q_res_depth(int ck, int wm, int wn, int ks, int pers) {
+  if (pers == 0) return 4;
+  const bool tight = (ck == 128 && ks == 2 && ((wm == 1 && wn == 4) || (wm == 2 && wn == 2))) || (ck == 32 && ks == 1 && wn == 1) ||
+                     (ck == 64 && wm == 2 && wn == 2 && ks == 1) || (ck == 64 && wm == 4 && wn == 1 && ks == 2);
+  return tight ? 2 : 4;
+}
+
+template <int CK, int WM, int WN, int KS, int AFF, int PERS, bool RES = false>
 __global__ void __launch_bounds__(64 * WM * WN * KS, 2) convq_kernel(const ConvP p) {
+  static_assert(!RES || (AFF == 2 && PERS != 2), "the second K section: two-tensor operand, not the one-block persistent form");
   constexpr int NT = 64 * WM * WN * KS;
   static_assert(NT == 256 || NT == 512, "four or eight waves");
   constexpr int QBN = 32 * WN, QEP = QBN + 4;
@@ -329,6 +337,79 @@
         fetch_a(1);
       }
     }
+    if constexpr (RES) {
+      __amdgpu_buffer_rsrc_t rsX3 = __builtin_amdgcn_make_buffer_rsrc(const_cast<void*>(a.x3), 0, (int)p.x3_bytes, 0x00020000);
+      __amdgpu_buffer_rsrc_t rsW3 = __builtin_amdgcn_make_buffer_rsrc(const_cast<void*>(a.w3), 0, (int)p.w3_bytes, 0x00020000);
+      uint32_t r_goff[QTM];
+#pragma unroll
+      for (int i = 0; i < QTM; ++i) {
+        const int q = i * 32 + li, py = q / QPW, px = q - py * QPW;
+        const int gy = pos.gy0 + wm * 8 + py, gx = pos.gx0 + px;
+        const uint32_t pixel = ((uint32_t)pos.img * (uint32_t)a.Hin + (uint32_t)gy) * (uint32_t)a.Win + (uint32_t)gx;
+        r_goff[i] = (gy < p.Hg && gx < p.Wg) ? pixel * (uint32_t)a.ldx3 * 2u + (uint32_t)lh * 16u : QOOB;
+      }
+      constexpr int RD = q_res_depth(CK, WM, WN, KS, PERS);
+      const int rchunks = a.C3 >> 4;
+      const int rsteps = (rchunks - kg + KS - 1) / KS;
+      qu32x4 rareg[RD][QTM], rbreg[RD];
+      auto res_load = [&](const int j, const int set) __attribute__((always_inline)) {
+        const bool live = j < rsteps;
+        const uint32_t c = (uint32_t)(j * KS + kg);
+#pragma unroll
+        for (int i = 0; i < QTM; ++i) rareg[set][i] = __builtin_amdgcn_raw_buffer_load_b128(rsX3, live ? r_goff[i] : QOOB, live ? c * 32u : 0u, 0);
+        rbreg[set] = __builtin_amdgcn_raw_buffer_load_b128(rsW3, live ? b_voff : QOOB, live ? c * nt32 : 0u, 0);
+      };
+      auto res_compute = [&](const int set) __attribute__((always_inline)) {
+        const bf16x8_t bf = __builtin_bit_cast(bf16x8_t, rbreg[set]);
+#pragma unroll
+        for (int i = 0; i < QTM; ++i) acc[i] = __builtin_amdgcn_mfma_f32_32x32x16_bf16(__builtin_bit_cast(bf16x8_t, rareg[set][i]), bf, acc[i], 0, 0, 0);
+      };
+#pragma unroll
+      for (int d = 0; d < RD; ++d) res_load(d, d);
+      if constexpr (KS == 2) {
+        float* xg = reinterpret_cast<float*>(smem + (PERS != 0 ? cur : 0u));
+        const int wv = wm * WN + wn;
+#pragma unroll
+        for (int pass = 0; pass < EPP; ++pass) {
+          __syncthreads();
+          if (kg == 1) {
+#pragma unroll
+            for (int i = 0; i < TPP; ++i)
+#pragma unroll
+              for (int r = 0; r < 16; ++r) xg[((wv * TPP + i) * 16 + r) * 64 + lane] = acc[pass * TPP + i][r];
+          }
+          __syncthreads();
+          if (kg == 0) {
+#pragma unroll
+            for (int i = 0; i < TPP; ++i)
+#pragma unroll
+              for (int r = 0; r < 16; ++r) acc[pass * TPP + i][r] += xg[((wv * TPP + i) * 16 + r) * 64 + lane];
+          }
+        }
+      }
+      if (KS == 1 || kg == 0) {
+#pragma unroll
+        for (int i = 0; i < QTM; ++i)
+#pragma unroll
+          for (int r = 0; r < 16; r += 2) {
+            const uint32_t w = pack_bf2(acc[i][r], acc[i][r + 1]);
+            acc[i][r] = bf_lo(w);
+            acc[i][r + 1] = bf_hi(w);
+          }
+      } else {
+#pragma unroll
+        for (int i = 0; i < QTM; ++i)
+#pragma unroll
+          for (int r = 0; r < 16; ++r) acc[i][r] = 0.f;
+      }
+      for (int j = 0; j < rsteps; j += RD) {
+#pragma unroll
+        for (int d = 0; d < RD; ++d) {
+          if (j + d < rsteps) res_compute(d);
+          res_load(j + d + RD, d);
+        }
+      }
+    }
     if constexpr (PERS == 2) {
       if (next_ok) {
 #pragma unroll
@@ -472,6 +553,13 @@
 
 constexpr bool q_pers_ok(int ck, int nt, int x_mode, int pers) { return pers == 0 || !(ck == 128 && nt == 256 && x_mode != 0); }
 
+constexpr bool q_res_inst(int ck, int wm, int wn, int ks, int pers) {
+  if (pers != 0)
+    return !((ck == 128 && wm == 2 && wn == 4 && ks == 1) || (ck == 64 && wm == 4 && wn == 2 && ks == 1) || (ck == 128 && wm == 2 && wn == 2 && ks == 2) ||
+             (ck == 32 && wm == 8 && wn == 1 && ks == 1) || (ck == 64 && wm == 2 && wn == 2 && ks == 1));
+  return !(ck == 32 && wm == 2 && wn == 4 && ks == 1);
+}
+
 template <int CK, int WM, int WN, int KS, int PERS>
 int convq_launch_t(const ConvPlan& pl, hipStream_t s) {
   constexpr int NT = 64 * WM * WN * KS;
@@ -484,7 +572,14 @@
     DFL_LDS_OPT_IN(k, kLdsOptIn, "dfl_conv2d (bf16, unrolled 3x3)")                                                            \
     hipLaunchKernelGGL(k, grid, dim3(NT), pl.lds, s, p);                                                                        \
   }
-  if (p.a.x_mode != 0) {
+  if (p.a.x3 != nullptr) {
+    DFL_REQUIRE(p.a.x_mode != 0 && p.splits <= 1, "dfl_conv2d (bf16, unrolled 3x3): the second K section (x3) needs x_mode 1 and an unsliced launch");
+    if constexpr (q_pers_ok(CK, NT, 1, PERS) && PERS != 2 && q_res_inst(CK, WM, WN, KS, PERS)) {
+      auto k = convq_kernel<CK, WM, WN, KS, 2, PERS, true>;
+      DFL_LDS_OPT_IN(k, kLdsOptIn, "dfl_conv2d (bf16, unrolled 3x3)")
+      hipLaunchKernelGGL(k, grid, dim3(NT), pl.lds, s, p);
+    } else DFL_REQUIRE(false, "dfl_conv2d (bf16, unrolled 3x3): this instance is not built with the second K section (dfl_conv_res_fuse_ok tells)");
+  } else if (p.a.x_mode != 0) {
     if constexpr (q_pers_ok(CK, NT, 1, PERS) && PERS != 2) DFL_CQ_LAUNCH(2)
     else DFL_REQUIRE(false, "dfl_conv2d (bf16, unrolled 3x3): the persistent form of this layout does not take the two-tensor operand");
   } else if (aff) DFL_CQ_LAUNCH(1)
@@ -546,6 +641,11 @@
   return off + (size_t)(3 * 32 * convq_layouts()[layout].WN + 3 * blk_per_slice * ck) * sizeof(float);
 }
 
+bool convq_res_ok(int layout, int ck, int pers) {
+  const QLayout c = convq_layouts()[layout];
+  return q_res_inst(ck, c.WM, c.WN, c.KS, pers != 0 ? 1 : 0);
+}
+
 bool convq_pers_ok(int layout, int ck, int x_mode) {
   const QLayout c = convq_layouts()[layout];
   return q_pers_ok(ck, 64 * c.WM * c.WN * c.KS, x_mode, 1);
diff --git a/deepfluorolabeling-ipcai2020_amd/plan.py b/deepfluorolabeling-ipcai2020_amd/plan.py
--- a/deepfluorolabeling-ipcai2020_amd/plan.py
+++ b/deepfluorolabeling-ipcai2020_amd/plan.py
@@ -60,6 +60,7 @@
 class UNetPlan:
     PACK_TILED = os.environ.get('DFL_PACK_TILED', '1') != '0'
     FUSE_BRB = os.environ.get('DFL_FUSE_BRB', '1') != '0'
+    FUSE_RES_DGRAD = os.environ.get('DFL_FUSE_RES_DGRAD', '1') != '0'
     FUSE_DOWN_STATS = os.environ.get('DFL_FUSE_DOWN_STATS', '1') != '0'
     FLUSH_BYTES = int(float(os.environ.get('DFL_FLUSH_MB', '16')) * (1 << 20))
     DPRE_OUT_BYTES = int(float(os.environ.get('DFL_DPRE_OUT_MB', '12')) * (1 << 20))
@@ -223,7 +224,7 @@
 
     def _conv(self, prog, x, w, y, KH, KW, stride, pad, Ntot, bias=None, in_aff=None, relu=0, add=None,
               add_aff=None, accumulate=0, scatter=0, stats=False, stat_other=None, Hout=None, Wout=None, x_split=0, brb=None,
-              in_live=None, add_live=None, stat_totals=None, x_out=None, out_aff=None):
+              in_live=None, add_live=None, stat_totals=None, x_out=None, out_aff=None, res=None):
         a = ConvArgs()
         a.x, a.w, a.y = x.ptr, w.data_ptr(), y.ptr
         a.w_split = self._packed_split.get(w.data_ptr(), 0)
@@ -260,6 +261,11 @@
         a.Ntot, a.ldy = Ntot, y.ld
         a.relu, a.accumulate, a.scatter2x2 = relu, accumulate, scatter
         a.latency_form = self._latency_form
+        if res is not None:
+            a.latency_form = 0
+            a.x3, a.w3, a.ldx3, a.C3 = res[0].ptr, res[1].data_ptr(), res[0].ld, res[0].C
+            if nat.check(self.lib.dfl_conv_res_fuse_ok(C.addressof(a)), 'dfl_conv_res_fuse_ok') != 1:
+                return False
         self._out_aff_taken = False
         if out_aff is not None:
             a.out_scale, a.out_shift = out_aff[0].data_ptr(), out_aff[1].data_ptr()
@@ -1049,11 +1055,17 @@
             g = dz
         elif dxin is not None:
             wd = self._pack_conv_dgrad(cv.w)
-            sums = self._conv(bwd, dpre, wd, dxin, 3, 3, 1, 2 - pad, blk.xin.C,
-                              x_split=dsplit, stats=dxin_stats and not self.do_res, brb=brb, x_out=dmat)
-            if self.do_res:
-                sums = self._conv(bwd, dout, self._pack_conv_dgrad(blk.rw), dxin, 1, 1, 1, 0, blk.xin.C,
-                                  accumulate=1, stats=dxin_stats)
+            wres = self._pack_conv_dgrad(blk.rw) if self.do_res else None
+            sums = False
+            if (self.do_res and self.FUSE_RES_DGRAD and fuse_brb and pad == 1 and bool(dxin.bf16) and bool(dout.bf16)
+                    and dout.C % 16 == 0):
+                sums = self._conv(bwd, dpre, wd, dxin, 3, 3, 1, 1, blk.xin.C, stats=dxin_stats, brb=brb, x_out=dmat,
+                                  res=(dout, wres))
+            if sums is False:
+                sums = self._conv(bwd, dpre, wd, dxin, 3, 3, 1, 2 - pad, blk.xin.C,
+                                  x_split=dsplit, stats=dxin_stats and not self.do_res, brb=brb, x_out=dmat)
+                if self.do_res:
+                    sums = self._conv(bwd, dout, wres, dxin, 1, 1, 1, 0, blk.xin.C, accumulate=1, stats=dxin_stats)
         if dmat is not None:
             self._layer_wgrad(cv, dmat, bias_plain=True)
         return g, sums
diff --git a/include/dfl_hip.h b/include/dfl_hip.h
--- a/include/dfl_hip.h
+++ b/include/dfl_hip.h
@@ -65,6 +65,9 @@
   int32_t latency_form;
   const float* out_scale;
   const float* out_shift;
+  const void* x3;
+  const void* w3;
+  int32_t ldx3, C3;
 } dfl_conv_args;
 #define DFL_BN_R 8
 
@@ -700,6 +703,7 @@
 int dfl_graph_destroy(dfl_graph_t graph);
 int dfl_conv_config(const dfl_conv_args* a);
 int dfl_wgrad_config(const dfl_wgrad_args* a);
+int dfl_conv_res_fuse_ok(const dfl_conv_args* a);
 
 #ifdef __cplusplus
 }
```

Result: no change. 4623 images/sec (-0.4%).
